# rug-marl-group2/scopa

Hardware: AMD Instinct MI355X
Metric: MiniScopa infoset-traversals/sec (higher is better)
Workload: dtype f64

## Files before the change

### include/scopa.h

```cpp
#ifndef SCOPA_H
#define SCOPA_H
#include <stddef.h>
#include <stdint.h>

#ifdef __cplusplus
extern "C" {
#endif

#define SCOPA_ABI_VERSION 1

enum {
    SCOPA_OK = 0,
    SCOPA_EINVAL = -1,
    SCOPA_ENODEV = -2,
    SCOPA_EHIP = -3,
    SCOPA_ESTATE = -4,
    SCOPA_ENOMEM = -5,
    SCOPA_ELIMIT = -6,
    SCOPA_ETIMEOUT = -7
};

#define SCOPA_N_CARDS 16
#define SCOPA_N_PLIES 8
#define SCOPA_N_DECISION 1653
#define SCOPA_N_TERMINAL 576
#define SCOPA_N_NODES 2229
#define SCOPA_MAX_ACTIONS 4

#define SCOPA_STEP_CLONED 0x80u
#define SCOPA_STEP_COUNT_MASK 0x7Fu
typedef struct scopa_state {
    uint16_t hand[2];
    uint32_t table;
    uint8_t  nh[2];
    uint8_t  nt;
    uint8_t  step;
    uint8_t  ncap[2];
    uint8_t  scopas[2];
} scopa_state;

typedef struct scopa_ctx scopa_ctx;

int32_t     scopa_abi_version(void);
const char *scopa_strerror(int32_t status);
const char *scopa_last_error(const scopa_ctx *ctx);

int32_t scopa_ctx_create(int32_t device_id, void *hip_stream, scopa_ctx **out);
int32_t scopa_ctx_destroy(scopa_ctx *ctx);
int32_t scopa_ctx_synchronize(scopa_ctx *ctx);

int32_t scopa_deal_py_seed(int64_t seed, uint8_t perm16[16]);
int32_t scopa_state_init(const uint8_t perm16[16], scopa_state *out);
int32_t scopa_state_step(scopa_state *s, int32_t action);
int32_t scopa_state_clone(const scopa_state *s, scopa_state *out);
int32_t scopa_state_is_terminal(const scopa_state *s);
int32_t scopa_state_current_player(const scopa_state *s);
int32_t scopa_state_legal(const scopa_state *s, int32_t player , int32_t out[4], int32_t *n);
int32_t scopa_state_rewards_x2(const scopa_state *s, int32_t r2[2]);
int32_t scopa_state_infoset_key(const scopa_state *s, int32_t player, uint64_t *key);
int32_t scopa_key_to_string(uint64_t key, char *buf, int32_t cap);
int32_t scopa_state_infoset_string(const scopa_state *s, int32_t player, char *buf, int32_t cap);

int32_t scopa_step_batch(scopa_ctx *ctx, scopa_state *d_states, const uint8_t *d_actions, int64_t n);
int32_t scopa_step_batch_host(scopa_ctx *ctx, scopa_state *h_states, const uint8_t *h_actions, int64_t n);

int32_t scopa_set_deal(scopa_ctx *ctx, const uint8_t perm16[16]);
int32_t scopa_tree_counts(scopa_ctx *ctx, int32_t *n_nodes, int32_t *n_decision, int32_t *n_infosets);
int32_t scopa_tree_export(scopa_ctx *ctx, scopa_state *h_states, int32_t *h_infoset, int8_t *h_r2,
                          uint64_t *h_infoset_key, int8_t *h_infoset_nlegal, int8_t *h_infoset_legal);

int32_t scopa_tables_reset(scopa_ctx *ctx);
int32_t scopa_tables_get(scopa_ctx *ctx, double *h_regret, double *h_strategy, double *h_local);
int32_t scopa_tables_set(scopa_ctx *ctx, const double *h_regret, const double *h_strategy, const double *h_local);

int32_t scopa_visited_get(scopa_ctx *ctx, uint32_t *h_seq);

int32_t scopa_cfr_exact_iterate(scopa_ctx *ctx, int32_t n_iters, double *h_root_values);
int32_t scopa_cfr_exact_traverse(scopa_ctx *ctx, int32_t traverser, double *h_value);
int32_t scopa_cfr_exact_mode(scopa_ctx *ctx, int32_t sequential);
int32_t scopa_cfr_exact_last_route(scopa_ctx *ctx, int32_t *route);
int32_t scopa_cfr_exact_traverse_from(scopa_ctx *ctx, int32_t traverser, int32_t depth, const int32_t *path,
                                      double reach_p0, double reach_p1, double *h_value);

int32_t scopa_cfr_sync_iterate(scopa_ctx *ctx, int32_t n_iters);

int32_t scopa_mccfr_replay(scopa_ctx *ctx, int32_t n_iters, const double *h_uniforms, int64_t n_uniforms,
                           int64_t *consumed);

int32_t scopa_mccfr_seed(scopa_ctx *ctx, uint64_t seed);
int32_t scopa_mccfr_iterate(scopa_ctx *ctx, uint32_t batch, uint32_t n_iters);
int32_t scopa_mccfr_traverse(scopa_ctx *ctx, uint32_t iteration, uint32_t b0, uint32_t nb);
int32_t scopa_mccfr_delta_buffer(scopa_ctx *ctx, void **d_delta, size_t *bytes);
int32_t scopa_mccfr_bind_delta(scopa_ctx *ctx, void *d_buf, size_t bytes);
int32_t scopa_mccfr_delta_get(scopa_ctx *ctx, double *h_delta);
int32_t scopa_mccfr_delta_set(scopa_ctx *ctx, const double *h_delta);
int32_t scopa_mccfr_apply(scopa_ctx *ctx);
int32_t scopa_mccfr_iteration_counter(scopa_ctx *ctx, uint32_t *iteration);
int32_t scopa_mccfr_graph_mode(scopa_ctx *ctx, int32_t on);
int32_t scopa_debug_lds_limit(scopa_ctx *ctx, int32_t bytes);

int32_t scopa_sdcfr_frontier_width(int32_t traverser, int32_t ply);
int32_t scopa_sdcfr_features(scopa_ctx *ctx, int32_t ply, int64_t n, const int32_t *d_idx, float *d_feats, float *d_mask);
int32_t scopa_sdcfr_expand(scopa_ctx *ctx, int32_t ply, int32_t traverser, int64_t n, const int32_t *d_idx, const float *d_adv,
                           int32_t *d_child_idx, float *d_pol, const double *d_uniforms, uint32_t iteration, uint32_t b0);
int32_t scopa_sdcfr_terminal_values(scopa_ctx *ctx, int32_t traverser, int64_t n, const int32_t *d_idx, float *d_val);
int32_t scopa_sdcfr_backward(scopa_ctx *ctx, int32_t ply, int32_t traverser, int64_t n, const int32_t *d_idx, const float *d_pol,
                             const float *d_child_val, float *d_val, const float *d_feats, const float *d_mask, float *d_mem_feat,
                             float *d_mem_regret, float *d_mem_mask, int64_t capacity, int64_t write_base);
int32_t scopa_sdcfr_visits(scopa_ctx *ctx, uint64_t *decision_visits);
int32_t scopa_sdcfr_policy_get(scopa_ctx *ctx, float *h_policy, uint64_t *h_thr);
#define SCOPA_SDCFR_IMAGE_FLOATS 13520
int32_t scopa_sdcfr_image_floats(void);
int32_t scopa_sdcfr_pack_weights(scopa_ctx *ctx, int32_t player, const float *d_w1, const float *d_b1, const float *d_w2,
                                 const float *d_b2, const float *d_w3, const float *d_b3, float *d_image);
int32_t scopa_sdcfr_traverse_fused(scopa_ctx *ctx, int32_t traverser, int32_t batch, const float *d_image, float *d_mem_feat,
                                   float *d_mem_regret, float *d_mem_mask, int64_t capacity, int64_t write_base,
                                   float *d_root_values, const double *d_uniforms, uint32_t iteration, uint32_t b0);
int32_t scopa_sdcfr_mode(scopa_ctx *ctx, int32_t forward_per_visit);
int32_t scopa_sdcfr_tuning(scopa_ctx *ctx, int32_t traversals_per_task, int32_t wavefronts_per_task);
int32_t scopa_sdcfr_train_params(void);
int32_t scopa_sdcfr_train_steps(scopa_ctx *ctx, const int64_t *d_rows, int32_t n_rows, int32_t n_steps, const float *d_feat, const float *d_regret, const float *d_mask,
                                int64_t capacity, float *d_w1, float *d_b1, float *d_w2, float *d_b2, float *d_w3, float *d_b3, float *d_state,
                                int32_t first_step, float lr, float *d_loss);
int32_t scopa_sdcfr_train_step(scopa_ctx *ctx, const int64_t *d_rows, int32_t n_rows, const float *d_feat, const float *d_regret, const float *d_mask,
                               int64_t capacity, float *d_w1, float *d_b1, float *d_w2, float *d_b2, float *d_w3, float *d_b3, float *d_state,
                               int32_t step, float lr, float *d_loss);
int32_t scopa_sdcfr_average_policy(scopa_ctx *ctx, int32_t player, int32_t n_snap, const float *d_w1, const float *d_b1, const float *d_w2,
                                   const float *d_b2, const float *d_w3, const float *d_b3, int32_t max_size, const int32_t *d_slots,
                                   const float *d_coef, double *d_policy);
int32_t scopa_features_from_states(scopa_ctx *ctx, const scopa_state *d_states, int64_t n, float *d_feats, float *d_mask);
int32_t scopa_eval_init_states(scopa_ctx *ctx, scopa_state *d_states, int64_t n);
int32_t scopa_eval_step(scopa_ctx *ctx, scopa_state *d_states, int64_t n, const float *d_probs, const int32_t *d_trained_seat,
                        uint32_t stream_id, uint32_t ply_tag);

int32_t scopa_eval_tabular_prepare(scopa_ctx *ctx, const double *d_policy);
int32_t scopa_eval_tabular_step(scopa_ctx *ctx, scopa_state *d_states, int32_t *d_node_idx, int64_t n, int32_t ply,
                                const double *d_policy, const int32_t *d_trained_seat, uint32_t stream_id);
int32_t scopa_eval_tabular_match(scopa_ctx *ctx, int64_t n, int64_t n_seat0, uint32_t stream_id, scopa_state *d_states_out, int32_t *d_node_idx_out,
                                 int64_t h_stats[10]);

int32_t scopa_exploitability(scopa_ctx *ctx, const double *h_policy, double *h_out4, double *h_policy_out);

typedef struct scopa_multi scopa_multi;
int32_t scopa_multi_create(scopa_ctx *ctx, int32_t n_deals, scopa_multi **out);
int32_t scopa_multi_destroy(scopa_multi *m);
int32_t scopa_multi_deal_py_seeds(scopa_multi *m, const int64_t *h_seeds);
int32_t scopa_multi_set_perms(scopa_multi *m, const uint8_t *h_perms );
int32_t scopa_multi_perms_get(scopa_multi *m, uint8_t *h_perms);
int32_t scopa_multi_build(scopa_multi *m, int32_t *h_n_infosets);
int32_t scopa_multi_cfr_exact_iterate(scopa_multi *m, int32_t n_iters);
int32_t scopa_multi_cfr_exact_iterate_lanes(scopa_multi *m, int32_t n_iters);
int32_t scopa_multi_cfr_sync_iterate(scopa_multi *m, int32_t n_iters);
int32_t scopa_multi_mccfr_iterate(scopa_multi *m, uint32_t batch, uint32_t n_iters, uint64_t seed);
int32_t scopa_multi_exploitability(scopa_multi *m, double *h_out4);
int32_t scopa_multi_tables_get(scopa_multi *m, int32_t deal, double *h_regret, double *h_strategy, double *h_local, uint64_t *h_keys);
int32_t scopa_multi_tables_set(scopa_multi *m, int32_t deal, const double *h_regret, const double *h_strategy, const double *h_local);
int32_t scopa_multi_counters(scopa_multi *m, uint64_t *decision_visits, uint64_t *terminal_visits);

typedef struct scopa_full_state {
    uint64_t table[2];
    uint64_t cap[2];
    uint32_t hand[2];
    uint32_t game;
    uint8_t  nh[2], nt, deck_pos, round, last_capture , scopas[2];
    uint16_t step;
    uint8_t  terminal;
    int8_t   r2_p0;
    uint8_t  flags;
    uint8_t  pad[7];
} scopa_full_state;
int32_t scopa_full_deal_py_seed(int64_t seed, uint8_t perm40[40]);
int32_t scopa_full_state_init(const uint8_t deck40[40], uint32_t game, scopa_full_state *out);
int32_t scopa_full_state_step(scopa_full_state *s, const uint8_t deck40[40], int32_t action);
int32_t scopa_full_state_legal(const scopa_full_state *s, int32_t player, int32_t out[3], int32_t *n);
int32_t scopa_full_state_infoset_string(const scopa_full_state *s, int32_t player, char *buf, int32_t cap);
int32_t scopa_full_step_batch(scopa_ctx *ctx, scopa_full_state *d_states, const uint8_t *d_actions, const uint8_t *d_decks, int64_t n);
int32_t scopa_full_step_batch_host(scopa_ctx *ctx, scopa_full_state *h_states, const uint8_t *h_actions, const uint8_t *h_decks,
                                   int64_t n_decks, int64_t n);
int32_t scopa_full_random_playouts(scopa_ctx *ctx, const int64_t *h_seeds, int64_t n_games, int8_t *h_r2_p0, int16_t *h_plies);

typedef struct scopa_team_state {
    uint64_t history;
    uint32_t table;
    uint16_t hand[4];
    uint16_t cap[4];
    uint8_t  nh[4];
    uint8_t  scopas[4];
    uint8_t  nt, step, last_capture_team , flags ;
} scopa_team_state;
int32_t scopa_team_state_init(const uint8_t perm16[16], scopa_team_state *out);
int32_t scopa_team_state_step(scopa_team_state *s, int32_t action);
int32_t scopa_team_state_legal(const scopa_team_state *s, int32_t out[4], int32_t *n);
int32_t scopa_team_state_rewards_x2(const scopa_team_state *s, int32_t r2_seat[4]);
int32_t scopa_team_state_infoset_string(const scopa_team_state *s, int32_t team, char *buf, int32_t cap);
int32_t scopa_team_step_batch(scopa_ctx *ctx, scopa_team_state *d_states, const uint8_t *d_actions, int64_t n);
int32_t scopa_team_step_batch_host(scopa_ctx *ctx, scopa_team_state *h_states, const uint8_t *h_actions, int64_t n);
int32_t scopa_team_random_playouts(scopa_ctx *ctx, const int64_t *h_seeds, int64_t n_games, int8_t *h_r2_team0, uint8_t *h_scopas);

int32_t scopa_p2p_create(scopa_ctx *ctx, int32_t rank, int32_t world, uint8_t handle_out[64]);
int32_t scopa_p2p_connect(scopa_ctx *ctx, const uint8_t *handles );
int32_t scopa_p2p_allreduce_delta(scopa_ctx *ctx);
int32_t scopa_p2p_set_form(scopa_ctx *ctx, int32_t light);
int32_t scopa_p2p_set_budget(scopa_ctx *ctx, double seconds);
int32_t scopa_mccfr_iterate_sharded(scopa_ctx *ctx, uint32_t b0, uint32_t nb, uint32_t n_iters);
int32_t scopa_p2p_status(scopa_ctx *ctx, int32_t *timeouts, uint64_t *exchanges);
int32_t scopa_p2p_destroy(scopa_ctx *ctx);

int32_t scopa_counters(scopa_ctx *ctx, uint64_t *decision_visits, uint64_t *terminal_visits);
int32_t scopa_prof_enable(scopa_ctx *ctx, int32_t stride);
int32_t scopa_prof_read(scopa_ctx *ctx, int64_t *launches, double *kernel_ms);
int32_t scopa_prof_device(scopa_ctx *ctx, int64_t *launches, double *kernel_ms);
int32_t scopa_prof_phases(scopa_ctx *ctx, double out_us[3]);
int32_t scopa_prof_spread(scopa_ctx *ctx, double out_us[3]);

#ifdef __cplusplus
}
#endif
#endif
```

### scopa_amd/_lib.py

```python
import ctypes as C
import os

import numpy as np

_HERE = os.path.dirname(os.path.abspath(__file__))
LIB_PATH = os.environ.get("SCOPA_HIP_LIBRARY") or os.path.join(_HERE, "libscopa_hip.so")

SCOPA_OK, SCOPA_EINVAL, SCOPA_ENODEV, SCOPA_EHIP, SCOPA_ESTATE, SCOPA_ENOMEM, SCOPA_ELIMIT, SCOPA_ETIMEOUT = 0, -1, -2, -3, -4, -5, -6, -7
N_NODES, N_DECISION, N_TERMINAL = 2229, 1653, 576

SYMBOLS = [
    "scopa_abi_version", "scopa_strerror", "scopa_last_error", "scopa_ctx_create", "scopa_ctx_destroy",
    "scopa_ctx_synchronize", "scopa_deal_py_seed", "scopa_state_init", "scopa_state_step", "scopa_state_clone", "scopa_state_is_terminal",
    "scopa_state_current_player", "scopa_state_legal", "scopa_state_rewards_x2", "scopa_state_infoset_key",
    "scopa_key_to_string", "scopa_state_infoset_string", "scopa_step_batch", "scopa_step_batch_host", "scopa_set_deal",
    "scopa_tree_counts", "scopa_tree_export", "scopa_tables_reset", "scopa_tables_get", "scopa_tables_set",
    "scopa_visited_get", "scopa_cfr_exact_iterate", "scopa_cfr_exact_traverse", "scopa_cfr_exact_mode", "scopa_cfr_exact_last_route", "scopa_cfr_exact_traverse_from", "scopa_mccfr_replay", "scopa_mccfr_seed",
    "scopa_mccfr_iterate", "scopa_mccfr_traverse", "scopa_mccfr_delta_buffer", "scopa_mccfr_bind_delta", "scopa_mccfr_delta_get", "scopa_mccfr_delta_set", "scopa_mccfr_apply",
    "scopa_mccfr_iteration_counter", "scopa_mccfr_graph_mode", "scopa_debug_lds_limit", "scopa_sdcfr_frontier_width", "scopa_sdcfr_features", "scopa_sdcfr_expand",
    "scopa_sdcfr_terminal_values", "scopa_sdcfr_backward", "scopa_sdcfr_visits", "scopa_sdcfr_policy_get", "scopa_sdcfr_traverse_fused", "scopa_sdcfr_image_floats", "scopa_sdcfr_pack_weights", "scopa_sdcfr_tuning", "scopa_sdcfr_mode", "scopa_sdcfr_train_params", "scopa_sdcfr_train_step", "scopa_sdcfr_train_steps", "scopa_sdcfr_average_policy", "scopa_features_from_states",
    "scopa_eval_init_states", "scopa_eval_step", "scopa_eval_tabular_step", "scopa_eval_tabular_prepare", "scopa_eval_tabular_match", "scopa_cfr_sync_iterate", "scopa_multi_create", "scopa_multi_destroy",
    "scopa_multi_deal_py_seeds", "scopa_multi_set_perms", "scopa_multi_perms_get", "scopa_multi_build", "scopa_multi_cfr_exact_iterate",
    "scopa_multi_cfr_exact_iterate_lanes", "scopa_multi_cfr_sync_iterate", "scopa_multi_mccfr_iterate", "scopa_multi_exploitability", "scopa_multi_tables_get", "scopa_multi_tables_set", "scopa_multi_counters", "scopa_full_deal_py_seed",
    "scopa_full_state_init", "scopa_full_state_step", "scopa_full_state_legal", "scopa_full_state_infoset_string",
    "scopa_full_step_batch", "scopa_full_step_batch_host", "scopa_full_random_playouts",
    "scopa_team_state_init", "scopa_team_state_step", "scopa_team_state_legal", "scopa_team_state_rewards_x2", "scopa_team_state_infoset_string",
    "scopa_team_step_batch", "scopa_team_step_batch_host", "scopa_team_random_playouts",
    "scopa_mccfr_iterate_sharded", "scopa_p2p_create", "scopa_p2p_connect", "scopa_p2p_allreduce_delta", "scopa_p2p_set_form", "scopa_p2p_set_budget", "scopa_p2p_status", "scopa_p2p_destroy", "scopa_exploitability", "scopa_counters", "scopa_prof_enable", "scopa_prof_read", "scopa_prof_device", "scopa_prof_phases", "scopa_prof_spread",
]


class ScopaError(RuntimeError):
    def __init__(self, status, where, detail=""):
        self.status = status
        msg = f"{where}: status {status}"
        try:
            msg += f" ({lib().scopa_strerror(status).decode()})"
        except Exception:
            pass
        if detail:
            msg += f": {detail}"
        super().__init__(msg)


class State16(C.Structure):
    _fields_ = [("hand", C.c_uint16 * 2), ("table", C.c_uint32), ("nh", C.c_uint8 * 2), ("nt", C.c_uint8),
                ("step", C.c_uint8), ("ncap", C.c_uint8 * 2), ("scopas", C.c_uint8 * 2)]


STEP_CLONED, STEP_COUNT_MASK = 0x80, 0x7F
STATE_DTYPE = np.dtype([("hand", "<u2", (2,)), ("table", "<u4"), ("nh", "u1", (2,)), ("nt", "u1"), ("step", "u1"),
                        ("ncap", "u1", (2,)), ("scopas", "u1", (2,))])
assert STATE_DTYPE.itemsize == 16 and C.sizeof(State16) == 16

_lib = None


def lib():
    global _lib
    if _lib is not None:
        return _lib
    try:
        import torch
    except ImportError:
        pass
    if not os.path.exists(LIB_PATH):
        raise OSError(f"{LIB_PATH} is missing: build it with `python __graft_entry__.py` or `python scopa_amd/build.py` "
                      "(the MiniScopa solver path has no fallback)")
    L = C.CDLL(LIB_PATH)
    vp, i32, i64, u32, u64 = C.c_void_p, C.c_int32, C.c_int64, C.c_uint32, C.c_uint64
    sig = {
        "scopa_abi_version": (i32, []),
        "scopa_strerror": (C.c_char_p, [i32]),
        "scopa_last_error": (C.c_char_p, [vp]),
        "scopa_ctx_create": (i32, [i32, vp, C.POINTER(vp)]),
        "scopa_ctx_destroy": (i32, [vp]),
        "scopa_ctx_synchronize": (i32, [vp]),
        "scopa_deal_py_seed": (i32, [i64, vp]),
        "scopa_state_init": (i32, [vp, C.POINTER(State16)]),
        "scopa_state_step": (i32, [C.POINTER(State16), i32]),
        "scopa_state_clone": (i32, [C.POINTER(State16), C.POINTER(State16)]),
        "scopa_state_is_terminal": (i32, [C.POINTER(State16)]),
        "scopa_state_current_player": (i32, [C.POINTER(State16)]),
        "scopa_state_legal": (i32, [C.POINTER(State16), i32, C.POINTER(i32 * 4), C.POINTER(i32)]),
        "scopa_state_rewards_x2": (i32, [C.POINTER(State16), C.POINTER(i32 * 2)]),
        "scopa_state_infoset_key": (i32, [C.POINTER(State16), i32, C.POINTER(u64)]),
        "scopa_key_to_string": (i32, [u64, C.c_char_p, i32]),
        "scopa_state_infoset_string": (i32, [C.POINTER(State16), i32, C.c_char_p, i32]),
        "scopa_step_batch": (i32, [vp, vp, vp, i64]),
        "scopa_step_batch_host": (i32, [vp, vp, vp, i64]),
        "scopa_set_deal": (i32, [vp, vp]),
        "scopa_tree_counts": (i32, [vp, C.POINTER(i32), C.POINTER(i32), C.POINTER(i32)]),
        "scopa_tree_export": (i32, [vp, vp, vp, vp, vp, vp, vp]),
        "scopa_tables_reset": (i32, [vp]),
        "scopa_tables_get": (i32, [vp, vp, vp, vp]),
        "scopa_tables_set": (i32, [vp, vp, vp, vp]),
        "scopa_cfr_exact_iterate": (i32, [vp, i32, vp]),
        "scopa_cfr_exact_traverse": (i32, [vp, i32, C.POINTER(C.c_double)]),
        "scopa_cfr_exact_mode": (i32, [vp, i32]),
        "scopa_cfr_exact_last_route": (i32, [vp, C.POINTER(i32)]),
        "scopa_cfr_exact_traverse_from": (i32, [vp, i32, i32, vp, C.c_double, C.c_double, C.POINTER(C.c_double)]),
        "scopa_visited_get": (i32, [vp, vp]),
        "scopa_mccfr_replay": (i32, [vp, i32, vp, i64, C.POINTER(i64)]),
        "scopa_mccfr_seed": (i32, [vp, u64]),
        "scopa_mccfr_iterate": (i32, [vp, u32, u32]),
        "scopa_mccfr_traverse": (i32, [vp, u32, u32, u32]),
        "scopa_mccfr_delta_buffer": (i32, [vp, C.POINTER(vp), C.POINTER(C.c_size_t)]),
        "scopa_mccfr_bind_delta": (i32, [vp, vp, C.c_size_t]),
        "scopa_mccfr_delta_get": (i32, [vp, vp]),
        "scopa_mccfr_delta_set": (i32, [vp, vp]),
        "scopa_mccfr_apply": (i32, [vp]),
        "scopa_mccfr_iteration_counter": (i32, [vp, C.POINTER(u32)]),
        "scopa_mccfr_graph_mode": (i32, [vp, i32]),
        "scopa_debug_lds_limit": (i32, [vp, i32]),
        "scopa_exploitability": (i32, [vp, vp, vp, vp]),
        "scopa_sdcfr_frontier_width": (i32, [i32, i32]),
        "scopa_sdcfr_features": (i32, [vp, i32, i64, vp, vp, vp]),
        "scopa_sdcfr_expand": (i32, [vp, i32, i32, i64, vp, vp, vp, vp, vp, u32, u32]),
        "scopa_sdcfr_terminal_values": (i32, [vp, i32, i64, vp, vp]),
        "scopa_sdcfr_backward": (i32, [vp, i32, i32, i64, vp, vp, vp, vp, vp, vp, vp, vp, vp, i64, i64]),
        "scopa_sdcfr_visits": (i32, [vp, C.POINTER(u64)]),
        "scopa_sdcfr_policy_get": (i32, [vp, vp, vp]),
        "scopa_sdcfr_traverse_fused": (i32, [vp, i32, i32, vp, vp, vp, vp, i64, i64, vp, vp, u32, u32]),
        "scopa_sdcfr_image_floats": (i32, []),
        "scopa_sdcfr_pack_weights": (i32, [vp, i32, vp, vp, vp, vp, vp, vp, vp]),
        "scopa_sdcfr_tuning": (i32, [vp, i32, i32]),
        "scopa_sdcfr_train_params": (i32, []),
        "scopa_sdcfr_train_step": (i32, [vp, vp, i32, vp, vp, vp, i64, vp, vp, vp, vp, vp, vp, vp, i32, C.c_float, vp]),
        "scopa_sdcfr_train_steps": (i32, [vp, vp, i32, i32, vp, vp, vp, i64, vp, vp, vp, vp, vp, vp, vp, i32, C.c_float, vp]),
        "scopa_sdcfr_mode": (i32, [vp, i32]),
        "scopa_sdcfr_average_policy": (i32, [vp, i32, i32, vp, vp, vp, vp, vp, vp, i32, vp, vp, vp]),
        "scopa_features_from_states": (i32, [vp, vp, i64, vp, vp]),
        "scopa_eval_init_states": (i32, [vp, vp, i64]),
        "scopa_eval_step": (i32, [vp, vp, i64, vp, vp, u32, u32]),
        "scopa_eval_tabular_step": (i32, [vp, vp, vp, i64, i32, vp, vp, u32]),
        "scopa_eval_tabular_prepare": (i32, [vp, vp]),
        "scopa_eval_tabular_match": (i32, [vp, i64, i64, u32, vp, vp, vp]),
        "scopa_cfr_sync_iterate": (i32, [vp, i32]),
        "scopa_multi_create": (i32, [vp, i32, C.POINTER(vp)]),
        "scopa_multi_destroy": (i32, [vp]),
        "scopa_multi_deal_py_seeds": (i32, [vp, vp]),
        "scopa_multi_set_perms": (i32, [vp, vp]),
        "scopa_multi_perms_get": (i32, [vp, vp]),
        "scopa_multi_build": (i32, [vp, vp]),
        "scopa_multi_cfr_exact_iterate": (i32, [vp, i32]),
        "scopa_multi_cfr_sync_iterate": (i32, [vp, i32]),
        "scopa_multi_cfr_exact_iterate_lanes": (i32, [vp, i32]),
        "scopa_multi_exploitability": (i32, [vp, vp]),
        "scopa_multi_mccfr_iterate": (i32, [vp, u32, u32, u64]),
        "scopa_multi_tables_get": (i32, [vp, i32, vp, vp, vp, vp]),
        "scopa_multi_tables_set": (i32, [vp, i32, vp, vp, vp]),
        "scopa_multi_counters": (i32, [vp, C.POINTER(u64), C.POINTER(u64)]),
        "scopa_full_deal_py_seed": (i32, [i64, vp]),
        "scopa_full_state_init": (i32, [vp, u32, vp]),
        "scopa_full_state_step": (i32, [vp, vp, i32]),
        "scopa_full_state_legal": (i32, [vp, i32, C.POINTER(i32 * 3), C.POINTER(i32)]),
        "scopa_full_state_infoset_string": (i32, [vp, i32, C.c_char_p, i32]),
        "scopa_full_step_batch": (i32, [vp, vp, vp, vp, i64]),
        "scopa_full_step_batch_host": (i32, [vp, vp, vp, vp, i64, i64]),
        "scopa_full_random_playouts": (i32, [vp, vp, i64, vp, vp]),
        "scopa_mccfr_iterate_sharded": (i32, [vp, u32, u32, u32]),
        "scopa_p2p_create": (i32, [vp, i32, i32, vp]),
        "scopa_p2p_connect": (i32, [vp, vp]),
        "scopa_p2p_allreduce_delta": (i32, [vp]),
        "scopa_p2p_set_form": (i32, [vp, i32]),
        "scopa_p2p_set_budget": (i32, [vp, C.c_double]),
        "scopa_p2p_status": (i32, [vp, C.POINTER(i32), C.POINTER(u64)]),
        "scopa_p2p_destroy": (i32, [vp]),
        "scopa_team_state_init": (i32, [vp, vp]),
        "scopa_team_state_step": (i32, [vp, i32]),
        "scopa_team_state_legal": (i32, [vp, C.POINTER(i32 * 4), C.POINTER(i32)]),
        "scopa_team_state_rewards_x2": (i32, [vp, C.POINTER(i32 * 4)]),
        "scopa_team_state_infoset_string": (i32, [vp, i32, C.c_char_p, i32]),
        "scopa_team_step_batch": (i32, [vp, vp, vp, i64]),
        "scopa_team_step_batch_host": (i32, [vp, vp, vp, i64]),
        "scopa_team_random_playouts": (i32, [vp, vp, i64, vp, vp]),
        "scopa_counters": (i32, [vp, C.POINTER(u64), C.POINTER(u64)]),
        "scopa_prof_enable": (i32, [vp, i32]),
        "scopa_prof_read": (i32, [vp, C.POINTER(i64), C.POINTER(C.c_double)]),
        "scopa_prof_device": (i32, [vp, C.POINTER(i64), C.POINTER(C.c_double)]),
        "scopa_prof_phases": (i32, [vp, C.POINTER(C.c_double * 3)]),
        "scopa_prof_spread": (i32, [vp, C.POINTER(C.c_double * 3)]),
    }
    lenient = bool(os.environ.get("SCOPA_HIP_LIBRARY")) and os.environ.get("SCOPA_AB_OLD_LIBRARY") == "1"
    for name, (res, args) in sig.items():
        if lenient and not hasattr(L, name):
            continue
        fn = getattr(L, name)
        fn.restype, fn.argtypes = res, args
    if L.scopa_abi_version() != 1:
        raise OSError("libscopa_hip.so ABI version mismatch")
    _lib = L
    return L


def _ptr(a):
    return a.ctypes.data_as(C.c_void_p) if a is not None else None


def deal_py_seed(seed):
    perm = np.zeros(16, np.uint8)
    rc = lib().scopa_deal_py_seed(int(seed), _ptr(perm))
    if rc:
        raise ScopaError(rc, "scopa_deal_py_seed")
    return perm


def key_to_string(key):
    buf = C.create_string_buffer(96)
    rc = lib().scopa_key_to_string(int(key), buf, 96)
    if rc < 0:
        raise ScopaError(rc, "scopa_key_to_string")
    return buf.value.decode()


class Context:

    def __init__(self, device=0, stream=None):
        self._h = C.c_void_p()
        self._L = lib()
        rc = self._L.scopa_ctx_create(int(device), C.c_void_p(stream) if stream else None, C.byref(self._h))
        if rc:
            self._h = None
            raise ScopaError(rc, "scopa_ctx_create", "a GPU is required: the solver path has no CPU fallback")
        self.device = device
        self.n_infosets = 0
        self._children = []

    def close(self):
        if getattr(self, "_h", None):
            for ref in getattr(self, "_children", []):
                child = ref()
                if child is not None:
                    child.close()
            self._L.scopa_ctx_destroy(self._h)
            self._h = None

    def __del__(self):
        try:
            self.close()
        except Exception:
            pass

    def _ck(self, rc, where):
        if rc:
            raise ScopaError(rc, where, self._L.scopa_last_error(self._h).decode())

    def synchronize(self):
        self._ck(self._L.scopa_ctx_synchronize(self._h), "scopa_ctx_synchronize")

    def step_batch_host(self, states, actions):
        assert states.dtype == STATE_DTYPE and states.flags.c_contiguous
        actions = np.ascontiguousarray(actions, np.uint8)
        assert actions.size == states.size
        self._ck(self._L.scopa_step_batch_host(self._h, _ptr(states), _ptr(actions), states.size), "scopa_step_batch_host")
        return states

    def step_batch(self, d_states_ptr, d_actions_ptr, n):
        self._ck(self._L.scopa_step_batch(self._h, C.c_void_p(d_states_ptr), C.c_void_p(d_actions_ptr), int(n)), "scopa_step_batch")

    def set_deal(self, perm16):
        perm = np.ascontiguousarray(perm16, np.uint8)
        assert perm.size == 16
        self._ck(self._L.scopa_set_deal(self._h, _ptr(perm)), "scopa_set_deal")
        a, b, c = C.c_int32(), C.c_int32(), C.c_int32()
        self._ck(self._L.scopa_tree_counts(self._h, C.byref(a), C.byref(b), C.byref(c)), "scopa_tree_counts")
        self.n_infosets = c.value
        self.perm = perm
        return self.n_infosets

    def tree_export(self):
        I = self.n_infosets
        out = dict(states=np.zeros(N_NODES, STATE_DTYPE), infoset=np.zeros(N_NODES, np.int32), r2=np.zeros((N_NODES, 2), np.int8),
                   infoset_key=np.zeros(I, np.uint64), infoset_nlegal=np.zeros(I, np.int8), infoset_legal=np.zeros((I, 4), np.int8))
        self._ck(self._L.scopa_tree_export(self._h, _ptr(out["states"]), _ptr(out["infoset"]), _ptr(out["r2"]),
                                           _ptr(out["infoset_key"]), _ptr(out["infoset_nlegal"]), _ptr(out["infoset_legal"])),
                 "scopa_tree_export")
        return out

    def tables_reset(self):
        self._ck(self._L.scopa_tables_reset(self._h), "scopa_tables_reset")

    def tables_get(self, regret=True, strategy=True, local=True):
        I = self.n_infosets
        R = np.zeros((I, 4)) if regret else None
        S = np.zeros((I, 4)) if strategy else None
        Lc = np.zeros((I, 4)) if local else None
        self._ck(self._L.scopa_tables_get(self._h, _ptr(R), _ptr(S), _ptr(Lc)), "scopa_tables_get")
        return R, S, Lc

    def tables_set(self, regret=None, strategy=None, local=None):
        arrs = []
        for a in (regret, strategy, local):
            if a is not None:
                a = np.ascontiguousarray(a, np.float64)
                assert a.shape == (self.n_infosets, 4)
            arrs.append(a)
        self._ck(self._L.scopa_tables_set(self._h, _ptr(arrs[0]), _ptr(arrs[1]), _ptr(arrs[2])), "scopa_tables_set")

    def cfr_exact_iterate(self, n_iters):
        rv = np.zeros((max(int(n_iters), 0), 2))
        self._ck(self._L.scopa_cfr_exact_iterate(self._h, int(n_iters), _ptr(rv)), "scopa_cfr_exact_iterate")
        return rv

    def cfr_exact_mode(self, sequential):
        self._ck(self._L.scopa_cfr_exact_mode(self._h, 1 if sequential else 0), "scopa_cfr_exact_mode")

    def cfr_exact_last_route(self):
        r = C.c_int32()
        self._ck(self._L.scopa_cfr_exact_last_route(self._h, C.byref(r)), "scopa_cfr_exact_last_route")
        return r.value

    def cfr_exact_traverse(self, traverser):
        v = C.c_double()
        self._ck(self._L.scopa_cfr_exact_traverse(self._h, int(traverser), C.byref(v)), "scopa_cfr_exact_traverse")
        return v.value

    def cfr_exact_traverse_from(self, traverser, path, reach_p0=1.0, reach_p1=1.0):
        pa = np.ascontiguousarray(path, np.int32)
        v = C.c_double()
        self._ck(self._L.scopa_cfr_exact_traverse_from(self._h, int(traverser), pa.size, _ptr(pa), float(reach_p0), float(reach_p1),
                                                       C.byref(v)), "scopa_cfr_exact_traverse_from")
        return v.value

    def visited_get(self):
        seq = np.zeros(self.n_infosets, np.uint32)
        self._ck(self._L.scopa_visited_get(self._h, _ptr(seq)), "scopa_visited_get")
        return seq

    def mccfr_replay(self, n_iters, uniforms):
        u = np.ascontiguousarray(uniforms, np.float64)
        used = C.c_int64()
        self._ck(self._L.scopa_mccfr_replay(self._h, int(n_iters), _ptr(u), u.size, C.byref(used)), "scopa_mccfr_replay")
        return used.value

    def mccfr_seed(self, seed):
        self._ck(self._L.scopa_mccfr_seed(self._h, int(seed)), "scopa_mccfr_seed")

    def mccfr_iterate(self, batch, n_iters):
        self._ck(self._L.scopa_mccfr_iterate(self._h, int(batch), int(n_iters)), "scopa_mccfr_iterate")

    def mccfr_traverse(self, iteration, b0, nb):
        self._ck(self._L.scopa_mccfr_traverse(self._h, int(iteration), int(b0), int(nb)), "scopa_mccfr_traverse")

    def mccfr_delta_buffer(self):
        p, n = C.c_void_p(), C.c_size_t()
        self._ck(self._L.scopa_mccfr_delta_buffer(self._h, C.byref(p), C.byref(n)), "scopa_mccfr_delta_buffer")
        return p.value, n.value

    def mccfr_bind_delta(self, d_ptr, nbytes):
        self._ck(self._L.scopa_mccfr_bind_delta(self._h, C.c_void_p(d_ptr) if d_ptr else None, int(nbytes)), "scopa_mccfr_bind_delta")

    def mccfr_delta_get(self):
        d = np.zeros((self.n_infosets, 5))
        self._ck(self._L.scopa_mccfr_delta_get(self._h, _ptr(d)), "scopa_mccfr_delta_get")
        return d

    def mccfr_delta_set(self, d):
        d = np.ascontiguousarray(d, np.float64)
        assert d.shape == (self.n_infosets, 5)
        self._ck(self._L.scopa_mccfr_delta_set(self._h, _ptr(d)), "scopa_mccfr_delta_set")

    def mccfr_apply(self):
        self._ck(self._L.scopa_mccfr_apply(self._h), "scopa_mccfr_apply")

    def mccfr_graph_mode(self, on):
        self._ck(self._L.scopa_mccfr_graph_mode(self._h, 1 if on else 0), "scopa_mccfr_graph_mode")

    def debug_lds_limit(self, nbytes):
        self._ck(self._L.scopa_debug_lds_limit(self._h, int(nbytes)), "scopa_debug_lds_limit")

    def mccfr_iteration(self):
        v = C.c_uint32()
        self._ck(self._L.scopa_mccfr_iteration_counter(self._h, C.byref(v)), "scopa_mccfr_iteration_counter")
        return v.value

    def exploitability(self, policy=None, return_policy=False):
        pin = None if policy is None else np.ascontiguousarray(policy, np.float64)
        out = np.zeros(4)
        pout = np.zeros((self.n_infosets, 4)) if return_policy else None
        self._ck(self._L.scopa_exploitability(self._h, _ptr(pin), _ptr(out), _ptr(pout)), "scopa_exploitability")
        res = dict(exploitability=out[0], br0=out[1], br1=out[2], value_p0=out[3])
        if return_policy:
            res["policy"] = pout
        return res

    def sdcfr_features(self, ply, n, idx_ptr, feats_ptr, mask_ptr):
        self._ck(self._L.scopa_sdcfr_features(self._h, ply, n, C.c_void_p(idx_ptr), C.c_void_p(feats_ptr), C.c_void_p(mask_ptr)), "scopa_sdcfr_features")

    def sdcfr_expand(self, ply, traverser, n, idx_ptr, adv_ptr, child_ptr, pol_ptr, uniforms_ptr, iteration, b0):
        self._ck(self._L.scopa_sdcfr_expand(self._h, ply, traverser, n, C.c_void_p(idx_ptr), C.c_void_p(adv_ptr), C.c_void_p(child_ptr),
                                            C.c_void_p(pol_ptr), C.c_void_p(uniforms_ptr) if uniforms_ptr else None, iteration, b0), "scopa_sdcfr_expand")

    def sdcfr_terminal_values(self, traverser, n, idx_ptr, val_ptr):
        self._ck(self._L.scopa_sdcfr_terminal_values(self._h, traverser, n, C.c_void_p(idx_ptr), C.c_void_p(val_ptr)), "scopa_sdcfr_terminal_values")

    def sdcfr_backward(self, ply, traverser, n, idx_ptr, pol_ptr, child_val_ptr, val_ptr, feats_ptr, mask_ptr, mem_feat_ptr, mem_regret_ptr,
                       mem_mask_ptr, capacity, write_base):
        vp = lambda x: C.c_void_p(x) if x else None
        self._ck(self._L.scopa_sdcfr_backward(self._h, ply, traverser, n, vp(idx_ptr), vp(pol_ptr), vp(child_val_ptr), vp(val_ptr), vp(feats_ptr),
                                              vp(mask_ptr), vp(mem_feat_ptr), vp(mem_regret_ptr), vp(mem_mask_ptr), capacity, write_base),
                 "scopa_sdcfr_backward")

    def sdcfr_pack_weights(self, player, w1_ptr, b1_ptr, w2_ptr, b2_ptr, w3_ptr, b3_ptr, image_ptr):
        self._ck(self._L.scopa_sdcfr_pack_weights(self._h, player, *(C.c_void_p(x) for x in (w1_ptr, b1_ptr, w2_ptr, b2_ptr, w3_ptr, b3_ptr, image_ptr))),
                 "scopa_sdcfr_pack_weights")

    def sdcfr_mode(self, forward_per_visit):
        self._ck(self._L.scopa_sdcfr_mode(self._h, 1 if forward_per_visit else 0), "scopa_sdcfr_mode")

    def sdcfr_tuning(self, traversals_per_task=0, wavefronts_per_task=0):
        self._ck(self._L.scopa_sdcfr_tuning(self._h, traversals_per_task, wavefronts_per_task), "scopa_sdcfr_tuning")

    def sdcfr_train_steps(self, rows_ptr, n_rows, n_steps, feat_ptr, regret_ptr, mask_ptr, capacity, param_ptrs, state_ptr, first_step, lr, loss_ptr):
        self._ck(self._L.scopa_sdcfr_train_steps(self._h, C.c_void_p(rows_ptr), int(n_rows), int(n_steps), C.c_void_p(feat_ptr), C.c_void_p(regret_ptr), C.c_void_p(mask_ptr),
                                                 int(capacity), *(C.c_void_p(p) for p in param_ptrs), C.c_void_p(state_ptr), int(first_step), float(lr),
                                                 C.c_void_p(loss_ptr)), "scopa_sdcfr_train_steps")

    def sdcfr_train_step(self, rows_ptr, n_rows, feat_ptr, regret_ptr, mask_ptr, capacity, param_ptrs, state_ptr, step, lr, loss_ptr):
        self._ck(self._L.scopa_sdcfr_train_step(self._h, C.c_void_p(rows_ptr), int(n_rows), C.c_void_p(feat_ptr), C.c_void_p(regret_ptr), C.c_void_p(mask_ptr),
                                                int(capacity), *(C.c_void_p(p) for p in param_ptrs), C.c_void_p(state_ptr), int(step), float(lr),
                                                C.c_void_p(loss_ptr)), "scopa_sdcfr_train_step")

    def sdcfr_traverse_fused(self, traverser, batch, weights_ptr, mem_feat_ptr, mem_regret_ptr, mem_mask_ptr, capacity, write_base,
                             root_values_ptr, uniforms_ptr, iteration, b0):
        self._ck(self._L.scopa_sdcfr_traverse_fused(self._h, traverser, batch, C.c_void_p(weights_ptr), C.c_void_p(mem_feat_ptr),
                                                    C.c_void_p(mem_regret_ptr), C.c_void_p(mem_mask_ptr), capacity, write_base,
                                                    C.c_void_p(root_values_ptr), C.c_void_p(uniforms_ptr) if uniforms_ptr else None,
                                                    iteration, b0), "scopa_sdcfr_traverse_fused")

    def sdcfr_average_policy(self, player, n_snap, param_ptrs, max_size, slots_ptr, coef_ptr, policy_ptr):
        vp = lambda x: C.c_void_p(x) if x else None
        self._ck(self._L.scopa_sdcfr_average_policy(self._h, int(player), int(n_snap), *(vp(p) for p in param_ptrs), int(max_size), vp(slots_ptr),
                                                    vp(coef_ptr), vp(policy_ptr)), "scopa_sdcfr_average_policy")

    def sdcfr_visits(self):
        v = C.c_uint64()
        self._ck(self._L.scopa_sdcfr_visits(self._h, C.byref(v)), "scopa_sdcfr_visits")
        return v.value

    def sdcfr_policy_get(self):
        pol, thr = np.zeros((N_DECISION, 4), np.float32), np.zeros((N_DECISION, 3), np.uint64)
        self._ck(self._L.scopa_sdcfr_policy_get(self._h, _ptr(pol), _ptr(thr)), "scopa_sdcfr_policy_get")
        return pol, thr

    def features_from_states(self, states_ptr, n, feats_ptr, mask_ptr):
        self._ck(self._L.scopa_features_from_states(self._h, C.c_void_p(states_ptr), n, C.c_void_p(feats_ptr), C.c_void_p(mask_ptr)), "scopa_features_from_states")

    def eval_init_states(self, states_ptr, n):
        self._ck(self._L.scopa_eval_init_states(self._h, C.c_void_p(states_ptr), n), "scopa_eval_init_states")

    def eval_step(self, states_ptr, n, probs_ptr, seat_ptr, stream_id, ply_tag):
        self._ck(self._L.scopa_eval_step(self._h, C.c_void_p(states_ptr), n, C.c_void_p(probs_ptr) if probs_ptr else None, C.c_void_p(seat_ptr),
                                         stream_id, ply_tag), "scopa_eval_step")

    def eval_tabular_prepare(self, policy_ptr):
        self._ck(self._L.scopa_eval_tabular_prepare(self._h, C.c_void_p(policy_ptr)), "scopa_eval_tabular_prepare")

    def eval_tabular_step(self, states_ptr, idx_ptr, n, ply, policy_ptr, seat_ptr, stream_id):
        self._ck(self._L.scopa_eval_tabular_step(self._h, C.c_void_p(states_ptr), C.c_void_p(idx_ptr), n, ply, C.c_void_p(policy_ptr) if policy_ptr else None,
                                                 C.c_void_p(seat_ptr), stream_id), "scopa_eval_tabular_step")

    def eval_tabular_match(self, n, n_seat0, stream_id, states_ptr=0, idx_ptr=0):
        st = np.zeros((2, 5), np.int64)
        self._ck(self._L.scopa_eval_tabular_match(self._h, int(n), int(n_seat0), stream_id, C.c_void_p(states_ptr) if states_ptr else None,
                                                  C.c_void_p(idx_ptr) if idx_ptr else None, _ptr(st)), "scopa_eval_tabular_match")
        return st

    def cfr_sync_iterate(self, n_iters):
        self._ck(self._L.scopa_cfr_sync_iterate(self._h, int(n_iters)), "scopa_cfr_sync_iterate")

    def full_step_batch_host(self, states, actions, decks):
        assert states.dtype == FULL_STATE_DTYPE
        actions = np.ascontiguousarray(actions, np.uint8)
        decks = np.ascontiguousarray(decks, np.uint8).reshape(-1, 40)
        self._ck(self._L.scopa_full_step_batch_host(self._h, _ptr(states), _ptr(actions), _ptr(decks), decks.shape[0], states.size),
                 "scopa_full_step_batch_host")
        return states

    def full_step_batch(self, states_ptr, actions_ptr, decks_ptr, n):
        self._ck(self._L.scopa_full_step_batch(self._h, C.c_void_p(states_ptr), C.c_void_p(actions_ptr), C.c_void_p(decks_ptr), int(n)), "scopa_full_step_batch")

    def full_random_playouts(self, seeds):
        seeds = np.ascontiguousarray(seeds, np.int64)
        r2, plies = np.zeros(seeds.size, np.int8), np.zeros(seeds.size, np.int16)
        self._ck(self._L.scopa_full_random_playouts(self._h, _ptr(seeds), seeds.size, _ptr(r2), _ptr(plies)), "scopa_full_random_playouts")
        return r2, plies

    def p2p_create(self, rank, world):
        h = np.zeros(64, np.uint8)
        self._ck(self._L.scopa_p2p_create(self._h, int(rank), int(world), _ptr(h)), "scopa_p2p_create")
        return h

    def p2p_connect(self, handles):
        handles = np.ascontiguousarray(handles, np.uint8).reshape(-1, 64)
        self._ck(self._L.scopa_p2p_connect(self._h, _ptr(handles)), "scopa_p2p_connect")

    def p2p_allreduce_delta(self):
        self._ck(self._L.scopa_p2p_allreduce_delta(self._h), "scopa_p2p_allreduce_delta")

    def mccfr_iterate_sharded(self, b0, nb, n_iters=1):
        self._ck(self._L.scopa_mccfr_iterate_sharded(self._h, int(b0), int(nb), int(n_iters)), "scopa_mccfr_iterate_sharded")

    def p2p_status(self):
        t, n = C.c_int32(), C.c_uint64()
        self._ck(self._L.scopa_p2p_status(self._h, C.byref(t), C.byref(n)), "scopa_p2p_status")
        return t.value, n.value

    def p2p_set_form(self, light):
        self._ck(self._L.scopa_p2p_set_form(self._h, 1 if light else 0), "scopa_p2p_set_form")

    def p2p_set_budget(self, seconds):
        self._ck(self._L.scopa_p2p_set_budget(self._h, float(seconds)), "scopa_p2p_set_budget")

    def p2p_destroy(self):
        self._ck(self._L.scopa_p2p_destroy(self._h), "scopa_p2p_destroy")

    def team_step_batch_host(self, states, actions):
        assert states.dtype == TEAM_STATE_DTYPE
        actions = np.ascontiguousarray(actions, np.uint8)
        self._ck(self._L.scopa_team_step_batch_host(self._h, _ptr(states), _ptr(actions), states.size), "scopa_team_step_batch_host")
        return states

    def team_step_batch(self, states_ptr, actions_ptr, n):
        self._ck(self._L.scopa_team_step_batch(self._h, C.c_void_p(states_ptr), C.c_void_p(actions_ptr), int(n)), "scopa_team_step_batch")

    def team_random_playouts(self, seeds):
        seeds = np.ascontiguousarray(seeds, np.int64)
        r2, sc = np.zeros(seeds.size, np.int8), np.zeros((seeds.size, 4), np.uint8)
        self._ck(self._L.scopa_team_random_playouts(self._h, _ptr(seeds), seeds.size, _ptr(r2), _ptr(sc)), "scopa_team_random_playouts")
        return r2, sc

    def counters(self):
        a, b = C.c_uint64(), C.c_uint64()
        self._ck(self._L.scopa_counters(self._h, C.byref(a), C.byref(b)), "scopa_counters")
        return a.value, b.value

    def prof_enable(self, stride=1):
        self._ck(self._L.scopa_prof_enable(self._h, int(stride)), "scopa_prof_enable")

    def prof_read(self):
        n, ms = C.c_int64(), C.c_double()
        self._ck(self._L.scopa_prof_read(self._h, C.byref(n), C.byref(ms)), "scopa_prof_read")
        return n.value, ms.value

    def prof_phases(self):
        out = (C.c_double * 3)()
        self._ck(self._L.scopa_prof_phases(self._h, C.byref(out)), "scopa_prof_phases")
        return tuple(out)

    def prof_spread(self):
        out = (C.c_double * 3)()
        self._ck(self._L.scopa_prof_spread(self._h, C.byref(out)), "scopa_prof_spread")
        return [out[0], out[1], out[2]]

    def prof_device(self):
        n, ms = C.c_int64(), C.c_double()
        self._ck(self._L.scopa_prof_device(self._h, C.byref(n), C.byref(ms)), "scopa_prof_device")
        return n.value, ms.value


FULL_STATE_DTYPE = np.dtype([("table", "<u8", (2,)), ("cap", "<u8", (2,)), ("hand", "<u4", (2,)), ("game", "<u4"), ("nh", "u1", (2,)),
                             ("nt", "u1"), ("deck_pos", "u1"), ("round", "u1"), ("last_capture", "u1"), ("scopas", "u1", (2,)),
                             ("step", "<u2"), ("terminal", "u1"), ("r2_p0", "i1"), ("flags", "u1"), ("pad", "u1", (7,))])
assert FULL_STATE_DTYPE.itemsize == 64


def full_deal_py_seed(seed):
    perm = np.zeros(40, np.uint8)
    rc = lib().scopa_full_deal_py_seed(int(seed), _ptr(perm))
    if rc:
        raise ScopaError(rc, "scopa_full_deal_py_seed")
    return perm


class FullState:

    def __init__(self, seed=42, deck=None, game=0):
        self.deck = np.ascontiguousarray(full_deal_py_seed(seed) if deck is None else deck, np.uint8)
        self.s = np.zeros(1, FULL_STATE_DTYPE)
        rc = lib().scopa_full_state_init(_ptr(self.deck), int(game), _ptr(self.s))
        if rc:
            raise ScopaError(rc, "scopa_full_state_init")

    def step(self, action):
        rc = lib().scopa_full_state_step(_ptr(self.s), _ptr(self.deck), int(action))
        if rc:
            raise ScopaError(rc, "scopa_full_state_step")

    def legal(self, player=-1):
        out, n = (C.c_int32 * 3)(), C.c_int32()
        lib().scopa_full_state_legal(_ptr(self.s), int(player), C.byref(out), C.byref(n))
        return [out[i] for i in range(n.value)]

    def is_terminal(self):
        return bool(self.s[0]["terminal"])

    def current_player(self):
        return -4 if self.is_terminal() else int(self.s[0]["step"]) & 1

    def rewards(self):
        r = int(self.s[0]["r2_p0"])
        return [r / 2.0, -r / 2.0] if self.is_terminal() else [0, 0]

    def infoset_string(self, player):
        buf = C.create_string_buffer(256)
        lib().scopa_full_state_infoset_string(_ptr(self.s), int(player), buf, 256)
        return buf.value.decode()

    def snapshot(self):
        return unpack_full_state(self.s[0])


def unpack_full_state(s):
    tab = [int((int(s["table"][i // 10]) >> (6 * (i % 10))) & 63) for i in range(int(s["nt"]))]
    hands = [[int((int(s["hand"][p]) >> (6 * i)) & 63) for i in range(int(s["nh"][p]))] for p in range(2)]
    caps = [[c for c in range(40) if (int(s["cap"][p]) >> c) & 1] for p in range(2)]
    last = int(s["last_capture"])
    return dict(hands=hands, table=tab, caps=caps, scopas=[int(s["scopas"][0]), int(s["scopas"][1])], round=int(s["round"]),
                step=int(s["step"]), deck_remaining=40 - int(s["deck_pos"]), last=-1 if last == 255 else last)


TEAM_STATE_DTYPE = np.dtype([("history", "<u8"), ("table", "<u4"), ("hand", "<u2", (4,)), ("cap", "<u2", (4,)), ("nh", "u1", (4,)),
                             ("scopas", "u1", (4,)), ("nt", "u1"), ("step", "u1"), ("last_capture_team", "u1"), ("flags", "u1")])
assert TEAM_STATE_DTYPE.itemsize == 40


class TeamState:

    def __init__(self, seed=42, perm=None):
        self.perm = np.ascontiguousarray(deal_py_seed(seed) if perm is None else perm, np.uint8)
        self.s = np.zeros(1, TEAM_STATE_DTYPE)
        rc = lib().scopa_team_state_init(_ptr(self.perm), _ptr(self.s))
        if rc:
            raise ScopaError(rc, "scopa_team_state_init")

    def copy(self):
        c = TeamState.__new__(TeamState)
        c.perm, c.s = self.perm, self.s.copy()
        return c

    def step(self, action):
        rc = lib().scopa_team_state_step(_ptr(self.s), int(action))
        if rc:
            raise ScopaError(rc, "scopa_team_state_step")

    def legal(self):
        out, n = (C.c_int32 * 4)(), C.c_int32()
        lib().scopa_team_state_legal(_ptr(self.s), C.byref(out), C.byref(n))
        return [out[i] for i in range(n.value)]

    def is_terminal(self):
        return bool(int(self.s[0]["flags"]) & 1)

    def seat(self):
        return int(self.s[0]["step"]) & 3

    def current_player(self):
        return -4 if self.is_terminal() else self.seat() >> 1

    def player_rewards(self):
        r = (C.c_int32 * 4)()
        lib().scopa_team_state_rewards_x2(_ptr(self.s), C.byref(r))
        return [r[i] / 2.0 for i in range(4)]

    def rewards(self):
        if not self.is_terminal():
            return [0, 0]
        r = self.player_rewards()
        return [(r[0] + r[1]) / 2, (r[2] + r[3]) / 2]

    def infoset_string(self, team):
        buf = C.create_string_buffer(256)
        lib().scopa_team_state_infoset_string(_ptr(self.s), int(team), buf, 256)
        return buf.value.decode()

    def history(self):
        h = int(self.s[0]["history"])
        return [(h >> (4 * i)) & 15 for i in range(int(self.s[0]["step"]))]

    def history_str(self):
        h = "-".join(map(str, self.history()))
        if self.is_terminal():
            return f"TERMINAL:{h}:" + ",".join(f"{r:.2f}" for r in self.rewards())
        return f"H:{h}:T{self.current_player()}"

    def snapshot(self):
        d = unpack_team_state(self.s[0])
        d.update(cur=self.current_player(), legal=self.legal(), info0=self.infoset_string(0), info1=self.infoset_string(1),
                 hist=self.history_str(), rewards=[float(r) for r in self.rewards()])
        return d


def unpack_team_state(s):
    hands = [[(int(s["hand"][p]) >> (4 * i)) & 15 for i in range(int(s["nh"][p]))] for p in range(4)]
    last = int(s["last_capture_team"])
    return dict(hands=hands, table=[(int(s["table"]) >> (4 * i)) & 15 for i in range(int(s["nt"]))],
                caps=[[c for c in range(16) if (int(s["cap"][p]) >> c) & 1] for p in range(4)], scopas=[int(x) for x in s["scopas"]],
                last=-1 if last == 255 else last, step=int(s["step"]), seat=int(s["step"]) & 3, term=bool(int(s["flags"]) & 1))


class MultiDeal:

    def __init__(self, ctx, n_deals):
        self.ctx, self.n = ctx, int(n_deals)
        self._L = lib()
        self._h = C.c_void_p()
        ctx._ck(self._L.scopa_multi_create(ctx._h, self.n, C.byref(self._h)), "scopa_multi_create")
        self.n_infosets = None
        import weakref
        ctx._children.append(weakref.ref(self))

    def close(self):
        if getattr(self, "_h", None):
            self._L.scopa_multi_destroy(self._h)
            self._h = None

    def __del__(self):
        try:
            self.close()
        except Exception:
            pass

    def deal_py_seeds(self, seeds):
        s = np.ascontiguousarray(seeds, np.int64)
        assert s.size == self.n
        self.ctx._ck(self._L.scopa_multi_deal_py_seeds(self._h, _ptr(s)), "scopa_multi_deal_py_seeds")

    def set_perms(self, perms):
        p = np.ascontiguousarray(perms, np.uint8)
        assert p.shape == (self.n, 16)
        self.ctx._ck(self._L.scopa_multi_set_perms(self._h, _ptr(p)), "scopa_multi_set_perms")

    def perms(self):
        p = np.zeros((self.n, 16), np.uint8)
        self.ctx._ck(self._L.scopa_multi_perms_get(self._h, _ptr(p)), "scopa_multi_perms_get")
        return p

    def build(self):
        ninf = np.zeros(self.n, np.int32)
        self.ctx._ck(self._L.scopa_multi_build(self._h, _ptr(ninf)), "scopa_multi_build")
        self.n_infosets = ninf
        return ninf

    def cfr_exact_iterate(self, n_iters):
        self.ctx._ck(self._L.scopa_multi_cfr_exact_iterate(self._h, int(n_iters)), "scopa_multi_cfr_exact_iterate")

    def cfr_exact_iterate_lanes(self, n_iters):
        self.ctx._ck(self._L.scopa_multi_cfr_exact_iterate_lanes(self._h, int(n_iters)), "scopa_multi_cfr_exact_iterate_lanes")

    def cfr_sync_iterate(self, n_iters):
        self.ctx._ck(self._L.scopa_multi_cfr_sync_iterate(self._h, int(n_iters)), "scopa_multi_cfr_sync_iterate")

    def mccfr_iterate(self, batch, n_iters, seed=0x5C09A):
        self.ctx._ck(self._L.scopa_multi_mccfr_iterate(self._h, int(batch), int(n_iters), int(seed)), "scopa_multi_mccfr_iterate")

    def exploitability(self):
        out = np.zeros((self.n, 4))
        self.ctx._ck(self._L.scopa_multi_exploitability(self._h, _ptr(out)), "scopa_multi_exploitability")
        return out

    def tables_get(self, deal):
        I = int(self.n_infosets[deal])
        R, S, Lc, K = np.zeros((I, 4)), np.zeros((I, 4)), np.zeros((I, 4)), np.zeros(I, np.uint64)
        self.ctx._ck(self._L.scopa_multi_tables_get(self._h, int(deal), _ptr(R), _ptr(S), _ptr(Lc), _ptr(K)), "scopa_multi_tables_get")
        return R, S, Lc, K

    def tables_set(self, deal, regret=None, strategy=None, local=None):
        arrs = []
        for a in (regret, strategy, local):
            if a is not None:
                a = np.ascontiguousarray(a, np.float64)
                assert a.shape == (int(self.n_infosets[deal]), 4)
            arrs.append(a)
        self.ctx._ck(self._L.scopa_multi_tables_set(self._h, int(deal), _ptr(arrs[0]), _ptr(arrs[1]), _ptr(arrs[2])), "scopa_multi_tables_set")

    def counters(self):
        a, b = C.c_uint64(), C.c_uint64()
        self.ctx._ck(self._L.scopa_multi_counters(self._h, C.byref(a), C.byref(b)), "scopa_multi_counters")
        return a.value, b.value
```

### scopa_amd/csrc/scopa_ctx.h

```cpp
#pragma once
#include <hip/hip_runtime.h>
#include <stdint.h>
#include <stdio.h>

#include <vector>

#include "../../include/scopa.h"
#include "scopa_rules.h"

struct scopa_p2p;

struct scopa_ctx {
    int device = -1;
    hipStream_t stream = nullptr;
    bool own_stream = false;
    char err[512] = {0};

    bool has_deal = false;
    uint8_t perm[16] = {0};
    int n_infosets = 0;

    scopa_state *d_states = nullptr;
    uint16_t *d_infoset = nullptr;
    int8_t *d_payoff = nullptr;
    uint64_t *d_key = nullptr;
    int32_t *d_meta = nullptr;
    uint32_t *d_visit = nullptr;

    double *d_regret = nullptr, *d_strat = nullptr, *d_local = nullptr;
    double *d_delta = nullptr;
    double *d_delta_own = nullptr;
    double *d_scratch = nullptr;
    double *d_sigcdf = nullptr;
    bool sigcdf_valid = false;
    bool mccfr_all_seen = false;
    uint32_t mccfr_seen_wait = 0;
    double *d_groups = nullptr;
    unsigned long long *d_clock = nullptr;
    uint16_t clock_grid[2048] = {0};
    double prof_phase_us[3] = {0.0, 0.0, 0.0};
    double prof_spread_us[3] = {0.0, 0.0, 0.0};
    size_t scratch_bytes = 0;

    unsigned long long *d_counters = nullptr;

    uint64_t seed = 0x5C09A;
    uint64_t sdcfr_visits = 0;
    void *d_sdnode = nullptr;
    bool sdnode_valid = false;
    void *d_eval_thr = nullptr;
    bool eval_thr_valid = false;
    void *d_train_partial = nullptr;
    void *d_sdpol = nullptr;
    void *d_sdavg = nullptr;
    size_t sdavg_bytes = 0;
    int sdcfr_mode = 0;
    uint32_t iteration = 0;

    bool prof_on = false;
    int prof_stride = 1;
    long long prof_tick = 0;
    std::vector<hipEvent_t> ev_pool;
    size_t ev_used = 0;
    int64_t prof_launches = 0;
    double prof_ms = 0.0;

    uint32_t *d_lane_tab = nullptr;
    uint16_t *d_sched = nullptr;
    int sched_steps = 0;
    bool sched_valid = false;
    int exact_last_route = -1;
    bool exact_sequential = false;

    scopa_p2p *p2p = nullptr;

    struct GraphEntry { uint32_t batch, k, track; void *exec; };
    std::vector<GraphEntry> mccfr_graphs;
    bool mccfr_graph_mode = false;

    int lds_limit = 160 * 1024;
    int n_cus = 256;
    uint32_t lds_attr_done = 0;
};

namespace scopa {

#ifndef SCOPA_GROUPS
#define SCOPA_GROUPS 16
#endif
#ifndef SCOPA_GROUP_PERM
#define SCOPA_GROUP_PERM 0
#endif
constexpr int kDeltaGroups = SCOPA_GROUPS;
constexpr int kGroupRows = 1664;
constexpr size_t kDeltaTable = (size_t)kGroupRows * 5;
__host__ __device__ inline size_t group_cell(int k, int r) {
#if SCOPA_GROUP_PERM == 1
    return (size_t)k * kGroupRows + (size_t)((r & 63) * 26 + (r >> 6));
#elif SCOPA_GROUP_PERM == 2
    return (size_t)k * kGroupRows + (size_t)((r & 7) * 208 + (r >> 3));
#else
    return (size_t)k * kGroupRows + (size_t)r;
#endif
}
constexpr int kClockSamples = 2048, kClockStride = 2048;

inline int32_t fail(scopa_ctx *ctx, int32_t code, const char *what, hipError_t e = hipSuccess) {
    if (ctx) {
        if (e != hipSuccess) snprintf(ctx->err, sizeof ctx->err, "%s: %s", what, hipGetErrorString(e));
        else snprintf(ctx->err, sizeof ctx->err, "%s", what);
    }
    return code;
}

#define SC_HIP(ctx, call)                                                         \
    do {                                                                          \
        hipError_t e__ = (call);                                                  \
        if (e__ != hipSuccess) return scopa::fail((ctx), SCOPA_EHIP, #call, e__); \
    } while (0)

#define SC_REQUIRE(ctx, cond, code, msg)                        \
    do {                                                        \
        if (!(cond)) return scopa::fail((ctx), (code), (msg)); \
    } while (0)

int32_t ensure_scratch(scopa_ctx *ctx, size_t bytes);

void range_push(const char *name);
void range_pop();
struct Range { explicit Range(const char *n) { range_push(n); } ~Range() { range_pop(); } };

enum LdsAttrKernel : uint32_t { kLdsTraverse = 1u, kLdsReplay = 8u, kLdsCfrExact = 16u, kLdsCfrSched = 512u, kLdsExploit = 32u, kLdsCfrSync = 64u, kLdsSdcfr = 128u, kLdsMulti = 256u, kLdsSdcfrReplay = 1024u, kLdsSdPolicy = 2048u, kLdsSdWalk0 = 4096u, kLdsSdWalk1 = 8192u };
inline int32_t ensure_lds_attr(scopa_ctx *ctx, uint32_t kernel_bit, const void *fn, int bytes) {
    if (ctx->lds_attr_done & kernel_bit) return SCOPA_OK;
    SC_HIP(ctx, hipFuncSetAttribute(fn, hipFuncAttributeMaxDynamicSharedMemorySize, bytes));
    ctx->lds_attr_done |= kernel_bit;
    return SCOPA_OK;
}
#define SC_LDS_ATTR(ctx, bit, kernel, bytes)                                                                     \
    do {                                                                                                         \
        const int32_t rc__ = scopa::ensure_lds_attr((ctx), (bit), reinterpret_cast<const void *>(kernel), (bytes)); \
        if (rc__ != SCOPA_OK) return rc__;                                                                       \
    } while (0)
bool prof_events(scopa_ctx *ctx, hipEvent_t *start, hipEvent_t *stop);
void p2p_release(scopa_ctx *ctx);
void mccfr_graphs_clear(scopa_ctx *ctx);

}
```

### scopa_amd/csrc/scopa_host.hip

```cpp
#include <string.h>

#include <new>

#include "scopa_ctx.h"

using namespace scopa;

namespace scopa {

int32_t ensure_scratch(scopa_ctx *ctx, size_t bytes) {
    if (bytes <= ctx->scratch_bytes) return SCOPA_OK;
    if (ctx->d_scratch) SC_HIP(ctx, hipFree(ctx->d_scratch));
    ctx->d_scratch = nullptr;
    ctx->scratch_bytes = 0;
    SC_HIP(ctx, hipMalloc(&ctx->d_scratch, bytes));
    ctx->scratch_bytes = bytes;
    return SCOPA_OK;
}

static void prof_pool_fill(scopa_ctx *ctx) {
    while (ctx->ev_pool.size() < 4096) {
        hipEvent_t e;
        if (hipEventCreate(&e) != hipSuccess) break;
        ctx->ev_pool.push_back(e);
    }
}

bool prof_events(scopa_ctx *ctx, hipEvent_t *start, hipEvent_t *stop) {
    if (!ctx->prof_on) return false;
    if ((ctx->prof_tick++ % ctx->prof_stride) != 0) return false;
    if (ctx->ev_used + 2 > ctx->ev_pool.size()) {
        if (ctx->ev_used) {
            (void)hipEventSynchronize(ctx->ev_pool[ctx->ev_used - 1]);
            for (size_t i = 0; i + 1 < ctx->ev_used; i += 2) {
                float ms = 0.f;
                if (hipEventElapsedTime(&ms, ctx->ev_pool[i], ctx->ev_pool[i + 1]) == hipSuccess) ctx->prof_ms += ms;
            }
            ctx->ev_used = 0;
        }
        if (ctx->ev_pool.empty()) prof_pool_fill(ctx);
    }
    if (ctx->ev_used + 2 > ctx->ev_pool.size()) return false;
    *start = ctx->ev_pool[ctx->ev_used];
    *stop = ctx->ev_pool[ctx->ev_used + 1];
    ctx->ev_used += 2;
    ctx->prof_launches++;
    return true;
}

}

#include <dlfcn.h>
namespace scopa {
namespace {
int (*g_roctx_push)(const char *) = nullptr;
int (*g_roctx_pop)() = nullptr;
int g_roctx_state = 0;
void roctx_resolve() {
    g_roctx_state = -1;
    const char *on = getenv("SCOPA_ROCTX");
    if (!on || on[0] != '1') return;
    for (const char *lib : {"librocprofiler-sdk-roctx.so", "libroctx64.so"}) {
        void *h = dlopen(lib, RTLD_NOW | RTLD_GLOBAL);
        if (!h) continue;
        g_roctx_push = reinterpret_cast<int (*)(const char *)>(dlsym(h, "roctxRangePushA"));
        g_roctx_pop = reinterpret_cast<int (*)()>(dlsym(h, "roctxRangePop"));
        if (g_roctx_push && g_roctx_pop) { g_roctx_state = 1; return; }
    }
}
}
void range_push(const char *name) {
    if (g_roctx_state == 0) roctx_resolve();
    if (g_roctx_state == 1) (void)g_roctx_push(name);
}
void range_pop() {
    if (g_roctx_state == 1) (void)g_roctx_pop();
}
}

extern "C" {

int32_t scopa_abi_version(void) { return SCOPA_ABI_VERSION; }

const char *scopa_strerror(int32_t status) {
    switch (status) {
        case SCOPA_OK: return "ok";
        case SCOPA_EINVAL: return "invalid argument";
        case SCOPA_ENODEV: return "no usable HIP device (the solver path has no CPU fallback)";
        case SCOPA_EHIP: return "HIP runtime error";
        case SCOPA_ESTATE: return "call order violated";
        case SCOPA_ENOMEM: return "out of memory";
        case SCOPA_ELIMIT: return "problem exceeds a compiled-in capacity";
        case SCOPA_ETIMEOUT: return "a peer did not answer within the wait budget";
        default: return "unknown status";
    }
}

const char *scopa_last_error(const scopa_ctx *ctx) { return ctx ? ctx->err : "null context"; }

int32_t scopa_ctx_create(int32_t device_id, void *hip_stream, scopa_ctx **out) {
    if (!out || device_id < 0) return SCOPA_EINVAL;
    *out = nullptr;
    int count = 0;
    if (hipGetDeviceCount(&count) != hipSuccess || count <= 0) return SCOPA_ENODEV;
    if (device_id >= count) return SCOPA_ENODEV;
    scopa_ctx *ctx = new (std::nothrow) scopa_ctx();
    if (!ctx) return SCOPA_ENOMEM;
    ctx->device = device_id;
    hipError_t e = hipSetDevice(device_id);
    if (e != hipSuccess) { delete ctx; return SCOPA_ENODEV; }
    hipDeviceProp_t prop;
    if (hipGetDeviceProperties(&prop, device_id) == hipSuccess) {
        ctx->n_cus = prop.multiProcessorCount;
        ctx->lds_limit = (int)prop.sharedMemPerBlock;
    }
    if (hip_stream) ctx->stream = (hipStream_t)hip_stream;
    else {
        e = hipStreamCreateWithFlags(&ctx->stream, hipStreamNonBlocking);
        if (e != hipSuccess) { delete ctx; return SCOPA_EHIP; }
        ctx->own_stream = true;
    }
    const size_t rows = (size_t)kDecision;
    bool ok = hipMalloc(&ctx->d_states, sizeof(scopa_state) * kNodes) == hipSuccess &&
              hipMalloc(&ctx->d_infoset, sizeof(uint16_t) * kDecision) == hipSuccess &&
              hipMalloc(&ctx->d_payoff, kTerminal) == hipSuccess &&
              hipMalloc(&ctx->d_key, sizeof(uint64_t) * kDecision) == hipSuccess &&
              hipMalloc(&ctx->d_meta, sizeof(int32_t) * 8) == hipSuccess &&
              hipMalloc(&ctx->d_visit, sizeof(uint32_t) * kDecision) == hipSuccess &&
              hipMalloc(&ctx->d_sigcdf, (size_t)kDecision * 6 * sizeof(double)) == hipSuccess &&
              hipMalloc(&ctx->d_groups, scopa::kDeltaGroups * scopa::kDeltaTable * sizeof(double)) == hipSuccess &&
              hipMalloc(&ctx->d_regret, rows * 4 * sizeof(double)) == hipSuccess &&
              hipMalloc(&ctx->d_strat, rows * 4 * sizeof(double)) == hipSuccess &&
              hipMalloc(&ctx->d_local, rows * 4 * sizeof(double)) == hipSuccess &&
              hipMalloc(&ctx->d_delta_own, rows * 5 * sizeof(double)) == hipSuccess &&
              hipMalloc(&ctx->d_counters, (8 + 2 * 1024) * sizeof(unsigned long long)) == hipSuccess;
    ctx->d_delta = ctx->d_delta_own;
    if (ok) ok = hipMemsetAsync(ctx->d_counters, 0, (8 + 2 * 1024) * sizeof(unsigned long long), ctx->stream) == hipSuccess &&
                 hipMemsetAsync(ctx->d_delta, 0, rows * 5 * sizeof(double), ctx->stream) == hipSuccess &&
                 hipMemsetAsync(ctx->d_groups, 0, scopa::kDeltaGroups * scopa::kDeltaTable * sizeof(double), ctx->stream) == hipSuccess;
    if (!ok) { scopa_ctx_destroy(ctx); return SCOPA_ENOMEM; }
    *out = ctx;
    return SCOPA_OK;
}

int32_t scopa_ctx_destroy(scopa_ctx *ctx) {
    if (!ctx) return SCOPA_EINVAL;
    (void)hipSetDevice(ctx->device);
    (void)hipStreamSynchronize(ctx->stream);
    scopa::p2p_release(ctx);
    scopa::mccfr_graphs_clear(ctx);
    for (hipEvent_t e : ctx->ev_pool) (void)hipEventDestroy(e);
    void *bufs[] = {ctx->d_states, ctx->d_infoset, ctx->d_payoff, ctx->d_key, ctx->d_meta, ctx->d_regret, ctx->d_strat,
                    ctx->d_local, ctx->d_delta_own, ctx->d_scratch, ctx->d_counters, ctx->d_visit, ctx->d_sigcdf, ctx->d_groups, ctx->d_clock, ctx->d_sched, ctx->d_lane_tab, ctx->d_sdnode, ctx->d_sdpol, ctx->d_train_partial, ctx->d_eval_thr, ctx->d_sdavg};
    for (void *b : bufs) if (b) (void)hipFree(b);
    if (ctx->own_stream) (void)hipStreamDestroy(ctx->stream);
    delete ctx;
    return SCOPA_OK;
}

int32_t scopa_debug_lds_limit(scopa_ctx *ctx, int32_t bytes) {
    if (!ctx || bytes < 0) return SCOPA_EINVAL;
    hipDeviceProp_t prop;
    SC_HIP(ctx, hipGetDeviceProperties(&prop, ctx->device));
    SC_REQUIRE(ctx, bytes == 0 || (bytes >= 64 * 1024 && (size_t)bytes <= prop.sharedMemPerBlock), SCOPA_EINVAL, "scopa_debug_lds_limit: 0 or 64 KB .. the device's limit");
    ctx->lds_limit = bytes ? bytes : (int)prop.sharedMemPerBlock;
    ctx->lds_attr_done = 0;
    scopa::mccfr_graphs_clear(ctx);
    return SCOPA_OK;
}

int32_t scopa_ctx_synchronize(scopa_ctx *ctx) {
    if (!ctx) return SCOPA_EINVAL;
    SC_HIP(ctx, hipStreamSynchronize(ctx->stream));
    return SCOPA_OK;
}

namespace {
struct Mt19937 {
    uint32_t mt[624];
    int at = 624;
    void seed_u32(uint32_t s) {
        mt[0] = s;
        for (int i = 1; i < 624; i++) mt[i] = 1812433253u * (mt[i - 1] ^ (mt[i - 1] >> 30)) + (uint32_t)i;
        at = 624;
    }
    void seed_array(const uint32_t *key, int n) {
        seed_u32(19650218u);
        int i = 1, j = 0;
        for (int k = n > 624 ? n : 624; k > 0; k--) {
            mt[i] = (mt[i] ^ ((mt[i - 1] ^ (mt[i - 1] >> 30)) * 1664525u)) + key[j] + (uint32_t)j;
            if (++i >= 624) { mt[0] = mt[623]; i = 1; }
            if (++j >= n) j = 0;
        }
        for (int k = 623; k > 0; k--) {
            mt[i] = (mt[i] ^ ((mt[i - 1] ^ (mt[i - 1] >> 30)) * 1566083941u)) - (uint32_t)i;
            if (++i >= 624) { mt[0] = mt[623]; i = 1; }
        }
        mt[0] = 0x80000000u;
    }
    void refill() {
        for (int k = 0; k < 624; k++) {
            const uint32_t y = (mt[k] & 0x80000000u) | (mt[(k + 1) % 624] & 0x7fffffffu);
            mt[k] = mt[(k + 397) % 624] ^ (y >> 1) ^ ((y & 1u) ? 0x9908b0dfu : 0u);
        }
        at = 0;
    }
    uint32_t next() {
        if (at >= 624) refill();
        uint32_t y = mt[at++];
        y ^= y >> 11;
        y ^= (y << 7) & 0x9d2c5680u;
        y ^= (y << 15) & 0xefc60000u;
        y ^= y >> 18;
        return y;
    }
    uint32_t below(uint32_t n) {
        int bits = 32 - __builtin_clz(n);
        uint32_t r;
        do r = next() >> (32 - bits); while (r >= n);
        return r;
    }
};
}

int32_t scopa_deal_py_seed(int64_t seed, uint8_t perm16[16]) {
    if (!perm16) return SCOPA_EINVAL;
    const uint64_t a = seed < 0 ? (uint64_t)0 - (uint64_t)seed : (uint64_t)seed;
    const uint32_t key[2] = {(uint32_t)a, (uint32_t)(a >> 32)};
    Mt19937 g;
    g.seed_array(key, key[1] ? 2 : 1);
    for (int i = 0; i < 16; i++) perm16[i] = (uint8_t)i;
    for (uint32_t i = 15; i >= 1; i--) {
        const uint32_t j = g.below(i + 1);
        const uint8_t t = perm16[i]; perm16[i] = perm16[j]; perm16[j] = t;
    }
    return SCOPA_OK;
}

static bool perm_ok(const uint8_t *p) {
    uint32_t seen = 0;
    for (int i = 0; i < 16; i++) { if (p[i] > 15) return false; seen |= 1u << p[i]; }
    return seen == 0xFFFFu;
}

int32_t scopa_state_init(const uint8_t perm16[16], scopa_state *out) {
    if (!perm16 || !out || !perm_ok(perm16)) return SCOPA_EINVAL;
    state_init(*out, perm16);
    return SCOPA_OK;
}

int32_t scopa_state_step(scopa_state *s, int32_t action) {
    if (!s || action < 0 || action > 15) return SCOPA_EINVAL;
    step(*s, action);
    return SCOPA_OK;
}

int32_t scopa_state_clone(const scopa_state *s, scopa_state *out) {
    if (!s || !out) return SCOPA_EINVAL;
    scopa_state c = *s;
    if (!is_terminal(c)) c.step = (uint8_t)(c.step | SCOPA_STEP_CLONED);
    *out = c;
    return SCOPA_OK;
}

int32_t scopa_state_is_terminal(const scopa_state *s) { return s ? (is_terminal(*s) ? 1 : 0) : SCOPA_EINVAL; }

int32_t scopa_state_current_player(const scopa_state *s) { return s ? current_player(*s) : SCOPA_EINVAL; }

int32_t scopa_state_legal(const scopa_state *s, int32_t player, int32_t out[4], int32_t *n) {
    if (!s || !out || !n || player > 1) return SCOPA_EINVAL;
    int tmp[4];
    *n = legal(*s, player, tmp);
    for (int i = 0; i < *n; i++) out[i] = tmp[i];
    return SCOPA_OK;
}

int32_t scopa_state_rewards_x2(const scopa_state *s, int32_t r2[2]) {
    if (!s || !r2) return SCOPA_EINVAL;
    int a, b;
    rewards_x2(*s, a, b);
    r2[0] = a; r2[1] = b;
    return SCOPA_OK;
}

int32_t scopa_state_infoset_key(const scopa_state *s, int32_t player, uint64_t *key) {
    if (!s || !key || player > 1) return SCOPA_EINVAL;
    if (player < 0) player = s->step & 1;
    *key = infoset_key(*s, player);
    return SCOPA_OK;
}

int32_t scopa_key_to_string(uint64_t key, char *buf, int32_t cap) {
    if (!buf || cap < 64) return SCOPA_EINVAL;
    static const char suit[4] = {'c', 'f', 'p', 'b'};
    const int player = (int)(key & 1), nh = (int)((key >> 1) & 7), nt = (int)((key >> 20) & 15);
    const uint32_t hand = (uint32_t)((key >> 4) & 0xFFFF), table = (uint32_t)(key >> 24);
    char *w = buf;
    w += sprintf(w, "P%d:H[", player);
    for (int i = 0; i < nh; i++) w += sprintf(w, "%s%d%c", i ? "-" : "", card_rank(nib(hand, i)), suit[nib(hand, i) >> 2]);
    w += sprintf(w, "]_T[");
    for (int i = 0; i < nt; i++) w += sprintf(w, "%s%d%c", i ? "-" : "", card_rank(nib(table, i)), suit[nib(table, i) >> 2]);
    w += sprintf(w, "]");
    return (int32_t)(w - buf);
}

int32_t scopa_state_infoset_string(const scopa_state *s, int32_t player, char *buf, int32_t cap) {
    if (!s || !buf || cap < 64 || player > 1) return SCOPA_EINVAL;
    if (player < 0) player = current_player(*s);
    if (is_terminal(*s) || player < 0) return (int32_t)sprintf(buf, "TERMINAL");
    return scopa_key_to_string(infoset_key(*s, player), buf, cap);
}

int32_t scopa_tables_get(scopa_ctx *ctx, double *h_regret, double *h_strategy, double *h_local) {
    if (!ctx) return SCOPA_EINVAL;
    SC_REQUIRE(ctx, ctx->has_deal, SCOPA_ESTATE, "scopa_tables_get: no deal set");
    const size_t bytes = (size_t)ctx->n_infosets * 4 * sizeof(double);
    if (h_regret) SC_HIP(ctx, hipMemcpyAsync(h_regret, ctx->d_regret, bytes, hipMemcpyDeviceToHost, ctx->stream));
    if (h_strategy) SC_HIP(ctx, hipMemcpyAsync(h_strategy, ctx->d_strat, bytes, hipMemcpyDeviceToHost, ctx->stream));
    if (h_local) SC_HIP(ctx, hipMemcpyAsync(h_local, ctx->d_local, bytes, hipMemcpyDeviceToHost, ctx->stream));
    SC_HIP(ctx, hipStreamSynchronize(ctx->stream));
    return SCOPA_OK;
}

int32_t scopa_tables_set(scopa_ctx *ctx, const double *h_regret, const double *h_strategy, const double *h_local) {
    if (!ctx) return SCOPA_EINVAL;
    SC_REQUIRE(ctx, ctx->has_deal, SCOPA_ESTATE, "scopa_tables_set: no deal set");
    const size_t bytes = (size_t)ctx->n_infosets * 4 * sizeof(double);
    if (h_regret) SC_HIP(ctx, hipMemcpyAsync(ctx->d_regret, h_regret, bytes, hipMemcpyHostToDevice, ctx->stream));
    if (h_strategy) SC_HIP(ctx, hipMemcpyAsync(ctx->d_strat, h_strategy, bytes, hipMemcpyHostToDevice, ctx->stream));
    if (h_local) SC_HIP(ctx, hipMemcpyAsync(ctx->d_local, h_local, bytes, hipMemcpyHostToDevice, ctx->stream));
    SC_HIP(ctx, hipStreamSynchronize(ctx->stream));
    ctx->sigcdf_valid = false;
    return SCOPA_OK;
}

int32_t scopa_sdcfr_policy_get(scopa_ctx *ctx, float *h_policy, uint64_t *h_thr) {
    if (!ctx || (!h_policy && !h_thr)) return SCOPA_EINVAL;
    SC_REQUIRE(ctx, ctx->d_sdpol != nullptr, SCOPA_ESTATE, "scopa_sdcfr_policy_get: no policy-table launch yet");
    if (h_policy) SC_HIP(ctx, hipMemcpyAsync(h_policy, ctx->d_sdpol, (size_t)kDecision * 4 * sizeof(float), hipMemcpyDeviceToHost, ctx->stream));
    if (h_thr) SC_HIP(ctx, hipMemcpyAsync(h_thr, reinterpret_cast<const float4 *>(ctx->d_sdpol) + kDecision, (size_t)kDecision * 3 * sizeof(uint64_t),
                                          hipMemcpyDeviceToHost, ctx->stream));
    SC_HIP(ctx, hipStreamSynchronize(ctx->stream));
    return SCOPA_OK;
}

int32_t scopa_visited_get(scopa_ctx *ctx, uint32_t *h_seq) {
    if (!ctx || !h_seq) return SCOPA_EINVAL;
    SC_REQUIRE(ctx, ctx->has_deal, SCOPA_ESTATE, "scopa_visited_get: no deal set");
    SC_HIP(ctx, hipMemcpyAsync(h_seq, ctx->d_visit, (size_t)ctx->n_infosets * sizeof(uint32_t), hipMemcpyDeviceToHost, ctx->stream));
    SC_HIP(ctx, hipStreamSynchronize(ctx->stream));
    return SCOPA_OK;
}

int32_t scopa_counters(scopa_ctx *ctx, uint64_t *decision_visits, uint64_t *terminal_visits) {
    if (!ctx) return SCOPA_EINVAL;
    static_assert(sizeof(unsigned long long) == 8, "counter layout");
    std::vector<unsigned long long> h(8 + 2 * 1024);
    SC_HIP(ctx, hipMemcpyAsync(h.data(), ctx->d_counters, h.size() * sizeof(unsigned long long), hipMemcpyDeviceToHost, ctx->stream));
    SC_HIP(ctx, hipStreamSynchronize(ctx->stream));
    unsigned long long d = h[0], t = h[1];
    for (int w = 0; w < 1024; w++) { d += h[8 + 2 * w]; t += h[9 + 2 * w]; }
    if (decision_visits) *decision_visits = d;
    if (terminal_visits) *terminal_visits = t;
    return SCOPA_OK;
}

int32_t scopa_prof_device(scopa_ctx *ctx, int64_t *launches, double *kernel_ms) {
    if (!ctx) return SCOPA_EINVAL;
    SC_HIP(ctx, hipStreamSynchronize(ctx->stream));
    const int64_t n = ctx->d_clock ? (ctx->prof_launches < scopa::kClockSamples ? ctx->prof_launches : scopa::kClockSamples) : 0;
    unsigned long long ticks = 0;
    if (n > 0) {
        std::vector<unsigned long long> h((size_t)n * scopa::kClockStride);
        SC_HIP(ctx, hipMemcpy(h.data(), ctx->d_clock, h.size() * sizeof(unsigned long long), hipMemcpyDeviceToHost));
        double ph[3] = {0.0, 0.0, 0.0}, sp[4] = {0.0, 0.0, 0.0, 0.0};
        long long wgs = 0, launches_seen = 0;
        for (int64_t s = 0; s < n; s++) {
            unsigned long long t0 = ~0ull, t1 = 0ull, late = 0ull, longest = 0ull;
            for (int w = 0; w < ctx->clock_grid[s]; w++) {
                const unsigned long long *q = &h[(size_t)s * scopa::kClockStride + 4 * w];
                t0 = q[0] < t0 ? q[0] : t0; t1 = q[3] > t1 ? q[3] : t1;
                for (int k = 0; k < 3; k++) ph[k] += (double)(q[k + 1] - q[k]);
                wgs++;
            }
            for (int w = 0; w < ctx->clock_grid[s]; w++) {
                const unsigned long long *q = &h[(size_t)s * scopa::kClockStride + 4 * w];
                sp[0] += (double)(q[0] - t0);
                late = q[0] - t0 > late ? q[0] - t0 : late;
                longest = q[3] - q[0] > longest ? q[3] - q[0] : longest;
            }
            if (ctx->clock_grid[s]) { sp[1] += (double)late; sp[2] += (double)longest; launches_seen++; }
            if (t1 > t0) ticks += t1 - t0;
        }
        for (int k = 0; k < 3; k++) ctx->prof_phase_us[k] = wgs ? ph[k] * 1e-2 / (double)wgs : 0.0;
        ctx->prof_spread_us[0] = wgs ? sp[0] * 1e-2 / (double)wgs : 0.0;
        ctx->prof_spread_us[1] = launches_seen ? sp[1] * 1e-2 / (double)launches_seen : 0.0;
        ctx->prof_spread_us[2] = launches_seen ? sp[2] * 1e-2 / (double)launches_seen : 0.0;
    }
    if (launches) *launches = n;
    if (kernel_ms) *kernel_ms = (double)ticks * 1e-5;
    return SCOPA_OK;
}

int32_t scopa_prof_phases(scopa_ctx *ctx, double out_us[3]) {
    if (!ctx || !out_us) return SCOPA_EINVAL;
    for (int k = 0; k < 3; k++) out_us[k] = ctx->prof_phase_us[k];
    return SCOPA_OK;
}

int32_t scopa_debug_clock_dump(scopa_ctx *ctx, unsigned long long *out, int32_t n, int32_t max_grid) {
    if (!ctx || !out || n <= 0 || !ctx->d_clock) return SCOPA_EINVAL;
    SC_HIP(ctx, hipStreamSynchronize(ctx->stream));
    const int64_t have = ctx->prof_launches < scopa::kClockSamples ? ctx->prof_launches : scopa::kClockSamples;
    if (have < n) return SCOPA_ESTATE;
    int grid = 0;
    for (int32_t s = 0; s < n; s++) {
        const int64_t slot = (ctx->prof_launches - 1 - s) % scopa::kClockSamples;
        grid = ctx->clock_grid[slot];
        if (grid <= 0 || grid > max_grid) return SCOPA_ELIMIT;
        SC_HIP(ctx, hipMemcpy(out + (size_t)s * max_grid * 4, ctx->d_clock + (size_t)slot * scopa::kClockStride, (size_t)grid * 4 * sizeof(unsigned long long), hipMemcpyDeviceToHost));
    }
    return grid;
}

int32_t scopa_prof_spread(scopa_ctx *ctx, double out_us[3]) {
    if (!ctx || !out_us) return SCOPA_EINVAL;
    for (int k = 0; k < 3; k++) out_us[k] = ctx->prof_spread_us[k];
    return SCOPA_OK;
}

int32_t scopa_prof_enable(scopa_ctx *ctx, int32_t stride) {
    if (!ctx || stride < 0) return SCOPA_EINVAL;
    SC_HIP(ctx, hipStreamSynchronize(ctx->stream));
    ctx->prof_on = stride != 0;
    ctx->prof_stride = stride > 0 ? stride : 1;
    ctx->prof_tick = 0;
    ctx->ev_used = 0;
    ctx->prof_launches = 0;
    ctx->prof_ms = 0.0;
    if (ctx->prof_on) scopa::prof_pool_fill(ctx);
    if (ctx->prof_on && !ctx->d_clock)
        SC_HIP(ctx, hipMalloc(&ctx->d_clock, (size_t)scopa::kClockSamples * scopa::kClockStride * sizeof(unsigned long long)));
    return SCOPA_OK;
}

int32_t scopa_prof_read(scopa_ctx *ctx, int64_t *launches, double *kernel_ms) {
    if (!ctx) return SCOPA_EINVAL;
    SC_HIP(ctx, hipStreamSynchronize(ctx->stream));
    for (size_t i = 0; i + 1 < ctx->ev_used; i += 2) {
        float ms = 0.f;
        if (hipEventElapsedTime(&ms, ctx->ev_pool[i], ctx->ev_pool[i + 1]) == hipSuccess) ctx->prof_ms += ms;
    }
    ctx->ev_used = 0;
    if (launches) *launches = ctx->prof_launches;
    if (kernel_ms) *kernel_ms = ctx->prof_ms;
    return SCOPA_OK;
}

}
```

### scopa_amd/csrc/scopa_mccfr.hip

```cpp
#include <hip/hip_ext.h>

#include "scopa_ctx.h"
#include "scopa_p2p.h"
#include "scopa_philox.h"

using namespace scopa;

namespace {

__device__ __forceinline__ void mc_sigma(const double *R, int n, double *sigma) {
    double pos[4];
#pragma unroll
    for (int i = 0; i < 4; i++) pos[i] = (i < n && R[i] > 0.0) ? R[i] : 0.0;
    double s = pos[0];
#pragma unroll
    for (int i = 1; i < 4; i++) if (i < n) s += pos[i];
#pragma unroll
    for (int i = 0; i < 4; i++) sigma[i] = i < n ? (s == 0.0 ? 1.0 / (double)n : pos[i] / s) : 0.0;
}

__device__ __forceinline__ void choice_cdf(const double *sigma, int n, uint32_t *thr) {
    double cdf[4];
    double c = sigma[0];
    cdf[0] = c;
#pragma unroll
    for (int i = 1; i < 4; i++) { if (i < n) c += sigma[i]; cdf[i] = c; }
    const double last = c;
#pragma unroll
    for (int i = 0; i < 4; i++) thr[i] = i < n ? (uint32_t)ceil((cdf[i] / last) * 2147483648.0) : 0xFFFFFFFFu;
}
__device__ __forceinline__ void row_store(double *__restrict__ row, const double *sg, const uint32_t *thr) {
    double2 *out = reinterpret_cast<double2 *>(row);
    out[0] = make_double2(sg[0], sg[1]);
    out[1] = make_double2(sg[2], sg[3]);
    out[2] = make_double2(__longlong_as_double((long long)(((unsigned long long)thr[1] << 32) | thr[0])),
                          __longlong_as_double((long long)(((unsigned long long)thr[3] << 32) | thr[2])));
}
__device__ __forceinline__ void choice_cdf_f64(const double *sigma, int n, double *cdf) {
    double c = sigma[0];
    cdf[0] = c;
    for (int i = 1; i < n; i++) { c += sigma[i]; cdf[i] = c; }
    const double last = cdf[n - 1];
    for (int i = 0; i < 4; i++) cdf[i] = i < n ? cdf[i] / last : 2.0;
}

__host__ __device__ constexpr int ntl_at(int trav, int d) { return trav == 0 ? (d + 1) >> 1 : d >> 1; }
__host__ __device__ constexpr int task_nodes(int trav, int d) {
    return ntl_at(trav, d) == 0 ? 1 : ntl_at(trav, d) == 1 ? 5 : ntl_at(trav, d) == 2 ? 20 : 60;
}

constexpr int kRow = 6;
constexpr int kUpd = 26;
constexpr unsigned int kPairDecisionVisits = (1 + 5 + 5 + 20 + 20 + 60 + 60 + 120) + (1 + 1 + 5 + 5 + 20 + 20 + 60 + 60), kPairTerminalVisits = 120 + 120;
static_assert(kPairDecisionVisits == 463, "291 + 172");

}

__global__ void __launch_bounds__(256)
k_mccfr_prepare(const uint64_t *__restrict__ g_key, const double *__restrict__ g_regret, double *__restrict__ g_sigcdf, int n_infosets) {
    const int r = blockIdx.x * blockDim.x + threadIdx.x;
    if (r >= n_infosets) return;
    const int n = (int)((g_key[r] >> 1) & 7);
    double R[4], sg[4];
    uint32_t thr[4];
    for (int c = 0; c < 4; c++) R[c] = g_regret[r * 4 + c];
    mc_sigma(R, n, sg);
    choice_cdf(sg, n, thr);
    row_store(g_sigcdf + r * kRow, sg, thr);
}

constexpr int kIdentSlot = 166;
struct WaveScratch {
    uint32_t npk[168];
    int8_t p6[128];
    uint32_t kdraw[64][4];
};
static_assert(sizeof(WaveScratch) % 16 == 0, "WaveScratch must keep 16-byte alignment");

__device__ __forceinline__ void wave_lds_sync() {
    __builtin_amdgcn_fence(__ATOMIC_RELEASE, "wavefront");
    __builtin_amdgcn_s_waitcnt(0xc07f);
    __builtin_amdgcn_wave_barrier();
    __builtin_amdgcn_fence(__ATOMIC_ACQUIRE, "wavefront");
}

__device__ __forceinline__ uint32_t lds_addr(const void *p) { return (uint32_t)(uintptr_t)(__attribute__((address_space(3))) const void *)p; }
__device__ __forceinline__ uint32_t lds_read_u32(uint32_t a) { return *(__attribute__((address_space(3))) const uint32_t *)(uintptr_t)a; }
__device__ __forceinline__ int lds_read_i8(uint32_t a) { return *(__attribute__((address_space(3))) const int8_t *)(uintptr_t)a; }
__device__ __forceinline__ double lds_read_f64(uint32_t a) { return *(__attribute__((address_space(3))) const double *)(uintptr_t)a; }
typedef uint32_t u32x4 __attribute__((ext_vector_type(4)));
__device__ __forceinline__ uint4 lds_read_u4(uint32_t a) {
    const u32x4 v = *(__attribute__((address_space(3))) const u32x4 *)(uintptr_t)a;
    return make_uint4(v.x, v.y, v.z, v.w);
}
__device__ __forceinline__ void lds_write_u4(uint32_t a, uint32_t x, uint32_t y, uint32_t z, uint32_t w) {
    *(__attribute__((address_space(3))) u32x4 *)(uintptr_t)a = u32x4{x, y, z, w};
}

constexpr int kLaneSlotVecs = 15;
constexpr int kStaticLds = 64 + kLaneSlotVecs * 1024;
constexpr int kStaticLdsMulti = kStaticLds;

template <int NP>
__device__ __forceinline__ void draw_pairs(uint32_t wsb, int lane, const uint32_t (&b)[NP], uint32_t iteration, uint32_t seed_lo, uint32_t seed_hi) {
    const int trav = lane < 44 ? 0 : 1, p = trav ? lane - 44 : lane;
    philox_out x[NP];
#pragma unroll
    for (int i = 0; i < NP; i++) x[i] = philox4x32_10((uint32_t)p, b[i], iteration, (uint32_t)trav, seed_lo, seed_hi);
#pragma unroll
    for (int i = 0; i < NP; i++)
        lds_write_u4(wsb + (uint32_t)(i * sizeof(WaveScratch) + offsetof(WaveScratch, kdraw)) + 16u * (uint32_t)lane, x[i].x0 >> 1, x[i].x1 >> 1, x[i].x2 >> 1, x[i].x3 >> 1);
    wave_lds_sync();
}

struct NodeRegs {
    uint32_t pk;
};

__host__ __device__ constexpr int npk_offset(int d) { return d == 0 ? 0 : d == 1 ? 2 : d == 2 ? 8 : d == 3 ? 18 : d == 4 ? 43 : 86; }
__host__ __device__ constexpr int npk_slot(int trav, int d, int j) { return npk_offset(d) + (trav ? task_nodes(0, d) : 0) + j; }
static_assert(npk_offset(1) == task_nodes(0, 0) + task_nodes(1, 0) && npk_offset(2) == npk_offset(1) + task_nodes(0, 1) + task_nodes(1, 1) &&
              npk_offset(3) == npk_offset(2) + task_nodes(0, 2) + task_nodes(1, 2) && npk_offset(4) == npk_offset(3) + task_nodes(0, 3) + task_nodes(1, 3) &&
              npk_offset(4) + task_nodes(0, 4) + task_nodes(1, 4) <= npk_offset(5) && npk_offset(5) + task_nodes(0, 5) + task_nodes(1, 5) == kIdentSlot,
              "record slots of plies 0..5 tile WaveScratch::npk");

constexpr int kLvLeaf = 7, kLvUpd = 9;
struct LaneTabRow { uint4 v[kLaneSlotVecs]; };

template <int D, int ROUND>
__device__ __forceinline__ void lane_slot_build(LaneTabRow &row, int lane) {
    constexpr int S = D + ROUND;
    constexpr int c0 = task_nodes(0, D), c1 = task_nodes(1, D);
    const int t = lane + 64 * ROUND;
    const bool valid = t < c0 + c1;
    const int trav = t < c0 ? 0 : 1;
    const int j = valid ? (trav ? t - c0 : t) : 0;
    const bool is_trav = (D & 1) == trav;
    const int ntl = trav == 0 ? (D + 1) >> 1 : D >> 1;
    uint32_t plane4 = 0u, amask = valid ? ~0u : 0u, aforce = 0u;
    if constexpr (D > 0) {
        constexpr int pd = D > 0 ? D - 1 : 0, pn = 4 - (pd >> 1);
        const bool p_trav = (pd & 1) == trav;
        int pj = j, br = 0;
        if (p_trav) { pj = j / (pn + 1); br = j - pj * (pn + 1); }
        if (valid) plane4 = 4u * (uint32_t)((trav ? task_nodes(0, pd) : 0) + pj);
        if (valid && p_trav && br > 0) { amask = 0u; aforce = (uint32_t)(br - 1); }
    }
    const int blk = (ntl == 0 ? 0 : ntl == 1 ? 1 : ntl == 2 ? 4 : 14) + (j >> 1);
    const uint32_t kword = valid ? (uint32_t)(offsetof(WaveScratch, kdraw) + 16 * ((trav ? 44 : 0) + blk) + 4 * ((j & 1) * 2 + (is_trav ? 1 : 0)))
                                 : (uint32_t)offsetof(WaveScratch, kdraw);
    row.v[S] = make_uint4(plane4, amask, aforce, kword);
}

__device__ __forceinline__ void upd_build(LaneTabRow &row, int x) {
    const uint32_t ident = (uint32_t)(offsetof(WaveScratch, npk) + 4 * kIdentSlot);
    uint32_t rec[5] = {ident, ident, ident, ident, ident}, am[5] = {24u, 24u, 24u, 24u, 24u}, af[5] = {0u, 0u, 0u, 0u, 0u};
    uint32_t own = ident, nX = 1u, p6o[4] = {(uint32_t)offsetof(WaveScratch, p6), (uint32_t)offsetof(WaveScratch, p6), (uint32_t)offsetof(WaveScratch, p6), (uint32_t)offsetof(WaveScratch, p6)};
    if (x < 2 * kUpd) {
        const int trav = x < kUpd ? 0 : 1, xx = trav ? x - kUpd : x;
        const int m = xx == 0 ? 0 : xx < 6 ? 1 : 2;
        int j = xx - (m == 0 ? 0 : m == 1 ? 1 : 6);
        const int d = 2 * m + trav;
        nX = (uint32_t)(4 - m);
        const int stride = m == 0 ? 12 : m == 1 ? 3 : 1;
        const int base = m == 0 ? 0 : m == 1 ? j * 12 : j * 3;
        for (int c = 0; c < 4; c++) p6o[c] = (uint32_t)(offsetof(WaveScratch, p6) + trav * 60 + base + ((c < (int)nX ? c : (int)nX - 1) + 1) * stride);
        own = (uint32_t)(offsetof(WaveScratch, npk) + 4 * npk_slot(trav, d, j));
        for (int c = d; c > 0; c--) {
            const int pd = c - 1, pn = 4 - (pd >> 1);
            int forced = 0;
            if ((pd & 1) == trav) { const int pj = j / (pn + 1), br = j - pj * (pn + 1); forced = br; j = pj; }
            rec[pd] = (uint32_t)(offsetof(WaveScratch, npk) + 4 * npk_slot(trav, pd, j));
            if (forced) { am[pd] = 0u; af[pd] = 8u * (uint32_t)(forced - 1); }
        }
    }
    row.v[kLvUpd + 0] = make_uint4(rec[0], rec[1], rec[2], rec[3]);
    row.v[kLvUpd + 1] = make_uint4(rec[4], own, nX, 0u);
    row.v[kLvUpd + 2] = make_uint4(p6o[0], p6o[1], p6o[2], p6o[3]);
    row.v[kLvUpd + 3] = make_uint4(am[0], am[1], am[2], am[3]);
    row.v[kLvUpd + 4] = make_uint4(am[4], af[0], af[1], af[2]);
    row.v[kLvUpd + 5] = make_uint4(af[3], af[4], 0u, 0u);
}

struct WalkEnv {
    uint32_t wsb;
    uint32_t tab;
    const uint16_t *s_inf;
    const int8_t *s_pay;
    const double *s_sigcdf;
    double *s_dR;
    uint8_t *s_seen;
    unsigned int *s_cnt;
};

template <int D, int NP>
__device__ __forceinline__ void ply_step(const WalkEnv &e, int lane, NodeRegs (&st)[NP]) {
    constexpr int n = 4 - (D >> 1);
    constexpr int c0 = task_nodes(0, D), c1 = task_nodes(1, D);
    constexpr int NR = c0 + c1 > 64 ? 2 : 1;
    struct Pre {
        int idx, In;
        uint32_t k, thr0, thr1, thr2;
    };
    Pre g[NP][NR];
    uint4 sl[NR];
#pragma unroll
    for (int r = 0; r < NR; r++) sl[r] = lds_read_u4(e.tab + 1024u * (uint32_t)(D + r));
#pragma unroll
    for (int i = 0; i < NP; i++)
#pragma unroll
        for (int r = 0; r < NR; r++) {
            Pre &q = g[i][r];
            q.idx = 0;
            if constexpr (D > 0) {
                constexpr int pn = 4 - ((D > 0 ? D - 1 : 0) >> 1);
                const uint32_t ppk = (uint32_t)__builtin_amdgcn_ds_bpermute((int)sl[r].x, (int)st[i].pk);
                const uint32_t act = ((ppk >> 21) & sl[r].y) | sl[r].z;
                q.idx = (int)((ppk & 1023u) * pn + act);
            }
            q.In = e.s_inf[level_offset(D) + q.idx];
            q.k = lds_read_u32(e.wsb + sl[r].w + (uint32_t)(i * sizeof(WaveScratch)));
            const uint32_t *thr = reinterpret_cast<const uint32_t *>(e.s_sigcdf + q.In * kRow + 4);
            q.thr0 = thr[0];
            q.thr1 = n > 2 ? thr[1] : 0xFFFFFFFFu;
            q.thr2 = n > 3 ? thr[2] : 0xFFFFFFFFu;
        }
#pragma unroll
    for (int i = 0; i < NP; i++)
#pragma unroll
        for (int r = 0; r < NR; r++) {
            const Pre &q = g[i][r];
            const int t = 64 * r + lane;
            if (t < c0 + c1) {
                const int a = (q.thr0 <= q.k) + (q.thr1 <= q.k) + (q.thr2 <= q.k);
                if ((D & 1) == (t < c0 ? 0 : 1)) atomicAdd(&e.s_cnt[q.In], 1u);
                else if (e.s_seen) e.s_seen[q.In] = 1;
                const uint32_t pk = (uint32_t)q.idx | ((uint32_t)q.In << 10) | ((uint32_t)a << 21);
                *(__attribute__((address_space(3))) uint32_t *)(uintptr_t)(e.wsb + (uint32_t)(i * sizeof(WaveScratch) + offsetof(WaveScratch, npk) + 4 * npk_offset(D)) + 4u * (uint32_t)t) = pk;
                if constexpr (D < 5) st[i].pk = pk;
            }
        }
    if constexpr (D == 5) wave_lds_sync();
}

#ifdef SCOPA_WALK_STAMPS
__device__ unsigned long long g_walk_stamps[16];
__device__ unsigned long long g_wave_clocks[3 * 16];
__device__ unsigned long long g_wave_phases[4 * 16];
#define WALK_STAMP(i) do { const unsigned long long now_ = clock64(); if (blockIdx.x == 0 && threadIdx.x == 0) { g_walk_stamps[i] += now_ - t_prev_; } t_prev_ = now_; } while (0)
#else
#define WALK_STAMP(i) do { } while (0)
#endif

template <int NP>
__device__ __forceinline__ void walk_pairs(const WalkEnv &e, int lane, const uint32_t (&b)[NP], uint32_t iteration, uint32_t seed_lo,
                                           uint32_t seed_hi, unsigned int &my_pairs) {
#ifdef SCOPA_WALK_STAMPS
    const unsigned long long w_start_ = wall_clock64();
    unsigned long long t_prev_ = clock64();
#endif
    draw_pairs<NP>(e.wsb, lane, b, iteration, seed_lo, seed_hi);
    WALK_STAMP(0);
    NodeRegs st[NP];
#pragma unroll
    for (int i = 0; i < NP; i++) st[i].pk = 0u;
    ply_step<0, NP>(e, lane, st); WALK_STAMP(1);
    ply_step<1, NP>(e, lane, st); WALK_STAMP(2);
    ply_step<2, NP>(e, lane, st); WALK_STAMP(3);
    ply_step<3, NP>(e, lane, st); WALK_STAMP(4);
    ply_step<4, NP>(e, lane, st); WALK_STAMP(5);
    ply_step<5, NP>(e, lane, st); WALK_STAMP(6);
    my_pairs += NP;
    {
        uint4 lf[2];
#pragma unroll
        for (int q = 0; q < 2; q++) lf[q] = lds_read_u4(e.tab + 1024u * (uint32_t)(kLvLeaf + q));
        uint32_t ppk[NP][2];
#pragma unroll
        for (int i = 0; i < NP; i++)
#pragma unroll
            for (int q = 0; q < 2; q++) ppk[i][q] = lds_read_u32(e.wsb + lf[q].x + (uint32_t)(i * sizeof(WaveScratch)));
        int I6[NP][2], I7[NP][2], pay[NP][2];
#pragma unroll
        for (int i = 0; i < NP; i++)
#pragma unroll
            for (int q = 0; q < 2; q++) {
                const uint32_t act = ((ppk[i][q] >> 21) & lf[q].y) | lf[q].z;
                const int idx6 = (int)((ppk[i][q] & 1023u) * 2 + act);
                I6[i][q] = e.s_inf[level_offset(6) + idx6];
                I7[i][q] = e.s_inf[level_offset(7) + idx6];
                pay[i][q] = e.s_pay[idx6];
            }
#pragma unroll
        for (int i = 0; i < NP; i++)
#pragma unroll
            for (int q = 0; q < 2; q++) {
                const int t = lane + 64 * q;
                if (t < 2 * 60) {
                    const int trv = t < 60 ? 0 : 1;
                    if (e.s_seen) e.s_seen[trv == 0 ? I7[i][q] : I6[i][q]] = 1;
                    atomicAdd(&e.s_cnt[trv == 0 ? I6[i][q] : I7[i][q]], 1u);
                    *(__attribute__((address_space(3))) int8_t *)(uintptr_t)(e.wsb + (uint32_t)(i * sizeof(WaveScratch) + offsetof(WaveScratch, p6)) + (uint32_t)t) =
                        (int8_t)(trv == 0 ? pay[i][q] : -pay[i][q]);
                }
            }
    }
    wave_lds_sync();
    WALK_STAMP(7);
    if (lane < 2 * kUpd) {
        const bool trav1 = lane >= kUpd;
        uint4 u[6];
#pragma unroll
        for (int q = 0; q < 6; q++) u[q] = lds_read_u4(e.tab + 1024u * (uint32_t)(kLvUpd + q));
        const uint32_t ro[5] = {u[0].x, u[0].y, u[0].z, u[0].w, u[1].x}, own = u[1].y;
        const int nX = (int)u[1].z;
        const uint32_t p6o[4] = {u[2].x, u[2].y, u[2].z, u[2].w};
        const uint32_t am[5] = {u[3].x, u[3].y, u[3].z, u[3].w, u[4].x}, af[5] = {u[4].y, u[4].z, u[4].w, u[5].x, u[5].y};
        uint32_t rec[NP][5];
        int IX[NP], pv[NP][4];
#pragma unroll
        for (int i = 0; i < NP; i++) {
            const uint32_t wi = e.wsb + (uint32_t)(i * sizeof(WaveScratch));
#pragma unroll
            for (int q = 0; q < 5; q++) rec[i][q] = lds_read_u32(wi + ro[q]);
            IX[i] = (int)((lds_read_u32(wi + own) >> 10) & 2047u);
#pragma unroll
            for (int c = 0; c < 4; c++) pv[i][c] = lds_read_i8(wi + p6o[c]);
        }
        double fq[NP][5], sg[NP][4];
        const uint32_t sig = lds_addr(e.s_sigcdf);
#pragma unroll
        for (int i = 0; i < NP; i++) {
#pragma unroll
            for (int q = 0; q < 5; q++)
                fq[i][q] = lds_read_f64(sig + ((rec[i][q] >> 10) & 2047u) * (uint32_t)(kRow * 8) + (((rec[i][q] >> 18) & am[q]) | af[q]));
            const double2 s01 = *reinterpret_cast<const double2 *>(e.s_sigcdf + IX[i] * kRow), s23 = *reinterpret_cast<const double2 *>(e.s_sigcdf + IX[i] * kRow + 2);
            sg[i][0] = s01.x; sg[i][1] = s01.y; sg[i][2] = s23.x; sg[i][3] = s23.y;
        }
#pragma unroll
        for (int i = 0; i < NP; i++) {
            const double even = (fq[i][0] * fq[i][2]) * fq[i][4], odd = fq[i][1] * fq[i][3];
            const double sX = trav1 ? odd : even, rX = trav1 ? even : odd;
            const double w = sX > 0.0 ? rX / sX : 0.0;
            double cfv[4], v = 0.0;
#pragma unroll
            for (int c = 0; c < 4; c++) {
                cfv[c] = 0.5 * (double)pv[i][c];
                const double t = fma(sg[i][c], cfv[c], v);
                v = c < nX ? t : v;
            }
#pragma unroll
            for (int c = 0; c < 4; c++) {
                const double delta = w * (cfv[c] - v);
                if (c < nX && delta != 0.0) atomicAdd(&e.s_dR[IX[i] * 4 + c], delta);
            }
        }
    }
    wave_lds_sync();
    WALK_STAMP(8);
#ifdef SCOPA_WALK_STAMPS
    if (blockIdx.x == 0 && threadIdx.x == 0) { g_walk_stamps[15] += NP; g_walk_stamps[14] += wall_clock64() - w_start_; }
#endif
}

__global__ void __launch_bounds__(64) k_lane_table(uint4 *__restrict__ g_tab) {
    const int lane = threadIdx.x;
    LaneTabRow row;
    for (int i = 0; i < kLaneSlotVecs; i++) row.v[i] = make_uint4(0u, 0u, 0u, 0u);
    lane_slot_build<0, 0>(row, lane);
    lane_slot_build<1, 0>(row, lane);
    lane_slot_build<2, 0>(row, lane);
    lane_slot_build<3, 0>(row, lane);
    lane_slot_build<4, 0>(row, lane);
    lane_slot_build<5, 0>(row, lane);
    lane_slot_build<5, 1>(row, lane);
    for (int q = 0; q < 2; q++) {
        const int t = lane + 64 * q;
        const bool on = t < 2 * 60;
        const int tt = on ? t : 0, trv = tt < 60 ? 0 : 1, j = trv ? tt - 60 : tt;
        int pj = j, kk = 0;
        if (trv == 1) { pj = j / 3; kk = j - pj * 3; }
        row.v[kLvLeaf + q] = make_uint4((uint32_t)(offsetof(WaveScratch, npk) + 4 * (npk_offset(5) + (trv ? 60 : 0) + pj)),
                                        (trv == 1 && kk > 0) ? 0u : ~0u, (trv == 1 && kk > 0) ? (uint32_t)(kk - 1) : 0u, 0u);
    }
    upd_build(row, lane);
    for (int i = 0; i < kLaneSlotVecs; i++) g_tab[i * 64 + lane] = row.v[i];
}

__device__ __forceinline__ void wave_scratch_init(WaveScratch *ws, int n_scratch, int lane, int n_infosets) {
    if (lane == 0)
        for (int i = 0; i < n_scratch; i++) ws[i].npk[kIdentSlot] = (uint32_t)n_infosets << 10;
}

__device__ __forceinline__ int group_of(unsigned int b) { return (int)((b >> 3) % kDeltaGroups); }

__global__ void __launch_bounds__(1024)
k_mccfr_traverse(const uint16_t *__restrict__ g_infoset, const int8_t *__restrict__ g_payoff,
                 const double *__restrict__ g_sigcdf, double *__restrict__ g_groups,
                 int n_infosets, uint32_t seed_lo, uint32_t seed_hi, uint32_t iteration, uint32_t b0, uint32_t nb,
                 unsigned long long *__restrict__ g_wg_counts, uint32_t *__restrict__ g_visit, unsigned long long *__restrict__ g_clock,
                 const uint4 *__restrict__ g_lane_tab, const uint32_t *__restrict__ g_iter, uint32_t track_seen) {
    extern __shared__ __align__(16) unsigned char smem[];
    __shared__ unsigned int s_vis[2];
    if (g_iter) iteration = *g_iter;
    __shared__ uint32_t s_next[1];
    __shared__ uint32_t s_slice[1];
    __shared__ uint4 s_lane_tab[kLaneSlotVecs * 64];
    const unsigned long long t_start = wall_clock64();
#ifdef SCOPA_WALK_STAMPS
    const unsigned long long c_entry_ = clock64();
#endif
    const int I = n_infosets;
    double *s_sigcdf = reinterpret_cast<double *>(smem);
    double *s_dR = s_sigcdf + (size_t)(I + 1) * kRow;
    WaveScratch *s_wave = reinterpret_cast<WaveScratch *>(s_dR + (size_t)I * 4);
    unsigned int *s_cnt = reinterpret_cast<unsigned int *>(s_wave + 2 * (blockDim.x >> 6));
    uint16_t *s_inf = reinterpret_cast<uint16_t *>(reinterpret_cast<unsigned char *>(s_cnt) + (((size_t)I * 4 + 15) & ~(size_t)15));
    int8_t *s_pay = reinterpret_cast<int8_t *>(s_inf + 1656);
    uint8_t *s_seen = reinterpret_cast<uint8_t *>(s_pay + kTerminal);

    const int tid = threadIdx.x, lane = tid & 63, wave = tid >> 6, n_waves = blockDim.x >> 6, nthr = blockDim.x;
    if (tid < 2) s_vis[tid] = 0u;
    const uint4 lane_piece = tid < kLaneSlotVecs * 64 ? g_lane_tab[tid] : make_uint4(0u, 0u, 0u, 0u);
    if (tid == 0) {
        s_slice[0] = 0u;
        const uint32_t per_wg = (nb + gridDim.x - 1) / gridDim.x, W = blockDim.x >> 6;
        const uint32_t first = blockIdx.x * per_wg, count = first < nb ? (nb - first < per_wg ? nb - first : per_wg) : 0u;
        s_next[0] = count >= 2 * W ? 2 * W : W;
    }
    const uint32_t *gi = reinterpret_cast<const uint32_t *>(g_infoset), *gp = reinterpret_cast<const uint32_t *>(g_payoff);
    {
        constexpr int kSig = 5;
        const double2 *g2 = reinterpret_cast<const double2 *>(g_sigcdf);
        double2 *s2 = reinterpret_cast<double2 *>(s_sigcdf);
        double2 v[kSig];
#pragma unroll
        for (int j = 0; j < kSig; j++) {
            const int idx = tid + j * nthr;
            v[j] = idx < I * 3 ? g2[idx] : make_double2(0.0, 0.0);
        }
        const uint32_t wi = tid < kDecision / 2 ? gi[tid] : 0u;
        const uint32_t wp = tid < kTerminal / 4 ? gp[tid] : 0u;
        const uint16_t last_inf = g_infoset[kDecision - 1];
        for (int i = tid; i < I * 2; i += nthr) reinterpret_cast<double2 *>(s_dR)[i] = make_double2(0.0, 0.0);
        for (int r = tid; r < I; r += nthr) s_cnt[r] = 0u;
        if (track_seen) for (int r = tid; r < I; r += nthr) s_seen[r] = 0;
        if (tid < 4) s_sigcdf[(size_t)I * kRow + tid] = 1.0;
#pragma unroll
        for (int j = 0; j < kSig; j++) {
            const int idx = tid + j * nthr;
            if (idx < I * 3) s2[idx] = v[j];
        }
        for (int idx = tid + kSig * nthr; idx < I * 3; idx += nthr) s2[idx] = g2[idx];
        if (tid < kLaneSlotVecs * 64) s_lane_tab[tid] = lane_piece;
        if (tid < kDecision / 2) reinterpret_cast<uint32_t *>(s_inf)[tid] = wi;
        if (tid == 0) s_inf[kDecision - 1] = last_inf;
        if (tid < kTerminal / 4) reinterpret_cast<uint32_t *>(s_pay)[tid] = wp;
    }
    for (int i = tid + nthr; i < kLaneSlotVecs * 64; i += nthr) s_lane_tab[i] = g_lane_tab[i];
    for (int i = tid + nthr; i < kDecision / 2; i += nthr) reinterpret_cast<uint32_t *>(s_inf)[i] = gi[i];
    for (int i = tid + nthr; i < kTerminal / 4; i += nthr) reinterpret_cast<uint32_t *>(s_pay)[i] = gp[i];
    __syncthreads();
    const unsigned long long t_pro = wall_clock64();
#ifdef SCOPA_WALK_STAMPS
    const unsigned long long c_barrier_ = clock64();
    unsigned long long c_loop0_ = 0, c_loop1_ = 0;
#endif

    WaveScratch *ws = s_wave + 2 * wave;
    wave_scratch_init(ws, 2, lane, I);
    WalkEnv env;
    env.wsb = lds_addr(ws); env.tab = lds_addr(s_lane_tab) + 16u * (uint32_t)lane;
    env.s_inf = s_inf; env.s_pay = s_pay; env.s_sigcdf = s_sigcdf; env.s_dR = s_dR; env.s_seen = track_seen ? s_seen : nullptr; env.s_cnt = s_cnt;
    unsigned int my_pairs = 0;
    {
#ifdef SCOPA_WALK_STAMPS
        const unsigned long long loop_start_ = clock64();
        c_loop0_ = loop_start_;
#endif
        const uint32_t per_wg = (nb + gridDim.x - 1) / gridDim.x;
        const uint32_t first = blockIdx.x * per_wg, count = first < nb ? (nb - first < per_wg ? nb - first : per_wg) : 0u;
        const uint32_t W = (uint32_t)n_waves;
        const bool start_two = count >= 2 * W;
        uint32_t c = start_two ? 2 * (uint32_t)wave : (uint32_t)wave, g = start_two ? 2u : 1u;
        for (;;) {
            if (g == 2 && c + 1 < count) {
                const uint32_t two[2] = {b0 + first + c, b0 + first + c + 1};
                walk_pairs<2>(env, lane, two, iteration, seed_lo, seed_hi, my_pairs);
            } else if (c < count) {
                const uint32_t one[1] = {b0 + first + c};
                walk_pairs<1>(env, lane, one, iteration, seed_lo, seed_hi, my_pairs);
            }
            if (count <= W || c + g >= count) break;
            g = count - c > 4 * W ? 2u : 1u;
            uint32_t got = 0;
            if (lane == 0) got = atomicAdd(s_next, g);
            c = (uint32_t)__builtin_amdgcn_readfirstlane((int)got);
            if (c >= count) break;
        }
#ifdef SCOPA_WALK_STAMPS
        c_loop1_ = clock64();
        if (lane == 0 && (blockIdx.x == 0 || blockIdx.x == 100)) g_wave_clocks[(blockIdx.x == 0 ? 0 : 16) + wave] += c_loop1_ - loop_start_;
        if (lane == 0 && blockIdx.x == 0) { unsigned int hw; asm volatile("s_getreg_b32 %0, hwreg(HW_REG_HW_ID)" : "=s"(hw)); g_wave_clocks[32 + wave] = hw; }
#endif
    }
    {
        uint32_t sl = 0;
        if (lane == 0) sl = atomicAdd(s_slice, 1u);
        sl = (uint32_t)__builtin_amdgcn_readfirstlane((int)sl);
        const int W = n_waves;
        if ((int)sl < W - W / 4) {
            const int per = (I + W - 1) / W, r0 = (W - 1 - (int)sl) * per, r1 = r0 + per < I ? r0 + per : I;
            double *tab = g_groups + (size_t)group_of(blockIdx.x) * kDeltaTable;
            for (int r = r0 + lane; r < r1; r += 64) {
#pragma unroll
                for (int k = 0; k < 4; k++) {
                    const double v = __longlong_as_double((long long)atomicExch(reinterpret_cast<unsigned long long *>(&s_dR[r * 4 + k]), 0ull));
                    if (v != 0.0) atomicAdd(&tab[group_cell(k, r)], v);
                }
                const unsigned int c = atomicExch(&s_cnt[r], 0u);
                if (c != 0u) { atomicAdd(&tab[group_cell(4, r)], (double)c); if (track_seen) s_seen[r] = 1; }
            }
        }
    }
    __syncthreads();

    const unsigned long long t_walk = wall_clock64();
    {
        const bool first0 = track_seen && tid < I && (s_seen[tid] || s_cnt[tid]) && g_visit[tid] == 0u;
        const bool first1 = track_seen && tid + nthr < I && (s_seen[tid + nthr] || s_cnt[tid + nthr]) && g_visit[tid + nthr] == 0u;
        double *tab = g_groups + (size_t)group_of(blockIdx.x) * kDeltaTable;
        for (int r = tid; r < I; r += nthr) {
            const double2 a = reinterpret_cast<const double2 *>(s_dR)[r * 2], b = reinterpret_cast<const double2 *>(s_dR)[r * 2 + 1];
            const unsigned int c = s_cnt[r];
            if (a.x != 0.0) atomicAdd(&tab[group_cell(0, r)], a.x);
            if (a.y != 0.0) atomicAdd(&tab[group_cell(1, r)], a.y);
            if (b.x != 0.0) atomicAdd(&tab[group_cell(2, r)], b.x);
            if (b.y != 0.0) atomicAdd(&tab[group_cell(3, r)], b.y);
            if (c != 0u) atomicAdd(&tab[group_cell(4, r)], (double)c);
        }
        if (first0) g_visit[tid] = 0x40000000u + (uint32_t)tid;
        if (first1) g_visit[tid + nthr] = 0x40000000u + (uint32_t)(tid + nthr);
        if (track_seen)
            for (int r = tid + 2 * nthr; r < I; r += nthr)
                if ((s_seen[r] || s_cnt[r]) && g_visit[r] == 0u) g_visit[r] = 0x40000000u + (uint32_t)r;
    }
    if (lane == 0) { atomicAdd(&s_vis[0], my_pairs * kPairDecisionVisits); atomicAdd(&s_vis[1], my_pairs * kPairTerminalVisits); }
    __syncthreads();
    if (tid < 2) atomicAdd(&g_wg_counts[blockIdx.x * 2 + tid], (unsigned long long)s_vis[tid]);
#ifdef SCOPA_WALK_STAMPS
    if (blockIdx.x == 0 && (tid & 63) == 0) {
        g_wave_phases[(tid >> 6)] += c_barrier_ - c_entry_; g_wave_phases[16 + (tid >> 6)] += c_loop0_ - c_barrier_;
        g_wave_phases[32 + (tid >> 6)] += c_loop1_ - c_loop0_; g_wave_phases[48 + (tid >> 6)] += clock64() - c_loop1_;
    }
#endif
    if (g_clock && tid == 0) {
        g_clock[blockIdx.x * 4] = t_start; g_clock[blockIdx.x * 4 + 1] = t_pro; g_clock[blockIdx.x * 4 + 2] = t_walk; g_clock[blockIdx.x * 4 + 3] = wall_clock64();
    }
}

__global__ void __launch_bounds__(1024)
k_mccfr_multi(const uint16_t *__restrict__ g_infoset, const int8_t *__restrict__ g_payoff, const uint64_t *__restrict__ g_key,
              double *__restrict__ g_regret, double *__restrict__ g_strat, const int32_t *__restrict__ g_meta, uint32_t *__restrict__ g_visit,
              unsigned long long *__restrict__ g_counters, uint32_t seed_lo, uint32_t seed_hi, uint32_t iter0, uint32_t n_iters,
              uint32_t batch, const uint4 *__restrict__ g_lane_tab) {
    extern __shared__ __align__(16) unsigned char smem[];
    __shared__ unsigned int s_vis[2];
    __shared__ uint4 s_lane_tab[kLaneSlotVecs * 64];
    for (int i = threadIdx.x; i < kLaneSlotVecs * 64; i += blockDim.x) s_lane_tab[i] = g_lane_tab[i];
    {
        const size_t deal = blockIdx.x;
        g_infoset += deal * kDecision; g_payoff += deal * kTerminal; g_key += deal * kDecision; g_regret += deal * kDecision * 4;
        g_strat += deal * kDecision * 4; g_meta += deal * 8; g_visit += deal * kDecision; g_counters += deal * 8;
    }
    const int I = g_meta[0];
    double *s_sigcdf = reinterpret_cast<double *>(smem);
    double *s_R = s_sigcdf + (size_t)(I + 1) * kRow;
    WaveScratch *s_wave = reinterpret_cast<WaveScratch *>(s_R + (size_t)I * 4);
    unsigned int *s_cnt = reinterpret_cast<unsigned int *>(s_wave + (blockDim.x >> 6));
    uint16_t *s_inf = reinterpret_cast<uint16_t *>(reinterpret_cast<unsigned char *>(s_cnt) + (((size_t)I * 4 + 15) & ~(size_t)15));
    int8_t *s_pay = reinterpret_cast<int8_t *>(s_inf + 1656);
    uint8_t *s_seen = reinterpret_cast<uint8_t *>(s_pay + kTerminal);
    const int tid = threadIdx.x, lane = tid & 63, wave = tid >> 6, n_waves = blockDim.x >> 6;
    if (tid < 2) s_vis[tid] = 0u;
    for (int i = tid; i < I * 4; i += blockDim.x) s_R[i] = g_regret[i];
    for (int r = tid; r < I; r += blockDim.x) { s_cnt[r] = 0u; s_seen[r] = 0; }
    for (int i = tid; i < kDecision; i += blockDim.x) s_inf[i] = g_infoset[i];
    for (int i = tid; i < kTerminal; i += blockDim.x) s_pay[i] = g_payoff[i];
    if (tid < 4) s_sigcdf[(size_t)I * kRow + tid] = 1.0;
    __syncthreads();
    WaveScratch *ws = s_wave + wave;
    wave_scratch_init(ws, 1, lane, I);
    WalkEnv env;
    env.wsb = lds_addr(ws); env.tab = lds_addr(s_lane_tab) + 16u * (uint32_t)lane;
    env.s_inf = s_inf; env.s_pay = s_pay; env.s_sigcdf = s_sigcdf; env.s_dR = s_R; env.s_seen = s_seen; env.s_cnt = s_cnt;
    unsigned int my_pairs = 0;
    for (uint32_t it = 0; it < n_iters; it++) {
        for (int r = tid; r < I; r += blockDim.x) {
            const int n = (int)((g_key[r] >> 1) & 7);
            double sg[4];
            uint32_t thr[4];
            mc_sigma(s_R + r * 4, n, sg);
            choice_cdf(sg, n, thr);
            for (int c = 0; c < 4; c++) { s_sigcdf[r * kRow + c] = sg[c]; reinterpret_cast<uint32_t *>(s_sigcdf + r * kRow + 4)[c] = thr[c]; }
        }
        __syncthreads();
        for (uint32_t pg = (uint32_t)wave; pg < batch; pg += (uint32_t)n_waves) {
            const uint32_t one[1] = {pg};
            walk_pairs<1>(env, lane, one, iter0 + it, seed_lo, seed_hi, my_pairs);
        }
        __syncthreads();
        for (int r = tid; r < I; r += blockDim.x) {
            const unsigned int c = s_cnt[r];
            if (c) {
                s_seen[r] = 1;
                const int n = (int)((g_key[r] >> 1) & 7);
                for (int k = 0; k < n; k++) g_strat[r * 4 + k] += (double)c * s_sigcdf[r * kRow + k];
                s_cnt[r] = 0u;
            }
        }
        __syncthreads();
    }
    for (int i = tid; i < I * 4; i += blockDim.x) g_regret[i] = s_R[i];
    for (int r = tid; r < I; r += blockDim.x) if (s_seen[r] && g_visit[r] == 0u) g_visit[r] = 0x40000000u + (uint32_t)r;
    if (lane == 0) { atomicAdd(&s_vis[0], my_pairs * kPairDecisionVisits); atomicAdd(&s_vis[1], my_pairs * kPairTerminalVisits); }
    __syncthreads();
    if (tid < 2) g_counters[tid] += s_vis[tid];
}

__global__ void __launch_bounds__(256)
k_mccfr_fold(double *__restrict__ g_groups, double *__restrict__ g_delta, int n_infosets) {
    const int r = blockIdx.x * blockDim.x + threadIdx.x;
    if (r >= n_infosets) return;
    double d[5] = {0.0, 0.0, 0.0, 0.0, 0.0};
    for (int g = 0; g < kDeltaGroups; g++)
        for (int k = 0; k < 5; k++) {
            double *q = g_groups + (size_t)g * kDeltaTable + group_cell(k, r);
            d[k] += *q;
            *q = 0.0;
        }
    for (int k = 0; k < 5; k++) g_delta[r * 5 + k] += d[k];
}

struct ApplyRow { double R[4], S[4], sg[4]; int n; };

__device__ __forceinline__ ApplyRow apply_row_load(int r, const uint64_t *__restrict__ g_key, const double *__restrict__ g_regret,
                                                   const double *__restrict__ g_strat, const double *__restrict__ g_sigcdf) {
    ApplyRow a;
    const double2 r0 = *reinterpret_cast<const double2 *>(g_regret + r * 4), r1 = *reinterpret_cast<const double2 *>(g_regret + r * 4 + 2);
    const double2 s0 = *reinterpret_cast<const double2 *>(g_strat + r * 4), s1 = *reinterpret_cast<const double2 *>(g_strat + r * 4 + 2);
    const double2 g0 = *reinterpret_cast<const double2 *>(g_sigcdf + r * kRow), g1 = *reinterpret_cast<const double2 *>(g_sigcdf + r * kRow + 2);
    a.n = (int)((g_key[r] >> 1) & 7);
    a.R[0] = r0.x; a.R[1] = r0.y; a.R[2] = r1.x; a.R[3] = r1.y;
    a.S[0] = s0.x; a.S[1] = s0.y; a.S[2] = s1.x; a.S[3] = s1.y;
    a.sg[0] = g0.x; a.sg[1] = g0.y; a.sg[2] = g1.x; a.sg[3] = g1.y;
    return a;
}

__device__ __forceinline__ void apply_row_store(int r, ApplyRow &a, const double (&d)[5], double *__restrict__ g_regret,
                                                double *__restrict__ g_strat, double *__restrict__ g_sigcdf) {
#pragma unroll
    for (int c = 0; c < 4; c++)
        if (c < a.n) { a.R[c] += d[c]; a.S[c] += d[4] * a.sg[c]; }
    *reinterpret_cast<double2 *>(g_regret + r * 4) = make_double2(a.R[0], a.R[1]);
    *reinterpret_cast<double2 *>(g_regret + r * 4 + 2) = make_double2(a.R[2], a.R[3]);
    *reinterpret_cast<double2 *>(g_strat + r * 4) = make_double2(a.S[0], a.S[1]);
    *reinterpret_cast<double2 *>(g_strat + r * 4 + 2) = make_double2(a.S[2], a.S[3]);
    double sg[4];
    uint32_t thr[4];
    mc_sigma(a.R, a.n, sg);
    choice_cdf(sg, a.n, thr);
    row_store(g_sigcdf + r * kRow, sg, thr);
}

__device__ __forceinline__ double groups_cell_take(double *__restrict__ g_groups, int r, int k) {
    double v[kDeltaGroups];
#pragma unroll
    for (int g = 0; g < kDeltaGroups; g++) v[g] = g_groups[(size_t)g * kDeltaTable + group_cell(k, r)];
    double d = 0.0;
#pragma unroll
    for (int g = 0; g < kDeltaGroups; g++) {
        d += v[g];
        if (v[g] != 0.0) g_groups[(size_t)g * kDeltaTable + group_cell(k, r)] = 0.0;
    }
    return d;
}

constexpr int kApplyLanes = 8, kApplyThreads = 64;

__global__ void __launch_bounds__(kApplyThreads)
k_mccfr_apply_groups(const uint64_t *__restrict__ g_key, double *__restrict__ g_regret, double *__restrict__ g_strat,
                     double *__restrict__ g_groups, int n_infosets, double *__restrict__ g_sigcdf, uint32_t *__restrict__ g_iter) {
    if (g_iter && blockIdx.x == 0 && threadIdx.x == 0) *g_iter += 1u;
    const int lane = threadIdx.x & 63, k = lane & (kApplyLanes - 1);
    const int r = (int)(blockIdx.x * blockDim.x + threadIdx.x) / kApplyLanes;
    const bool valid = r < n_infosets;
    ApplyRow a{};
    if (valid && k == 0) a = apply_row_load(r, g_key, g_regret, g_strat, g_sigcdf);
    const double mine = (valid && k < 5) ? groups_cell_take(g_groups, r, k) : 0.0;
    double d[5];
#pragma unroll
    for (int j = 0; j < 5; j++) d[j] = __shfl(mine, (lane & ~(kApplyLanes - 1)) + j);
    if (valid && k == 0) apply_row_store(r, a, d, g_regret, g_strat, g_sigcdf);
}

__global__ void __launch_bounds__(64)
k_mccfr_apply(const uint64_t *__restrict__ g_key, double *__restrict__ g_regret, double *__restrict__ g_strat,
              double *__restrict__ g_delta, int n_infosets, double *__restrict__ g_sigcdf) {
    const int r = blockIdx.x * blockDim.x + threadIdx.x;
    if (r >= n_infosets) return;
    double d[5];
    for (int k = 0; k < 5; k++) d[k] = g_delta[r * 5 + k];
    ApplyRow a = apply_row_load(r, g_key, g_regret, g_strat, g_sigcdf);
    for (int k = 0; k < 5; k++) g_delta[r * 5 + k] = 0.0;
    apply_row_store(r, a, d, g_regret, g_strat, g_sigcdf);
}

__global__ void __launch_bounds__(64)
k_mccfr_exchange_apply(scopa::P2PArgs xa, double *__restrict__ g_groups, const uint64_t *__restrict__ g_key, double *__restrict__ g_regret,
                       double *__restrict__ g_strat, double *__restrict__ g_sigcdf, int n_infosets) {
    __shared__ double xch[4][scopa::kP2PMaxWorld][5];
    const int rl = threadIdx.x >> 4, q = threadIdx.x & 15;
    const int r = blockIdx.x * 4 + rl;
    const bool valid = r < n_infosets;
    const double mine = (valid && q < 5) ? groups_cell_take(g_groups, r, q) : 0.0;
    double d[5];
#pragma unroll
    for (int j = 0; j < 5; j++) d[j] = __shfl(mine, (int)(threadIdx.x & ~15u) + j);
    ApplyRow a{};
    if (valid && q == 0) a = apply_row_load(r, g_key, g_regret, g_strat, g_sigcdf);
    scopa::p2p_exchange_wave4(xa, r, valid, q, d, xch[rl]);
    if (valid && q == 0) apply_row_store(r, a, d, g_regret, g_strat, g_sigcdf);
}

namespace {
struct ReplayWalk {
    double *R, *S;
    const uint16_t *inf;
    const int8_t *pay;
    uint32_t *visit;
    const double *uniforms;
    long long upos, n_uniforms;
    uint32_t seq;
    unsigned long long dvis, tvis;
};

template <int D, int TRAV>
__device__ __forceinline__ double replay_rec(ReplayWalk &w, int idx, double reach_opp, double samp_trav) {
    if constexpr (D == kPlies) {
        w.tvis++;
        const int p0 = w.pay[idx];
        return 0.5 * (double)(TRAV == 0 ? p0 : -p0);
    } else {
        constexpr int n = 4 - (D >> 1);
        constexpr bool is_trav = (D & 1) == TRAV;
        w.dvis++;
        const int I = w.inf[level_offset(D) + idx];
        if (w.visit[I] == 0u) w.visit[I] = ++w.seq;
        double R[4], sigma[4], cdf[4];
        for (int c = 0; c < 4; c++) R[c] = w.R[I * 4 + c];
        mc_sigma(R, n, sigma);
        choice_cdf_f64(sigma, n, cdf);
        const double u = w.upos < w.n_uniforms ? w.uniforms[w.upos] : 0.0;
        w.upos++;
        int a = (cdf[0] <= u) + (cdf[1] <= u) + (cdf[2] <= u) + (cdf[3] <= u);
        a = a < n - 1 ? a : n - 1;
        double sa = sigma[0];
        for (int i = 1; i < n; i++) sa = a == i ? sigma[i] : sa;
        if constexpr (!is_trav) {
            return replay_rec<D + 1, TRAV>(w, idx * n + a, reach_opp * sa, samp_trav);
        } else {
            const double util = replay_rec<D + 1, TRAV>(w, idx * n + a, reach_opp, samp_trav * sa);
            double cfv[4] = {0.0, 0.0, 0.0, 0.0};
#pragma unroll 1
            for (int i = 0; i < n; i++)
                cfv[i] = replay_rec<D + 1, TRAV>(w, idx * n + i, reach_opp, samp_trav * sigma[i]);
            double v = 0.0;
            for (int i = 0; i < n; i++) v = fma(sigma[i], cfv[i], v);
            const double wt = samp_trav > 0.0 ? reach_opp / samp_trav : 0.0;
            for (int i = 0; i < n; i++) {
                w.R[I * 4 + i] += wt * (cfv[i] - v);
                w.S[I * 4 + i] += 1.0 * sigma[i];
            }
            return util;
        }
    }
}
}

__global__ void __launch_bounds__(256)
k_mccfr_replay(const uint16_t *__restrict__ g_infoset, const int8_t *__restrict__ g_payoff, const uint64_t *__restrict__ g_key,
               double *__restrict__ g_regret, double *__restrict__ g_strat, const double *__restrict__ uniforms,
               long long n_uniforms, int n_iters, unsigned long long *__restrict__ g_counters, long long *__restrict__ consumed,
               uint32_t *__restrict__ g_visit, int32_t *__restrict__ g_meta) {
    extern __shared__ __align__(16) unsigned char smem[];
    __shared__ uint16_t s_inf[1656];
    __shared__ int8_t s_pay[kTerminal];
    __shared__ uint32_t s_visit[kDecision];
    const int tid = threadIdx.x, I = g_meta[0], cells = I * 4;
    double *R = reinterpret_cast<double *>(smem), *S = R + cells;
    for (int i = tid; i < cells; i += blockDim.x) { R[i] = g_regret[i]; S[i] = g_strat[i]; }
    for (int i = tid; i < kDecision; i += blockDim.x) s_inf[i] = g_infoset[i];
    for (int i = tid; i < kTerminal; i += blockDim.x) s_pay[i] = g_payoff[i];
    for (int i = tid; i < I; i += blockDim.x) s_visit[i] = g_visit[i];
    __syncthreads();
    if (tid == 0) {
        ReplayWalk w;
        w.R = R; w.S = S; w.inf = s_inf; w.pay = s_pay; w.visit = s_visit; w.uniforms = uniforms; w.upos = 0; w.n_uniforms = n_uniforms;
        w.seq = (uint32_t)g_meta[1]; w.dvis = 0; w.tvis = 0;
#pragma unroll 1
        for (int it = 0; it < n_iters; it++) {
            replay_rec<0, 0>(w, 0, 1.0, 1.0);
            replay_rec<0, 1>(w, 0, 1.0, 1.0);
        }
        g_counters[0] += w.dvis;
        g_counters[1] += w.tvis;
        g_meta[1] = (int32_t)w.seq;
        *consumed = w.upos;
    }
    __syncthreads();
    for (int i = tid; i < cells; i += blockDim.x) { g_regret[i] = R[i]; g_strat[i] = S[i]; }
    for (int i = tid; i < I; i += blockDim.x) g_visit[i] = s_visit[i];
}


static size_t traverse_lds_bytes(int n_infosets, int waves) {
    size_t b = ((size_t)(n_infosets + 1) * kRow + (size_t)n_infosets * 4) * sizeof(double);
    b += (size_t)waves * 2 * sizeof(WaveScratch);
    b += (((size_t)n_infosets * 4 + 15) & ~(size_t)15);
    b += 1656 * 2 + 576;
    b += (size_t)n_infosets;
    return (b + 15) & ~(size_t)15;
}

static int32_t ensure_lane_table(scopa_ctx *ctx) {
    if (ctx->d_lane_tab) return SCOPA_OK;
    SC_HIP(ctx, hipMalloc(&ctx->d_lane_tab, (size_t)kLaneSlotVecs * 64 * sizeof(uint4)));
    hipLaunchKernelGGL(k_lane_table, dim3(1), dim3(64), 0, ctx->stream, (uint4 *)ctx->d_lane_tab);
    SC_HIP(ctx, hipGetLastError());
    return SCOPA_OK;
}

struct TraverseGeom { int threads; size_t lds; uint32_t grid; };

static int32_t refresh_all_seen(scopa_ctx *ctx, bool now) {
    if (ctx->mccfr_all_seen) return SCOPA_OK;
    if (!now && ++ctx->mccfr_seen_wait < 16u) return SCOPA_OK;
    ctx->mccfr_seen_wait = 0;
    uint32_t h[kDecision];
    SC_HIP(ctx, hipMemcpyAsync(h, ctx->d_visit, (size_t)ctx->n_infosets * sizeof(uint32_t), hipMemcpyDeviceToHost, ctx->stream));
    SC_HIP(ctx, hipStreamSynchronize(ctx->stream));
    bool all = true;
    for (int r = 0; r < ctx->n_infosets; r++) all = all && h[r] != 0u;
    ctx->mccfr_all_seen = all;
    return SCOPA_OK;
}

static int32_t prepare_traverse(scopa_ctx *ctx, uint32_t nb, TraverseGeom *g) {
    int waves = 16;
    while (waves > 1 && traverse_lds_bytes(ctx->n_infosets, waves) + kStaticLds > (size_t)ctx->lds_limit) waves = waves > 2 ? waves - 2 : 1;
    g->threads = waves * 64;
    g->lds = traverse_lds_bytes(ctx->n_infosets, waves);
    SC_REQUIRE(ctx, g->lds + kStaticLds <= (size_t)ctx->lds_limit, SCOPA_ELIMIT, "mccfr traverse: infoset tables do not fit in LDS");
    SC_LDS_ATTR(ctx, scopa::kLdsTraverse, k_mccfr_traverse, ctx->lds_limit - kStaticLds);
    const uint32_t n_passes = (nb + waves - 1) / waves;
    g->grid = n_passes < (uint32_t)ctx->n_cus ? n_passes : (uint32_t)ctx->n_cus;
    SC_REQUIRE(ctx, g->grid <= 1024u, SCOPA_ELIMIT, "mccfr traverse: more than 1024 compute units");
    static_assert(kClockStride >= 4 * 512, "clock sample stride");
    if (int32_t rc = ensure_lane_table(ctx)) return rc;
    if (int32_t rc = refresh_all_seen(ctx, false)) return rc;
    if (!ctx->sigcdf_valid) {
        hipLaunchKernelGGL(k_mccfr_prepare, dim3((ctx->n_infosets + 255) / 256), dim3(256), 0, ctx->stream, ctx->d_key,
                           ctx->d_regret, ctx->d_sigcdf, ctx->n_infosets);
        SC_HIP(ctx, hipGetLastError());
        ctx->sigcdf_valid = true;
    }
    return SCOPA_OK;
}

static int32_t launch_traverse(scopa_ctx *ctx, uint32_t iteration, uint32_t b0, uint32_t nb) {
    TraverseGeom g;
    if (int32_t rc = prepare_traverse(ctx, nb, &g)) return rc;
    const int threads = g.threads;
    const size_t lds = g.lds;
    const uint32_t grid = g.grid;
    hipEvent_t ev0 = nullptr, ev1 = nullptr;
    const bool sampled = prof_events(ctx, &ev0, &ev1);
    unsigned long long *clock = sampled && ctx->d_clock && grid <= 512u ? ctx->d_clock + (size_t)((ctx->prof_launches - 1) % kClockSamples) * kClockStride : nullptr;
    if (sampled) ctx->clock_grid[(ctx->prof_launches - 1) % kClockSamples] = clock ? (uint16_t)grid : (uint16_t)0;
    if (sampled)
        hipExtLaunchKernelGGL(k_mccfr_traverse, dim3(grid), dim3(threads), lds, ctx->stream, ev0, ev1, 0, ctx->d_infoset, ctx->d_payoff,
                              ctx->d_sigcdf, ctx->d_groups, ctx->n_infosets, (uint32_t)ctx->seed, (uint32_t)(ctx->seed >> 32),
                              iteration, b0, nb, ctx->d_counters + 8, ctx->d_visit, clock, (const uint4 *)ctx->d_lane_tab, (const uint32_t *)nullptr,
                              ctx->mccfr_all_seen ? 0u : 1u);
    else
        hipLaunchKernelGGL(k_mccfr_traverse, dim3(grid), dim3(threads), lds, ctx->stream, ctx->d_infoset, ctx->d_payoff,
                           ctx->d_sigcdf, ctx->d_groups, ctx->n_infosets, (uint32_t)ctx->seed, (uint32_t)(ctx->seed >> 32),
                           iteration, b0, nb, ctx->d_counters + 8, ctx->d_visit, clock, (const uint4 *)ctx->d_lane_tab, (const uint32_t *)nullptr,
                           ctx->mccfr_all_seen ? 0u : 1u);
    SC_HIP(ctx, hipGetLastError());
    return SCOPA_OK;
}

void scopa::mccfr_graphs_clear(scopa_ctx *ctx) {
    for (auto &e : ctx->mccfr_graphs) (void)hipGraphExecDestroy((hipGraphExec_t)e.exec);
    ctx->mccfr_graphs.clear();
}

static int32_t graph_for(scopa_ctx *ctx, uint32_t batch, uint32_t k, hipGraphExec_t *out) {
    const uint32_t track = ctx->mccfr_all_seen ? 0u : 1u;
    for (auto &e : ctx->mccfr_graphs)
        if (e.batch == batch && e.k == k && e.track == track) { *out = (hipGraphExec_t)e.exec; return SCOPA_OK; }
    TraverseGeom g;
    if (int32_t rc = prepare_traverse(ctx, batch, &g)) return rc;
    uint32_t *d_iter = reinterpret_cast<uint32_t *>(ctx->d_meta + 2);
    hipGraph_t graph = nullptr;
    SC_HIP(ctx, hipStreamBeginCapture(ctx->stream, hipStreamCaptureModeThreadLocal));
    for (uint32_t i = 0; i < k; i++) {
        hipLaunchKernelGGL(k_mccfr_traverse, dim3(g.grid), dim3(g.threads), g.lds, ctx->stream, ctx->d_infoset, ctx->d_payoff,
                           ctx->d_sigcdf, ctx->d_groups, ctx->n_infosets, (uint32_t)ctx->seed, (uint32_t)(ctx->seed >> 32),
                           0u, 0u, batch, ctx->d_counters + 8, ctx->d_visit, (unsigned long long *)nullptr, (const uint4 *)ctx->d_lane_tab, (const uint32_t *)d_iter, track);
        hipLaunchKernelGGL(k_mccfr_apply_groups, dim3((ctx->n_infosets * kApplyLanes + kApplyThreads - 1) / kApplyThreads), dim3(kApplyThreads), 0, ctx->stream, ctx->d_key,
                           ctx->d_regret, ctx->d_strat, ctx->d_groups, ctx->n_infosets, ctx->d_sigcdf, d_iter);
    }
    const hipError_t e_end = hipStreamEndCapture(ctx->stream, &graph);
    if (e_end != hipSuccess || !graph) return scopa::fail(ctx, SCOPA_EHIP, "mccfr graph: stream capture", e_end);
    hipGraphExec_t exec = nullptr;
    const hipError_t e_inst = hipGraphInstantiate(&exec, graph, nullptr, nullptr, 0);
    (void)hipGraphDestroy(graph);
    if (e_inst != hipSuccess) return scopa::fail(ctx, SCOPA_EHIP, "mccfr graph: instantiate", e_inst);
    if (ctx->mccfr_graphs.size() >= 16) { (void)hipGraphExecDestroy((hipGraphExec_t)ctx->mccfr_graphs.front().exec); ctx->mccfr_graphs.erase(ctx->mccfr_graphs.begin()); }
    ctx->mccfr_graphs.push_back({batch, k, track, (void *)exec});
    *out = exec;
    return SCOPA_OK;
}

namespace scopa {
int32_t launch_mccfr_multi(scopa_ctx *ctx, int n_deals, int max_infosets, const uint16_t *d_infoset, const int8_t *d_payoff,
                           const uint64_t *d_key, double *d_regret, double *d_strat, const int32_t *d_meta, uint32_t *d_visit,
                           unsigned long long *d_counters, uint64_t seed, uint32_t iter0, uint32_t n_iters, uint32_t batch) {
    int waves = 16;
    auto need = [&](int w) {
        size_t b = ((size_t)(max_infosets + 1) * kRow + (size_t)max_infosets * 4) * sizeof(double) + (size_t)w * sizeof(WaveScratch);
        b += (((size_t)max_infosets * 4 + 15) & ~(size_t)15) + 1656 * 2 + 576 + (size_t)max_infosets;
        return (b + 15) & ~(size_t)15;
    };
    while (waves > 1 && need(waves) + kStaticLdsMulti > (size_t)ctx->lds_limit) waves -= 2;
    SC_REQUIRE(ctx, need(waves) + kStaticLdsMulti <= (size_t)ctx->lds_limit, SCOPA_ELIMIT, "mccfr multi: infoset tables do not fit in LDS");
    SC_LDS_ATTR(ctx, scopa::kLdsMulti, k_mccfr_multi, ctx->lds_limit - kStaticLdsMulti);
    if (int32_t rc = ensure_lane_table(ctx)) return rc;
    hipLaunchKernelGGL(k_mccfr_multi, dim3(n_deals), dim3(waves * 64), need(waves), ctx->stream, d_infoset, d_payoff, d_key, d_regret, d_strat,
                       d_meta, d_visit, d_counters, (uint32_t)seed, (uint32_t)(seed >> 32), iter0, n_iters, batch, (const uint4 *)ctx->d_lane_tab);
    SC_HIP(ctx, hipGetLastError());
    return SCOPA_OK;
}
}

extern "C" {

int32_t scopa_mccfr_seed(scopa_ctx *ctx, uint64_t seed) {
    if (!ctx) return SCOPA_EINVAL;
    if (seed != ctx->seed) scopa::mccfr_graphs_clear(ctx);
    ctx->seed = seed;
    return SCOPA_OK;
}

int32_t scopa_mccfr_traverse(scopa_ctx *ctx, uint32_t iteration, uint32_t b0, uint32_t nb) {
    if (!ctx) return SCOPA_EINVAL;
    SC_REQUIRE(ctx, ctx->has_deal, SCOPA_ESTATE, "scopa_mccfr_traverse: no deal set");
    SC_REQUIRE(ctx, nb <= (1u << 30), SCOPA_EINVAL, "scopa_mccfr_traverse: batch too large");
    if (nb == 0) return SCOPA_OK;
    SC_HIP(ctx, hipSetDevice(ctx->device));
    scopa::Range r("scopa mccfr traverse (split path)");
    const int32_t rc = launch_traverse(ctx, iteration, b0, nb);
    if (rc != SCOPA_OK) return rc;
    hipLaunchKernelGGL(k_mccfr_fold, dim3((ctx->n_infosets + 255) / 256), dim3(256), 0, ctx->stream, ctx->d_groups, ctx->d_delta, ctx->n_infosets);
    SC_HIP(ctx, hipGetLastError());
    return SCOPA_OK;
}

int32_t scopa_mccfr_delta_buffer(scopa_ctx *ctx, void **d_delta, size_t *bytes) {
    if (!ctx || !d_delta || !bytes) return SCOPA_EINVAL;
    SC_REQUIRE(ctx, ctx->has_deal, SCOPA_ESTATE, "scopa_mccfr_delta_buffer: no deal set");
    *d_delta = ctx->d_delta;
    *bytes = (size_t)ctx->n_infosets * 5 * sizeof(double);
    return SCOPA_OK;
}

int32_t scopa_mccfr_bind_delta(scopa_ctx *ctx, void *d_buf, size_t bytes) {
    if (!ctx) return SCOPA_EINVAL;
    SC_REQUIRE(ctx, ctx->has_deal, SCOPA_ESTATE, "scopa_mccfr_bind_delta: no deal set");
    const size_t need = (size_t)ctx->n_infosets * 5 * sizeof(double);
    if (d_buf) {
        SC_REQUIRE(ctx, bytes >= need, SCOPA_EINVAL, "scopa_mccfr_bind_delta: buffer smaller than n_infosets*5 float64");
        SC_REQUIRE(ctx, ((uintptr_t)d_buf & 15) == 0, SCOPA_EINVAL, "scopa_mccfr_bind_delta: buffer must be 16-byte aligned");
        ctx->d_delta = static_cast<double *>(d_buf);
    } else {
        ctx->d_delta = ctx->d_delta_own;
    }
    SC_HIP(ctx, hipSetDevice(ctx->device));
    SC_HIP(ctx, hipMemsetAsync(ctx->d_delta, 0, need, ctx->stream));
    return SCOPA_OK;
}

int32_t scopa_mccfr_delta_get(scopa_ctx *ctx, double *h_delta) {
    if (!ctx || !h_delta) return SCOPA_EINVAL;
    SC_REQUIRE(ctx, ctx->has_deal, SCOPA_ESTATE, "scopa_mccfr_delta_get: no deal set");
    SC_HIP(ctx, hipMemcpyAsync(h_delta, ctx->d_delta, (size_t)ctx->n_infosets * 5 * sizeof(double), hipMemcpyDeviceToHost, ctx->stream));
    SC_HIP(ctx, hipStreamSynchronize(ctx->stream));
    return SCOPA_OK;
}

int32_t scopa_mccfr_delta_set(scopa_ctx *ctx, const double *h_delta) {
    if (!ctx || !h_delta) return SCOPA_EINVAL;
    SC_REQUIRE(ctx, ctx->has_deal, SCOPA_ESTATE, "scopa_mccfr_delta_set: no deal set");
    SC_HIP(ctx, hipMemcpyAsync(ctx->d_delta, h_delta, (size_t)ctx->n_infosets * 5 * sizeof(double), hipMemcpyHostToDevice, ctx->stream));
    SC_HIP(ctx, hipStreamSynchronize(ctx->stream));
    return SCOPA_OK;
}

int32_t scopa_mccfr_apply(scopa_ctx *ctx) {
    if (!ctx) return SCOPA_EINVAL;
    SC_REQUIRE(ctx, ctx->has_deal, SCOPA_ESTATE, "scopa_mccfr_apply: no deal set");
    SC_HIP(ctx, hipSetDevice(ctx->device));
    scopa::Range r("scopa mccfr apply (split path)");
    if (!ctx->sigcdf_valid) {
        hipLaunchKernelGGL(k_mccfr_prepare, dim3((ctx->n_infosets + 255) / 256), dim3(256), 0, ctx->stream, ctx->d_key,
                           ctx->d_regret, ctx->d_sigcdf, ctx->n_infosets);
        SC_HIP(ctx, hipGetLastError());
    }
    hipLaunchKernelGGL(k_mccfr_apply, dim3((ctx->n_infosets + 63) / 64), dim3(64), 0, ctx->stream, ctx->d_key,
                       ctx->d_regret, ctx->d_strat, ctx->d_delta, ctx->n_infosets, ctx->d_sigcdf);
    SC_HIP(ctx, hipGetLastError());
    ctx->sigcdf_valid = true;
    ctx->iteration++;
    return SCOPA_OK;
}

int32_t scopa_mccfr_iteration_counter(scopa_ctx *ctx, uint32_t *iteration) {
    if (!ctx || !iteration) return SCOPA_EINVAL;
    *iteration = ctx->iteration;
    return SCOPA_OK;
}

int32_t scopa_mccfr_iterate(scopa_ctx *ctx, uint32_t batch, uint32_t n_iters) {
    if (!ctx) return SCOPA_EINVAL;
    SC_REQUIRE(ctx, ctx->has_deal, SCOPA_ESTATE, "scopa_mccfr_iterate: no deal set");
    SC_REQUIRE(ctx, batch > 0 && batch <= (1u << 30), SCOPA_EINVAL, "scopa_mccfr_iterate: bad batch");
    SC_HIP(ctx, hipSetDevice(ctx->device));
    if (ctx->mccfr_graph_mode && !ctx->prof_on && n_iters > 1) {
        TraverseGeom g;
        if (int32_t rc = prepare_traverse(ctx, batch, &g)) return rc;
        SC_HIP(ctx, hipMemsetD32Async(reinterpret_cast<hipDeviceptr_t>(ctx->d_meta + 2), (int)ctx->iteration, 1, ctx->stream));
        for (uint32_t left = n_iters; left > 0;) {
            const uint32_t k = left >= 64u ? 64u : left;
            if (int32_t rc = refresh_all_seen(ctx, true)) return rc;
            hipGraphExec_t exec = nullptr;
            if (int32_t rc = graph_for(ctx, batch, k, &exec)) return rc;
            SC_HIP(ctx, hipGraphLaunch(exec, ctx->stream));
            ctx->iteration += k;
            left -= k;
        }
        ctx->sigcdf_valid = true;
        return SCOPA_OK;
    }
    for (uint32_t it = 0; it < n_iters; it++) {
        int32_t rc;
        { scopa::Range r("scopa mccfr traverse"); rc = launch_traverse(ctx, ctx->iteration, 0, batch); }
        if (rc != SCOPA_OK) return rc;
        scopa::Range r("scopa mccfr apply");
        hipLaunchKernelGGL(k_mccfr_apply_groups, dim3((ctx->n_infosets * kApplyLanes + kApplyThreads - 1) / kApplyThreads), dim3(kApplyThreads), 0, ctx->stream, ctx->d_key,
                           ctx->d_regret, ctx->d_strat, ctx->d_groups, ctx->n_infosets, ctx->d_sigcdf, (uint32_t *)nullptr);
        SC_HIP(ctx, hipGetLastError());
        ctx->sigcdf_valid = true;
        ctx->iteration++;
    }
    return SCOPA_OK;
}

int32_t scopa_mccfr_graph_mode(scopa_ctx *ctx, int32_t on) {
    if (!ctx) return SCOPA_EINVAL;
    ctx->mccfr_graph_mode = on != 0;
    if (!on) scopa::mccfr_graphs_clear(ctx);
    return SCOPA_OK;
}

int32_t scopa_mccfr_iterate_sharded(scopa_ctx *ctx, uint32_t b0, uint32_t nb, uint32_t n_iters) {
    if (!ctx) return SCOPA_EINVAL;
    SC_REQUIRE(ctx, ctx->has_deal, SCOPA_ESTATE, "scopa_mccfr_iterate_sharded: no deal set");
    SC_REQUIRE(ctx, nb > 0 && nb <= (1u << 30), SCOPA_EINVAL, "scopa_mccfr_iterate_sharded: bad slice");
    SC_HIP(ctx, hipSetDevice(ctx->device));
    for (uint32_t it = 0; it < n_iters; it++) {
        scopa::P2PArgs xa{};
        SC_REQUIRE(ctx, scopa::p2p_next_args(ctx, &xa), SCOPA_ESTATE, "mccfr sharded iteration: peer exchange not connected");
        int32_t rc;
        { scopa::Range r("scopa mccfr traverse"); rc = launch_traverse(ctx, ctx->iteration, b0, nb); }
        if (rc != SCOPA_OK) return rc;
        scopa::Range r("scopa mccfr exchange + apply");
        hipLaunchKernelGGL(k_mccfr_exchange_apply, dim3((ctx->n_infosets + 3) / 4), dim3(64), 0, ctx->stream, xa, ctx->d_groups, ctx->d_key,
                           ctx->d_regret, ctx->d_strat, ctx->d_sigcdf, ctx->n_infosets);
        SC_HIP(ctx, hipGetLastError());
        ctx->sigcdf_valid = true;
        ctx->iteration++;
    }
    SC_HIP(ctx, hipStreamSynchronize(ctx->stream));
    return scopa::p2p_check(ctx, "scopa_mccfr_iterate_sharded");
}

int32_t scopa_mccfr_replay(scopa_ctx *ctx, int32_t n_iters, const double *h_uniforms, int64_t n_uniforms, int64_t *consumed) {
    if (!ctx || n_iters < 0 || n_uniforms < 0 || (n_uniforms > 0 && !h_uniforms)) return SCOPA_EINVAL;
    SC_REQUIRE(ctx, ctx->has_deal, SCOPA_ESTATE, "scopa_mccfr_replay: no deal set");
    SC_HIP(ctx, hipSetDevice(ctx->device));
    const size_t ubytes = (size_t)n_uniforms * sizeof(double);
    { const int32_t rc = ensure_scratch(ctx, ubytes + 64); if (rc != SCOPA_OK) return rc; }
    long long *d_consumed = reinterpret_cast<long long *>(ctx->d_scratch);
    double *d_u = ctx->d_scratch + 8;
    if (n_uniforms) SC_HIP(ctx, hipMemcpyAsync(d_u, h_uniforms, ubytes, hipMemcpyHostToDevice, ctx->stream));
    SC_LDS_ATTR(ctx, scopa::kLdsReplay, k_mccfr_replay, ctx->lds_limit - 12 * 1024);
    hipLaunchKernelGGL(k_mccfr_replay, dim3(1), dim3(256), (size_t)ctx->n_infosets * 64, ctx->stream, ctx->d_infoset, ctx->d_payoff, ctx->d_key,
                       ctx->d_regret, ctx->d_strat, d_u, (long long)n_uniforms, (int)n_iters, ctx->d_counters, d_consumed,
                       ctx->d_visit, ctx->d_meta);
    SC_HIP(ctx, hipGetLastError());
    long long used = 0;
    SC_HIP(ctx, hipMemcpyAsync(&used, d_consumed, sizeof used, hipMemcpyDeviceToHost, ctx->stream));
    SC_HIP(ctx, hipStreamSynchronize(ctx->stream));
    ctx->sigcdf_valid = false;
    if (consumed) *consumed = used;
    return SCOPA_OK;
}

}

#ifdef SCOPA_WALK_STAMPS
extern "C" int scopa_debug_wave_phases(unsigned long long *out64) {
    return hipMemcpyFromSymbol(out64, HIP_SYMBOL(g_wave_phases), sizeof(unsigned long long) * 64) == hipSuccess ? 0 : -1;
}
extern "C" int scopa_debug_wave_clocks(unsigned long long *out48) {
    return hipMemcpyFromSymbol(out48, HIP_SYMBOL(g_wave_clocks), sizeof(unsigned long long) * 48) == hipSuccess ? 0 : -1;
}
extern "C" int scopa_debug_walk_stamps(unsigned long long *out16, int reset) {
    if (hipMemcpyFromSymbol(out16, HIP_SYMBOL(g_walk_stamps), sizeof(unsigned long long) * 16) != hipSuccess) return -1;
    if (reset) { unsigned long long z[16] = {0}; if (hipMemcpyToSymbol(HIP_SYMBOL(g_walk_stamps), z, sizeof(z)) != hipSuccess) return -1; }
    return 0;
}
#endif
```

Baseline: 136.2 billion.

## Precompute next iteration's first Philox draws in apply kernel spare workgroups

Adds extra workgroups to the apply kernel that compute the Philox random blocks for the first walk of each wave in the next iteration and store them to a global buffer. The traverse kernel then loads these precomputed draws into registers at startup instead of running Philox before its first walk, taking RNG latency off the traverse critical path. It also hoists the per-workgroup batch partition and slice row counts to host-computed kernel arguments. This costs an extra global buffer, extra apply-kernel blocks, tag bookkeeping, and an additional load per lane. The graph-mode path does not use the predrawn values.

```diff
diff --git a/include/scopa.h b/include/scopa.h
--- a/include/scopa.h
+++ b/include/scopa.h
@@ -97,6 +97,8 @@
 int32_t scopa_mccfr_apply(scopa_ctx *ctx);
 int32_t scopa_mccfr_iteration_counter(scopa_ctx *ctx, uint32_t *iteration);
 int32_t scopa_mccfr_graph_mode(scopa_ctx *ctx, int32_t on);
+int32_t scopa_mccfr_predraw(scopa_ctx *ctx, int32_t on);
+int32_t scopa_mccfr_predraw_get(scopa_ctx *ctx, uint32_t *h_words, size_t capacity_bytes, size_t *bytes, uint32_t *tag);
 int32_t scopa_debug_lds_limit(scopa_ctx *ctx, int32_t bytes);
 
 int32_t scopa_sdcfr_frontier_width(int32_t traverser, int32_t ply);
diff --git a/scopa_amd/_lib.py b/scopa_amd/_lib.py
--- a/scopa_amd/_lib.py
+++ b/scopa_amd/_lib.py
@@ -17,7 +17,7 @@
     "scopa_tree_counts", "scopa_tree_export", "scopa_tables_reset", "scopa_tables_get", "scopa_tables_set",
     "scopa_visited_get", "scopa_cfr_exact_iterate", "scopa_cfr_exact_traverse", "scopa_cfr_exact_mode", "scopa_cfr_exact_last_route", "scopa_cfr_exact_traverse_from", "scopa_mccfr_replay", "scopa_mccfr_seed",
     "scopa_mccfr_iterate", "scopa_mccfr_traverse", "scopa_mccfr_delta_buffer", "scopa_mccfr_bind_delta", "scopa_mccfr_delta_get", "scopa_mccfr_delta_set", "scopa_mccfr_apply",
-    "scopa_mccfr_iteration_counter", "scopa_mccfr_graph_mode", "scopa_debug_lds_limit", "scopa_sdcfr_frontier_width", "scopa_sdcfr_features", "scopa_sdcfr_expand",
+    "scopa_mccfr_iteration_counter", "scopa_mccfr_graph_mode", "scopa_mccfr_predraw", "scopa_mccfr_predraw_get", "scopa_debug_lds_limit", "scopa_sdcfr_frontier_width", "scopa_sdcfr_features", "scopa_sdcfr_expand",
     "scopa_sdcfr_terminal_values", "scopa_sdcfr_backward", "scopa_sdcfr_visits", "scopa_sdcfr_policy_get", "scopa_sdcfr_traverse_fused", "scopa_sdcfr_image_floats", "scopa_sdcfr_pack_weights", "scopa_sdcfr_tuning", "scopa_sdcfr_mode", "scopa_sdcfr_train_params", "scopa_sdcfr_train_step", "scopa_sdcfr_train_steps", "scopa_sdcfr_average_policy", "scopa_features_from_states",
     "scopa_eval_init_states", "scopa_eval_step", "scopa_eval_tabular_step", "scopa_eval_tabular_prepare", "scopa_eval_tabular_match", "scopa_cfr_sync_iterate", "scopa_multi_create", "scopa_multi_destroy",
     "scopa_multi_deal_py_seeds", "scopa_multi_set_perms", "scopa_multi_perms_get", "scopa_multi_build", "scopa_multi_cfr_exact_iterate",
@@ -112,6 +112,8 @@
         "scopa_mccfr_apply": (i32, [vp]),
         "scopa_mccfr_iteration_counter": (i32, [vp, C.POINTER(u32)]),
         "scopa_mccfr_graph_mode": (i32, [vp, i32]),
+        "scopa_mccfr_predraw": (i32, [vp, i32]),
+        "scopa_mccfr_predraw_get": (i32, [vp, vp, C.c_size_t, C.POINTER(C.c_size_t), C.POINTER(C.c_uint32 * 8)]),
         "scopa_debug_lds_limit": (i32, [vp, i32]),
         "scopa_exploitability": (i32, [vp, vp, vp, vp]),
         "scopa_sdcfr_frontier_width": (i32, [i32, i32]),
@@ -367,6 +369,19 @@
     def mccfr_graph_mode(self, on):
         self._ck(self._L.scopa_mccfr_graph_mode(self._h, 1 if on else 0), "scopa_mccfr_graph_mode")
 
+    def mccfr_predraw(self, on):
+        self._ck(self._L.scopa_mccfr_predraw(self._h, 1 if on else 0), "scopa_mccfr_predraw")
+
+    def mccfr_predraw_get(self):
+        n, tag = C.c_size_t(), (C.c_uint32 * 8)()
+        self._ck(self._L.scopa_mccfr_predraw_get(self._h, None, 0, C.byref(n), C.byref(tag)), "scopa_mccfr_predraw_get")
+        if not tag[0]:
+            return None, None
+        t = dict(iteration=tag[1], b0=tag[2], nb=tag[3], grid=tag[4], threads=tag[5], slots=tag[6], per_wg=tag[7])
+        w = np.zeros(n.value // 4, np.uint32)
+        self._ck(self._L.scopa_mccfr_predraw_get(self._h, _ptr(w), w.nbytes, C.byref(n), C.byref(tag)), "scopa_mccfr_predraw_get")
+        return t, w.reshape(t["grid"], t["threads"] // 64, t["slots"], 64, 4)
+
     def debug_lds_limit(self, nbytes):
         self._ck(self._L.scopa_debug_lds_limit(self._h, int(nbytes)), "scopa_debug_lds_limit")
 
diff --git a/scopa_amd/csrc/scopa_ctx.h b/scopa_amd/csrc/scopa_ctx.h
--- a/scopa_amd/csrc/scopa_ctx.h
+++ b/scopa_amd/csrc/scopa_ctx.h
@@ -78,6 +78,11 @@
     std::vector<GraphEntry> mccfr_graphs;
     bool mccfr_graph_mode = false;
 
+    void *d_draws = nullptr;
+    size_t draws_bytes = 0;
+    bool predraw_on = true;
+    struct DrawsTag { bool valid = false; uint64_t seed = 0; uint32_t iteration = 0, b0 = 0, nb = 0, grid = 0, threads = 0; } draws_tag;
+
     int lds_limit = 160 * 1024;
     int n_cus = 256;
     uint32_t lds_attr_done = 0;
diff --git a/scopa_amd/csrc/scopa_host.hip b/scopa_amd/csrc/scopa_host.hip
--- a/scopa_amd/csrc/scopa_host.hip
+++ b/scopa_amd/csrc/scopa_host.hip
@@ -151,7 +151,7 @@
     scopa::mccfr_graphs_clear(ctx);
     for (hipEvent_t e : ctx->ev_pool) (void)hipEventDestroy(e);
     void *bufs[] = {ctx->d_states, ctx->d_infoset, ctx->d_payoff, ctx->d_key, ctx->d_meta, ctx->d_regret, ctx->d_strat,
-                    ctx->d_local, ctx->d_delta_own, ctx->d_scratch, ctx->d_counters, ctx->d_visit, ctx->d_sigcdf, ctx->d_groups, ctx->d_clock, ctx->d_sched, ctx->d_lane_tab, ctx->d_sdnode, ctx->d_sdpol, ctx->d_train_partial, ctx->d_eval_thr, ctx->d_sdavg};
+                    ctx->d_local, ctx->d_delta_own, ctx->d_scratch, ctx->d_counters, ctx->d_visit, ctx->d_sigcdf, ctx->d_groups, ctx->d_clock, ctx->d_sched, ctx->d_lane_tab, ctx->d_draws, ctx->d_sdnode, ctx->d_sdpol, ctx->d_train_partial, ctx->d_eval_thr, ctx->d_sdavg};
     for (void *b : bufs) if (b) (void)hipFree(b);
     if (ctx->own_stream) (void)hipStreamDestroy(ctx->stream);
     delete ctx;
diff --git a/scopa_amd/csrc/scopa_mccfr.hip b/scopa_amd/csrc/scopa_mccfr.hip
--- a/scopa_amd/csrc/scopa_mccfr.hip
+++ b/scopa_amd/csrc/scopa_mccfr.hip
@@ -101,15 +101,26 @@
 constexpr int kStaticLds = 64 + kLaneSlotVecs * 1024;
 constexpr int kStaticLdsMulti = kStaticLds;
 
+__device__ __forceinline__ philox_out draw_block(int lane, uint32_t b, uint32_t iteration, uint32_t seed_lo, uint32_t seed_hi) {
+    const int trav = lane < 44 ? 0 : 1, p = trav ? lane - 44 : lane;
+    return philox4x32_10((uint32_t)p, b, iteration, (uint32_t)trav, seed_lo, seed_hi);
+}
+
 template <int NP>
 __device__ __forceinline__ void draw_pairs(uint32_t wsb, int lane, const uint32_t (&b)[NP], uint32_t iteration, uint32_t seed_lo, uint32_t seed_hi) {
-    const int trav = lane < 44 ? 0 : 1, p = trav ? lane - 44 : lane;
     philox_out x[NP];
 #pragma unroll
-    for (int i = 0; i < NP; i++) x[i] = philox4x32_10((uint32_t)p, b[i], iteration, (uint32_t)trav, seed_lo, seed_hi);
+    for (int i = 0; i < NP; i++) x[i] = draw_block(lane, b[i], iteration, seed_lo, seed_hi);
 #pragma unroll
     for (int i = 0; i < NP; i++)
         lds_write_u4(wsb + (uint32_t)(i * sizeof(WaveScratch) + offsetof(WaveScratch, kdraw)) + 16u * (uint32_t)lane, x[i].x0 >> 1, x[i].x1 >> 1, x[i].x2 >> 1, x[i].x3 >> 1);
+    wave_lds_sync();
+}
+template <int NP>
+__device__ __forceinline__ void draws_put(uint32_t wsb, int lane, const uint4 (&pre)[2]) {
+#pragma unroll
+    for (int i = 0; i < NP; i++)
+        lds_write_u4(wsb + (uint32_t)(i * sizeof(WaveScratch) + offsetof(WaveScratch, kdraw)) + 16u * (uint32_t)lane, pre[i].x, pre[i].y, pre[i].z, pre[i].w);
     wave_lds_sync();
 }
 
@@ -252,14 +263,15 @@
 #define WALK_STAMP(i) do { } while (0)
 #endif
 
-template <int NP>
+template <int NP, bool PRE = false>
 __device__ __forceinline__ void walk_pairs(const WalkEnv &e, int lane, const uint32_t (&b)[NP], uint32_t iteration, uint32_t seed_lo,
-                                           uint32_t seed_hi, unsigned int &my_pairs) {
+                                           uint32_t seed_hi, unsigned int &my_pairs, const uint4 (&pre)[2]) {
 #ifdef SCOPA_WALK_STAMPS
     const unsigned long long w_start_ = wall_clock64();
     unsigned long long t_prev_ = clock64();
 #endif
-    draw_pairs<NP>(e.wsb, lane, b, iteration, seed_lo, seed_hi);
+    if constexpr (PRE) draws_put<NP>(e.wsb, lane, pre);
+    else draw_pairs<NP>(e.wsb, lane, b, iteration, seed_lo, seed_hi);
     WALK_STAMP(0);
     NodeRegs st[NP];
 #pragma unroll
@@ -399,7 +411,8 @@
                  const double *__restrict__ g_sigcdf, double *__restrict__ g_groups,
                  int n_infosets, uint32_t seed_lo, uint32_t seed_hi, uint32_t iteration, uint32_t b0, uint32_t nb,
                  unsigned long long *__restrict__ g_wg_counts, uint32_t *__restrict__ g_visit, unsigned long long *__restrict__ g_clock,
-                 const uint4 *__restrict__ g_lane_tab, const uint32_t *__restrict__ g_iter, uint32_t track_seen) {
+                 const uint4 *__restrict__ g_lane_tab, const uint32_t *__restrict__ g_iter, uint32_t track_seen,
+                 uint32_t per_wg, uint32_t slice_rows, const uint4 *__restrict__ g_draws, uint32_t draw_slots) {
     extern __shared__ __align__(16) unsigned char smem[];
     __shared__ unsigned int s_vis[2];
     if (g_iter) iteration = *g_iter;
@@ -420,13 +433,19 @@
     uint8_t *s_seen = reinterpret_cast<uint8_t *>(s_pay + kTerminal);
 
     const int tid = threadIdx.x, lane = tid & 63, wave = tid >> 6, n_waves = blockDim.x >> 6, nthr = blockDim.x;
+    const uint32_t first = blockIdx.x * per_wg, count = first < nb ? (nb - first < per_wg ? nb - first : per_wg) : 0u;
+    const bool start_two = count >= 2 * (uint32_t)n_waves;
+    uint4 pre[2] = {make_uint4(0u, 0u, 0u, 0u), make_uint4(0u, 0u, 0u, 0u)};
+    if (g_draws) {
+        const uint4 *q = g_draws + ((size_t)(blockIdx.x * (uint32_t)n_waves + (uint32_t)wave) * draw_slots) * 64 + lane;
+        pre[0] = q[0];
+        if (draw_slots == 2) pre[1] = q[64];
+    }
     if (tid < 2) s_vis[tid] = 0u;
     const uint4 lane_piece = tid < kLaneSlotVecs * 64 ? g_lane_tab[tid] : make_uint4(0u, 0u, 0u, 0u);
     if (tid == 0) {
         s_slice[0] = 0u;
-        const uint32_t per_wg = (nb + gridDim.x - 1) / gridDim.x, W = blockDim.x >> 6;
-        const uint32_t first = blockIdx.x * per_wg, count = first < nb ? (nb - first < per_wg ? nb - first : per_wg) : 0u;
-        s_next[0] = count >= 2 * W ? 2 * W : W;
+        s_next[0] = start_two ? 2 * (uint32_t)n_waves : (uint32_t)n_waves;
     }
     const uint32_t *gi = reinterpret_cast<const uint32_t *>(g_infoset), *gp = reinterpret_cast<const uint32_t *>(g_payoff);
     {
@@ -478,18 +497,28 @@
         const unsigned long long loop_start_ = clock64();
         c_loop0_ = loop_start_;
 #endif
-        const uint32_t per_wg = (nb + gridDim.x - 1) / gridDim.x;
-        const uint32_t first = blockIdx.x * per_wg, count = first < nb ? (nb - first < per_wg ? nb - first : per_wg) : 0u;
         const uint32_t W = (uint32_t)n_waves;
-        const bool start_two = count >= 2 * W;
         uint32_t c = start_two ? 2 * (uint32_t)wave : (uint32_t)wave, g = start_two ? 2u : 1u;
-        for (;;) {
-            if (g == 2 && c + 1 < count) {
+        bool walked = false;
+        if (g_draws) {
+            if (start_two) {
                 const uint32_t two[2] = {b0 + first + c, b0 + first + c + 1};
-                walk_pairs<2>(env, lane, two, iteration, seed_lo, seed_hi, my_pairs);
+                walk_pairs<2, true>(env, lane, two, iteration, seed_lo, seed_hi, my_pairs, pre);
             } else if (c < count) {
                 const uint32_t one[1] = {b0 + first + c};
-                walk_pairs<1>(env, lane, one, iteration, seed_lo, seed_hi, my_pairs);
+                walk_pairs<1, true>(env, lane, one, iteration, seed_lo, seed_hi, my_pairs, pre);
+            }
+            walked = true;
+        }
+        for (;;) {
+            if (walked) {
+                walked = false;
+            } else if (g == 2 && c + 1 < count) {
+                const uint32_t two[2] = {b0 + first + c, b0 + first + c + 1};
+                walk_pairs<2>(env, lane, two, iteration, seed_lo, seed_hi, my_pairs, pre);
+            } else if (c < count) {
+                const uint32_t one[1] = {b0 + first + c};
+                walk_pairs<1>(env, lane, one, iteration, seed_lo, seed_hi, my_pairs, pre);
             }
             if (count <= W || c + g >= count) break;
             g = count - c > 4 * W ? 2u : 1u;
@@ -510,7 +539,7 @@
         sl = (uint32_t)__builtin_amdgcn_readfirstlane((int)sl);
         const int W = n_waves;
         if ((int)sl < W - W / 4) {
-            const int per = (I + W - 1) / W, r0 = (W - 1 - (int)sl) * per, r1 = r0 + per < I ? r0 + per : I;
+            const int per = (int)slice_rows, r0 = (W - 1 - (int)sl) * per, r1 = r0 + per < I ? r0 + per : I;
             double *tab = g_groups + (size_t)group_of(blockIdx.x) * kDeltaTable;
             for (int r = r0 + lane; r < r1; r += 64) {
 #pragma unroll
@@ -595,6 +624,7 @@
     env.wsb = lds_addr(ws); env.tab = lds_addr(s_lane_tab) + 16u * (uint32_t)lane;
     env.s_inf = s_inf; env.s_pay = s_pay; env.s_sigcdf = s_sigcdf; env.s_dR = s_R; env.s_seen = s_seen; env.s_cnt = s_cnt;
     unsigned int my_pairs = 0;
+    const uint4 no_pre[2] = {};
     for (uint32_t it = 0; it < n_iters; it++) {
         for (int r = tid; r < I; r += blockDim.x) {
             const int n = (int)((g_key[r] >> 1) & 7);
@@ -607,7 +637,7 @@
         __syncthreads();
         for (uint32_t pg = (uint32_t)wave; pg < batch; pg += (uint32_t)n_waves) {
             const uint32_t one[1] = {pg};
-            walk_pairs<1>(env, lane, one, iter0 + it, seed_lo, seed_hi, my_pairs);
+            walk_pairs<1>(env, lane, one, iter0 + it, seed_lo, seed_hi, my_pairs, no_pre);
         }
         __syncthreads();
         for (int r = tid; r < I; r += blockDim.x) {
@@ -688,9 +718,58 @@
 
 constexpr int kApplyLanes = 8, kApplyThreads = 64;
 
+#ifndef SCOPA_PREDRAW_STORE
+#define SCOPA_PREDRAW_STORE 2
+#endif
+constexpr int kPredrawItems = 4;
+struct PredrawArgs {
+    uint4 *g_draws;
+    uint32_t n_items;
+    uint32_t seed_lo, seed_hi, iteration, b0, nb, per_wg, waves, slots;
+};
+
+__device__ __forceinline__ void predraw_produce(const PredrawArgs &pa, uint32_t pb, int lane) {
+    uint32_t id[kPredrawItems];
+    bool on[kPredrawItems];
+#pragma unroll
+    for (int q = 0; q < kPredrawItems; q++) {
+        const uint32_t item = pb * kPredrawItems + (uint32_t)q;
+        on[q] = item < pa.n_items;
+        const uint32_t wv = pa.slots == 2 ? item >> 1 : item, s = pa.slots == 2 ? item & 1u : 0u;
+        const uint32_t w = wv / pa.waves, v = wv - w * pa.waves;
+        const uint32_t first = w * pa.per_wg, count = first < pa.nb ? (pa.nb - first < pa.per_wg ? pa.nb - first : pa.per_wg) : 0u;
+        const uint32_t c = count >= 2 * pa.waves ? 2 * v + s : v;
+        id[q] = pa.b0 + first + c;
+    }
+    philox_out x[kPredrawItems];
+#pragma unroll
+    for (int q = 0; q < kPredrawItems; q++) x[q] = draw_block(lane, id[q], pa.iteration, pa.seed_lo, pa.seed_hi);
+#if SCOPA_PREDRAW_STORE == 2
+    const __amdgpu_buffer_rsrc_t rsrc = __builtin_amdgcn_make_buffer_rsrc(pa.g_draws, 0, (int)(pa.n_items * 1024u), 0x00020000);
+#endif
+#pragma unroll
+    for (int q = 0; q < kPredrawItems; q++) {
+        if (!on[q]) continue;
+        const uint32_t at = (pb * kPredrawItems + (uint32_t)q) * 64u + (uint32_t)lane;
+        const u32x4 val = u32x4{x[q].x0 >> 1, x[q].x1 >> 1, x[q].x2 >> 1, x[q].x3 >> 1};
+#if SCOPA_PREDRAW_STORE == 2
+        __builtin_amdgcn_raw_buffer_store_b128(val, rsrc, (int)(at * 16u), 0, 16);
+#elif SCOPA_PREDRAW_STORE == 1
+        __builtin_nontemporal_store(val, reinterpret_cast<u32x4 *>(pa.g_draws) + at);
+#else
+        reinterpret_cast<u32x4 *>(pa.g_draws)[at] = val;
+#endif
+    }
+}
+
 __global__ void __launch_bounds__(kApplyThreads)
 k_mccfr_apply_groups(const uint64_t *__restrict__ g_key, double *__restrict__ g_regret, double *__restrict__ g_strat,
-                     double *__restrict__ g_groups, int n_infosets, double *__restrict__ g_sigcdf, uint32_t *__restrict__ g_iter) {
+                     double *__restrict__ g_groups, int n_infosets, double *__restrict__ g_sigcdf, uint32_t *__restrict__ g_iter,
+                     uint32_t n_apply_wgs, PredrawArgs pa) {
+    if (blockIdx.x >= n_apply_wgs) {
+        predraw_produce(pa, blockIdx.x - n_apply_wgs, (int)(threadIdx.x & 63));
+        return;
+    }
     if (g_iter && blockIdx.x == 0 && threadIdx.x == 0) *g_iter += 1u;
     const int lane = threadIdx.x & 63, k = lane & (kApplyLanes - 1);
     const int r = (int)(blockIdx.x * blockDim.x + threadIdx.x) / kApplyLanes;
@@ -841,7 +920,7 @@
     return SCOPA_OK;
 }
 
-struct TraverseGeom { int threads; size_t lds; uint32_t grid; };
+struct TraverseGeom { int threads; size_t lds; uint32_t grid, per_wg, slice_rows, draw_slots; };
 
 static int32_t refresh_all_seen(scopa_ctx *ctx, bool now) {
     if (ctx->mccfr_all_seen) return SCOPA_OK;
@@ -866,6 +945,9 @@
     const uint32_t n_passes = (nb + waves - 1) / waves;
     g->grid = n_passes < (uint32_t)ctx->n_cus ? n_passes : (uint32_t)ctx->n_cus;
     SC_REQUIRE(ctx, g->grid <= 1024u, SCOPA_ELIMIT, "mccfr traverse: more than 1024 compute units");
+    g->per_wg = (nb + g->grid - 1) / g->grid;
+    g->slice_rows = (uint32_t)((ctx->n_infosets + waves - 1) / waves);
+    g->draw_slots = g->per_wg >= 2u * (uint32_t)waves ? 2u : 1u;
     static_assert(kClockStride >= 4 * 512, "clock sample stride");
     if (int32_t rc = ensure_lane_table(ctx)) return rc;
     if (int32_t rc = refresh_all_seen(ctx, false)) return rc;
@@ -878,12 +960,17 @@
     return SCOPA_OK;
 }
 
-static int32_t launch_traverse(scopa_ctx *ctx, uint32_t iteration, uint32_t b0, uint32_t nb) {
+static int32_t launch_traverse(scopa_ctx *ctx, uint32_t iteration, uint32_t b0, uint32_t nb, TraverseGeom *geom = nullptr) {
     TraverseGeom g;
     if (int32_t rc = prepare_traverse(ctx, nb, &g)) return rc;
+    if (geom) *geom = g;
     const int threads = g.threads;
     const size_t lds = g.lds;
     const uint32_t grid = g.grid;
+    const scopa_ctx::DrawsTag &t = ctx->draws_tag;
+    const uint4 *const draws = ctx->predraw_on && t.valid && t.seed == ctx->seed && t.iteration == iteration && t.b0 == b0 && t.nb == nb && t.grid == grid &&
+                                 t.threads == (uint32_t)threads
+                             ? (const uint4 *)ctx->d_draws : nullptr;
     hipEvent_t ev0 = nullptr, ev1 = nullptr;
     const bool sampled = prof_events(ctx, &ev0, &ev1);
     unsigned long long *clock = sampled && ctx->d_clock && grid <= 512u ? ctx->d_clock + (size_t)((ctx->prof_launches - 1) % kClockSamples) * kClockStride : nullptr;
@@ -892,12 +979,40 @@
         hipExtLaunchKernelGGL(k_mccfr_traverse, dim3(grid), dim3(threads), lds, ctx->stream, ev0, ev1, 0, ctx->d_infoset, ctx->d_payoff,
                               ctx->d_sigcdf, ctx->d_groups, ctx->n_infosets, (uint32_t)ctx->seed, (uint32_t)(ctx->seed >> 32),
                               iteration, b0, nb, ctx->d_counters + 8, ctx->d_visit, clock, (const uint4 *)ctx->d_lane_tab, (const uint32_t *)nullptr,
-                              ctx->mccfr_all_seen ? 0u : 1u);
+                              ctx->mccfr_all_seen ? 0u : 1u, g.per_wg, g.slice_rows, draws, g.draw_slots);
     else
         hipLaunchKernelGGL(k_mccfr_traverse, dim3(grid), dim3(threads), lds, ctx->stream, ctx->d_infoset, ctx->d_payoff,
                            ctx->d_sigcdf, ctx->d_groups, ctx->n_infosets, (uint32_t)ctx->seed, (uint32_t)(ctx->seed >> 32),
                            iteration, b0, nb, ctx->d_counters + 8, ctx->d_visit, clock, (const uint4 *)ctx->d_lane_tab, (const uint32_t *)nullptr,
-                           ctx->mccfr_all_seen ? 0u : 1u);
+                           ctx->mccfr_all_seen ? 0u : 1u, g.per_wg, g.slice_rows, draws, g.draw_slots);
+    SC_HIP(ctx, hipGetLastError());
+    return SCOPA_OK;
+}
+
+static int32_t launch_apply_groups(scopa_ctx *ctx, const TraverseGeom &g, uint32_t iteration, uint32_t b0, uint32_t nb) {
+    const uint32_t n_apply = (uint32_t)((ctx->n_infosets * kApplyLanes + kApplyThreads - 1) / kApplyThreads);
+    PredrawArgs pa{};
+    uint32_t n_produce = 0;
+    const uint32_t waves = (uint32_t)g.threads / 64u;
+    if (ctx->predraw_on && nb <= 2u * waves * g.grid) {
+        const uint32_t n_items = g.grid * waves * g.draw_slots;
+        const size_t bytes = (size_t)n_items * 1024;
+        if (bytes > ctx->draws_bytes) {
+            ctx->draws_tag.valid = false;
+            if (ctx->d_draws) SC_HIP(ctx, hipFree(ctx->d_draws));
+            ctx->d_draws = nullptr; ctx->draws_bytes = 0;
+            SC_HIP(ctx, hipMalloc(&ctx->d_draws, bytes));
+            ctx->draws_bytes = bytes;
+        }
+        pa.g_draws = (uint4 *)ctx->d_draws; pa.n_items = n_items;
+        pa.seed_lo = (uint32_t)ctx->seed; pa.seed_hi = (uint32_t)(ctx->seed >> 32);
+        pa.iteration = iteration + 1; pa.b0 = b0; pa.nb = nb; pa.per_wg = g.per_wg; pa.waves = waves; pa.slots = g.draw_slots;
+        n_produce = (n_items + kPredrawItems - 1) / kPredrawItems;
+        ctx->draws_tag.valid = true; ctx->draws_tag.seed = ctx->seed; ctx->draws_tag.iteration = iteration + 1;
+        ctx->draws_tag.b0 = b0; ctx->draws_tag.nb = nb; ctx->draws_tag.grid = g.grid; ctx->draws_tag.threads = (uint32_t)g.threads;
+    }
+    hipLaunchKernelGGL(k_mccfr_apply_groups, dim3(n_apply + n_produce), dim3(kApplyThreads), 0, ctx->stream, ctx->d_key,
+                       ctx->d_regret, ctx->d_strat, ctx->d_groups, ctx->n_infosets, ctx->d_sigcdf, (uint32_t *)nullptr, n_apply, pa);
     SC_HIP(ctx, hipGetLastError());
     return SCOPA_OK;
 }
@@ -919,9 +1034,11 @@
     for (uint32_t i = 0; i < k; i++) {
         hipLaunchKernelGGL(k_mccfr_traverse, dim3(g.grid), dim3(g.threads), g.lds, ctx->stream, ctx->d_infoset, ctx->d_payoff,
                            ctx->d_sigcdf, ctx->d_groups, ctx->n_infosets, (uint32_t)ctx->seed, (uint32_t)(ctx->seed >> 32),
-                           0u, 0u, batch, ctx->d_counters + 8, ctx->d_visit, (unsigned long long *)nullptr, (const uint4 *)ctx->d_lane_tab, (const uint32_t *)d_iter, track);
-        hipLaunchKernelGGL(k_mccfr_apply_groups, dim3((ctx->n_infosets * kApplyLanes + kApplyThreads - 1) / kApplyThreads), dim3(kApplyThreads), 0, ctx->stream, ctx->d_key,
-                           ctx->d_regret, ctx->d_strat, ctx->d_groups, ctx->n_infosets, ctx->d_sigcdf, d_iter);
+                           0u, 0u, batch, ctx->d_counters + 8, ctx->d_visit, (unsigned long long *)nullptr, (const uint4 *)ctx->d_lane_tab, (const uint32_t *)d_iter, track,
+                           g.per_wg, g.slice_rows, (const uint4 *)nullptr, g.draw_slots);
+        const uint32_t n_apply = (uint32_t)((ctx->n_infosets * kApplyLanes + kApplyThreads - 1) / kApplyThreads);
+        hipLaunchKernelGGL(k_mccfr_apply_groups, dim3(n_apply), dim3(kApplyThreads), 0, ctx->stream, ctx->d_key,
+                           ctx->d_regret, ctx->d_strat, ctx->d_groups, ctx->n_infosets, ctx->d_sigcdf, d_iter, n_apply, PredrawArgs{});
     }
     const hipError_t e_end = hipStreamEndCapture(ctx->stream, &graph);
     if (e_end != hipSuccess || !graph) return scopa::fail(ctx, SCOPA_EHIP, "mccfr graph: stream capture", e_end);
@@ -1066,15 +1183,35 @@
     }
     for (uint32_t it = 0; it < n_iters; it++) {
         int32_t rc;
-        { scopa::Range r("scopa mccfr traverse"); rc = launch_traverse(ctx, ctx->iteration, 0, batch); }
+        TraverseGeom g;
+        { scopa::Range r("scopa mccfr traverse"); rc = launch_traverse(ctx, ctx->iteration, 0, batch, &g); }
         if (rc != SCOPA_OK) return rc;
         scopa::Range r("scopa mccfr apply");
-        hipLaunchKernelGGL(k_mccfr_apply_groups, dim3((ctx->n_infosets * kApplyLanes + kApplyThreads - 1) / kApplyThreads), dim3(kApplyThreads), 0, ctx->stream, ctx->d_key,
-                           ctx->d_regret, ctx->d_strat, ctx->d_groups, ctx->n_infosets, ctx->d_sigcdf, (uint32_t *)nullptr);
-        SC_HIP(ctx, hipGetLastError());
+        if ((rc = launch_apply_groups(ctx, g, ctx->iteration, 0, batch)) != SCOPA_OK) return rc;
         ctx->sigcdf_valid = true;
         ctx->iteration++;
     }
+    return SCOPA_OK;
+}
+
+int32_t scopa_mccfr_predraw(scopa_ctx *ctx, int32_t on) {
+    if (!ctx) return SCOPA_EINVAL;
+    ctx->predraw_on = on != 0;
+    if (!on) ctx->draws_tag.valid = false;
+    return SCOPA_OK;
+}
+
+int32_t scopa_mccfr_predraw_get(scopa_ctx *ctx, uint32_t *h_words, size_t capacity_bytes, size_t *bytes, uint32_t *tag) {
+    if (!ctx || !bytes || !tag) return SCOPA_EINVAL;
+    const scopa_ctx::DrawsTag &t = ctx->draws_tag;
+    const uint32_t waves = t.threads / 64u, per_wg = t.valid ? (t.nb + t.grid - 1) / t.grid : 0u, slots = t.valid && per_wg >= 2u * waves ? 2u : 1u;
+    *bytes = t.valid ? (size_t)t.grid * waves * slots * 1024 : 0;
+    tag[0] = t.valid ? 1u : 0u; tag[1] = t.iteration; tag[2] = t.b0; tag[3] = t.nb; tag[4] = t.grid; tag[5] = t.threads; tag[6] = slots; tag[7] = per_wg;
+    if (!t.valid || !h_words) return SCOPA_OK;
+    SC_REQUIRE(ctx, capacity_bytes >= *bytes, SCOPA_EINVAL, "scopa_mccfr_predraw_get: buffer too small");
+    SC_HIP(ctx, hipSetDevice(ctx->device));
+    SC_HIP(ctx, hipMemcpyAsync(h_words, ctx->d_draws, *bytes, hipMemcpyDeviceToHost, ctx->stream));
+    SC_HIP(ctx, hipStreamSynchronize(ctx->stream));
     return SCOPA_OK;
 }
 
```

After: 120.3 billion. 0.883x the previous value.
